# arpg/vicalib

Measured on AMD Instinct MI355X. Metric: corner_residuals_per_sec, higher is better.
Workload: dtype f64

## Files before the change

include/vicalib_amd.h:

```cpp
#ifndef VICALIB_AMD_H_
#define VICALIB_AMD_H_

#ifdef __cplusplus
extern "C" {
#endif

typedef struct vc_calibrator vc_calibrator;

enum {
  VC_OK = 0,
  VC_ERR_NO_DEVICE = -1,
  VC_ERR_BAD_ARG = -2,
  VC_ERR_RUNNING = -3,
  VC_ERR_TIME_ORDER = -4,
  VC_ERR_TOO_MANY_POINTS = -5,
  VC_ERR_NUMERIC = -6,
  VC_ERR_UNSUPPORTED = -7,
  VC_ERR_NO_CONVERGENCE = -8
};

enum { VC_MODEL_FOV = 0, VC_MODEL_POLY2 = 1, VC_MODEL_POLY3 = 2, VC_MODEL_KB4 = 3, VC_MODEL_LINEAR = 4, VC_MODEL_RATIONAL6 = 5 };

int vc_create(vc_calibrator** out, int device);
void vc_destroy(vc_calibrator* h);
int vc_clear(vc_calibrator* h);

int vc_add_camera(vc_calibrator* h, int model, const double* params, int nparams, int width, int height,
                  const double T_ck[7]);
int vc_fix_camera_intrinsics(vc_calibrator* h, int should_fix);
int vc_add_frame(vc_calibrator* h, const double T_wk[7], double time);
int vc_set_frame_pose(vc_calibrator* h, int frame, const double T_wk[7]);
int vc_init_frame_poses_pnp(vc_calibrator* h, int* n_initialised);
int vc_pnp_planar(int model, const double* params, int nparams, int n, const double* p_w ,
                  const double* p_c , double T_cw[7], double* rms_px);
int vc_pnp_planar_ransac(int model, const double* params, int nparams, int n, const double* p_w, const double* p_c,
                         int iterations, double tol_px, double T_cw[7], double* rms_px, int* n_inliers, char* inlier);
int vc_set_pnp_ransac(vc_calibrator* h, int iterations, double tol_px);
int vc_add_observations(vc_calibrator* h, int frame, int camera, int n, const double* p_w ,
                        const double* p_c );
int vc_add_observation_tiles(vc_calibrator* h, int n_tiles, const int* tile_frame, const int* tile_cam,
                             const long long* tile_off , const double* points, int n_points,
                             const int* point_id, const double* p_c );
int vc_add_imu(vc_calibrator* h, int n, const double* gyro , const double* accel ,
               const double* time );

int vc_set_sigmas(vc_calibrator* h, double gyro_sigma, double accel_sigma);
int vc_set_biases(vc_calibrator* h, const double biases[6]);
int vc_set_scale_factor(vc_calibrator* h, const double scale[6]);
int vc_set_time_offset(vc_calibrator* h, double offset);
int vc_set_function_tolerance(vc_calibrator* h, double tol);
int vc_set_optimization_flags(vc_calibrator* h, int bias_active, int inertial_active, int rotation_only,
                              int optimize_time_offset);
int vc_set_max_iters(vc_calibrator* h, int max_iters);
int vc_set_tolerances(vc_calibrator* h, double gradient_tolerance, double parameter_tolerance);
int vc_set_calibrate_imu(vc_calibrator* h, int calibrate_imu);
int vc_set_remove_outliers(vc_calibrator* h, int remove_outliers, double outlier_threshold);

int vc_solve(vc_calibrator* h);
int vc_start(vc_calibrator* h);
int vc_resume(vc_calibrator* h);
int vc_set_stage_limit(vc_calibrator* h, int n);
int vc_is_running(vc_calibrator* h);
int vc_stop(vc_calibrator* h);

int vc_num_frames(vc_calibrator* h);
int vc_num_imu_blocks(vc_calibrator* h);
int vc_num_cameras(vc_calibrator* h);
int vc_get_camera(vc_calibrator* h, int camera, double* params, int* nparams, double T_ck[7]);
int vc_get_frame(vc_calibrator* h, int frame, double T_wk[7], double v_w[3], double* time);
int vc_get_biases(vc_calibrator* h, double biases[6]);
int vc_get_scale_factor(vc_calibrator* h, double scale[6]);
int vc_get_gravity(vc_calibrator* h, double g_dir[2]);
double vc_time_offset(vc_calibrator* h);
double vc_mean_squared_error(vc_calibrator* h);
int vc_get_camera_proj_rmse(vc_calibrator* h, double* rmse );
unsigned vc_get_num_iterations(vc_calibrator* h);
int vc_num_imu_measurements(vc_calibrator* h);
int vc_get_imu_measurements(vc_calibrator* h, double* gyro, double* accel, double* time, int max_n);
int vc_get_integration_poses(vc_calibrator* h, int id, double* poses, int max_poses);
int vc_print_results(vc_calibrator* h, char* buf, int len);
int vc_write_camera_models(vc_calibrator* h, const char* filename);

int vc_solution_covariance_dim(vc_calibrator* h);
int vc_get_solution_covariance(vc_calibrator* h, double* cov, int max_n, int* n);
int vc_get_solution_covariance_names(vc_calibrator* h, char* buf, int len);

int vc_set_gravity(vc_calibrator* h, const double g_dir[2]);
int vc_set_frame_velocities(vc_calibrator* h, const double* v_w , int n);
int vc_trace_len(vc_calibrator* h);
int vc_get_trace(vc_calibrator* h, double* rows, int max_rows);
typedef int (*vc_allreduce_fn)(void* ctx, double* device_buf, int count, int op );
int vc_set_shard(vc_calibrator* h, int rank, int world_size, vc_allreduce_fn fn, void* ctx);
void* vc_get_stream(vc_calibrator* h);
int vc_rccl_unique_id(void* out128);
int vc_set_shard_rccl(vc_calibrator* h, int rank, int world_size, const void* unique_id128);
typedef struct vc_shard_comm vc_shard_comm;
int vc_shard_comm_create(int device, int rank, int world_size, const void* unique_id128, vc_shard_comm** out);
int vc_set_shard_comm(vc_calibrator* h, vc_shard_comm* comm);
void vc_shard_comm_destroy(vc_shard_comm* comm);
long long vc_allreduce_calls(vc_calibrator* h);
int vc_shard_info(vc_calibrator* h, int* rank, int* world_size, int* rccl_ranks, int* rccl_rank);
int vc_pass_paths(vc_calibrator* h, int* out6);
const char* vc_last_error(void);
int vc_prepare(vc_calibrator* h);
int vc_linearize(vc_calibrator* h, double* cost, double* Hpp, double* gp, double* S, double* g_red,
                 double* hss_diag, double* g_s);
int vc_shared_dim(vc_calibrator* h);
int vc_step_hold(vc_calibrator* h, double radius, double* cost, double* delta_s, double* slam, double* frame_lam, double* poses,
                 double* vels, double* cams, double* imus);
int vc_run_iterations(vc_calibrator* h, int iters, int* jac_sweeps, int* res_sweeps);
int vc_download_state(vc_calibrator* h);
int vc_evaluate(vc_calibrator* h, double* cost, double* sum_sq);
int vc_time_kernels(vc_calibrator* h, int reps, double* jac_ms, double* res_ms);
int vc_set_kernel_timing(vc_calibrator* h, int on);
int vc_sync_timeouts(const vc_calibrator* h);
int vc_get_kernel_timing(vc_calibrator* h, char* names, int names_len, double* total_ms, long long* count, int max_entries);
int vc_time_stages(vc_calibrator* h, int reps, double out[6]);
int vc_get_imu_blocks(vc_calibrator* h, double* H, double* g, double* cost);
int vc_get_imu_weights(vc_calibrator* h, double* W);
int vc_report_compute(vc_calibrator* h, int bins_x, int bins_y);
int vc_report_corners(vc_calibrator* h, long long first, long long n, double* r, int* frame, int* camera, unsigned char* flags);
long long vc_report_num_corners(vc_calibrator* h);
int vc_report_num_views(vc_calibrator* h);
int vc_report_views(vc_calibrator* h, int* frame, int* camera, int* count, int* removed, double* sum_sq, double* max_err,
                    long long* worst_corner);
int vc_report_error_map(vc_calibrator* h, int camera, double* cells);
int vc_report_num_imu_blocks(vc_calibrator* h);
int vc_report_imu(vc_calibrator* h, double* whitened , double* unwhitened , unsigned char* flags);
int vc_time_report_sweeps(vc_calibrator* h, int reps, double out_ms[3]);
int vc_holdout_clear(vc_calibrator* h);
int vc_holdout_add_tiles(vc_calibrator* h, int n_tiles, const int* tile_frame, const int* tile_cam, const long long* tile_off ,
                         const double* points, int n_points, const int* point_id, const double* p_c );
int vc_holdout_compute(vc_calibrator* h, const double* seeds, int max_iters);
int vc_holdout_num_frames(vc_calibrator* h);
int vc_holdout_num_views(vc_calibrator* h);
long long vc_holdout_num_corners(vc_calibrator* h);
int vc_holdout_frames(vc_calibrator* h, double* T_wk , int* status, int* iterations, double* cost0, double* cost, int* behind);
int vc_holdout_views(vc_calibrator* h, int* frame, int* camera, int* count, double* sum_sq, double* max_err, long long* worst_corner);
int vc_holdout_corners(vc_calibrator* h, long long first, long long n, double* r , int* frame, int* camera);
int vc_holdout_camera_rmse(vc_calibrator* h, double* rmse , long long* count );
int vc_time_holdout(vc_calibrator* h, int reps, double out_ms[2]);
int vc_get_debug_stamps(vc_calibrator* h, long long out[32]);
long long vc_num_observations(vc_calibrator* h);
int vc_num_tiles(vc_calibrator* h);

typedef struct vc_detector vc_detector;
int vc_detector_create(int device, int width, int height, vc_detector** out);
void vc_detector_destroy(vc_detector* d);
int vc_detector_set_params(vc_detector* d, int black_on_white, double at_threshold, double at_window_ratio, double conic_min_area,
                           double conic_min_density, double conic_min_aspect);
int vc_detector_find(vc_detector* d, const unsigned char* image, int pitch, double* centres, int max_conics, int* n_found);
int vc_detector_find_conics(vc_detector* d, const unsigned char* image, int pitch, double* centres, double* conics, int* boxes, int max_conics,
                            int* n_found);
int vc_target_make_pattern(int rows, int cols, unsigned seed, int* pattern);
int vc_target_find(const double* centres, const double* conics, int n, const int* pattern, int rows, int cols, int* dot_index, int* n_matched);

typedef struct vc_undistorter vc_undistorter;
int vc_undistorter_create(int device, int model, const double* params, int nparams, int src_w, int src_h, const double dst_linear[4], int dst_w,
                          int dst_h, const double R_ds[9], int fill, vc_undistorter** out);
int vc_undistorter_create_for_camera(vc_calibrator* h, int camera, const double dst_linear[4], int dst_w, int dst_h, const double R_ds[9], int fill,
                                     vc_undistorter** out);
void vc_undistorter_destroy(vc_undistorter* u);
int vc_undistort_fit_linear(int model, const double* params, int nparams, int src_w, int src_h, int dst_w, int dst_h, double alpha, double dst_linear[4]);
int vc_undistort_images(vc_undistorter* u, int n, const unsigned char* src, int src_pitch, long long src_stride, unsigned char* dst, int dst_pitch,
                        long long dst_stride);
int vc_undistort_images_device(vc_undistorter* u, int n, const unsigned char* d_src, int src_pitch, long long src_stride, unsigned char* d_dst,
                               int dst_pitch, long long dst_stride);
void* vc_undistort_stream(vc_undistorter* u);
int vc_undistort_points(vc_undistorter* u, int n, const double* src_px , double* dst_px , unsigned char* valid );
int vc_undistort_get_map(vc_undistorter* u, float* map, unsigned char* valid);
int vc_undistort_get_linear(vc_undistorter* u, double dst_linear[4], int dst_size[2]);
int vc_time_undistort(vc_undistorter* u, int n_images, int reps, double out_ms[3]);

int vc_stereo_rectify_rotations(const double T_ck_a[7], const double T_ck_b[7], double R_ds_a[9], double R_ds_b[9], double* baseline);
int vc_stereo_fit_linear(int model_a, const double* params_a, int nparams_a, int w_a, int h_a, const double R_ds_a[9], int model_b, const double* params_b,
                         int nparams_b, int w_b, int h_b, const double R_ds_b[9], int dst_w, int dst_h, double alpha, double dst_linear[4]);
int vc_match_tiles(int n_tiles, const int* tile_frame, const int* tile_cam, const long long* tile_off , const int* point_id, int cam_a,
                   int cam_b, int* n_frames, long long* n_pairs, int* frame, long long* frame_off, long long* pos_a, long long* pos_b);
typedef struct vc_rectifier vc_rectifier;
int vc_rectifier_create(int device, int model_a, const double* params_a, int nparams_a, int w_a, int h_a, const double T_ck_a[7], int model_b,
                        const double* params_b, int nparams_b, int w_b, int h_b, const double T_ck_b[7], const double dst_linear[4], int dst_w, int dst_h,
                        double alpha, int fill, vc_rectifier** out);
int vc_rectifier_create_for_cameras(vc_calibrator* h, int cam_a, int cam_b, const double dst_linear[4], int dst_w, int dst_h, double alpha, int fill,
                                    vc_rectifier** out);
void vc_rectifier_destroy(vc_rectifier* r);
vc_undistorter* vc_rectifier_side(vc_rectifier* r, int side);
int vc_rectifier_get(vc_rectifier* r, double R_ds_a[9], double R_ds_b[9], double dst_linear[4], int dst_size[2], double* baseline, double T_ck_rect_a[7],
                     double T_ck_rect_b[7]);
int vc_rectify_pairs(vc_rectifier* r, int n, const unsigned char* src_a, int src_pitch_a, long long src_stride_a, const unsigned char* src_b, int src_pitch_b,
                     long long src_stride_b, unsigned char* dst_a, int dst_pitch_a, long long dst_stride_a, unsigned char* dst_b, int dst_pitch_b,
                     long long dst_stride_b);
int vc_rectify_check(vc_rectifier* r, int n_frames, const long long* frame_off , const double* px_a, const double* px_b, const double* target,
                     double* pairs_out, unsigned char* flags, int* count, int* invalid, double* sum_dv, double* sum_dv2, double* max_abs_dv, long long* worst,
                     double* mean_z, double* rigid_rms);
int vc_time_rectify_check(vc_rectifier* r, int reps, double* out_ms);

typedef struct vc_comparer vc_comparer;
int vc_comparer_create(int device, int model_a, const double* params_a, int nparams_a, int model_b, const double* params_b, int nparams_b, int width,
                       int height, int grid_x, int grid_y, vc_comparer** out);
int vc_comparer_create_for_camera(vc_calibrator* h, int camera, int model_b, const double* params_b, int nparams_b, int grid_x, int grid_y, vc_comparer** out);
void vc_comparer_destroy(vc_comparer* c);
int vc_compare_run(vc_comparer* c, double fit_radius, int max_iters, const double R_ba[9]);
int vc_compare_get_fit(vc_comparer* c, double R_ba[9], int* status, int* iterations, int* n_fit, int* n_left_out, double* cost0, double* cost);
int vc_compare_get_map(vc_comparer* c, double* diff , unsigned char* flags );
int vc_compare_summary(vc_comparer* c, long long* count, long long* invalid, double* sum_du, double* sum_dv, double* sum_sq, double* max_err, long long* worst);
int vc_compare_rings(vc_comparer* c, int n_rings, long long* count, long long* invalid, double* sum_sq, double* max_err);
int vc_compare_extrinsics(const double T_ck_a0[7], const double T_ck_ac[7], const double T_ck_b0[7], const double T_ck_bc[7], const double R_0[9],
                          const double R_c[9], double out4[4]);
int vc_time_compare(vc_comparer* c, int reps, double out_ms[3]);

typedef struct vc_converter vc_converter;
int vc_converter_create(int device, int model_a, const double* params_a, int nparams_a, int width, int height, int model_b, int grid_x, int grid_y,
                        vc_converter** out);
int vc_converter_create_for_camera(vc_calibrator* h, int camera, int model_b, int grid_x, int grid_y, vc_converter** out);
void vc_converter_destroy(vc_converter* c);
int vc_convert_run(vc_converter* c, double fit_radius, int max_iters, const double* start, unsigned int free_mask);
int vc_convert_get(vc_converter* c, double* params_b, int* nparams_b, int* status, int* iterations, int* n_fit, int* n_left_out, double* cost0, double* cost,
                   double* max_err, long long* worst);
int vc_convert_comparer(vc_converter* c, vc_comparer** out);
int vc_time_convert(vc_converter* c, int reps, double out_ms[3]);

typedef struct vc_uncertainty vc_uncertainty;
int vc_uncertainty_create(int device, int model, const double* params, int nparams, int width, int height, int grid_x, int grid_y, vc_uncertainty** out);
int vc_uncertainty_create_for_camera(vc_calibrator* h, int camera, int grid_x, int grid_y, vc_uncertainty** out);
void vc_uncertainty_destroy(vc_uncertainty* u);
int vc_uncertainty_run(vc_uncertainty* u, const double* cov, double sigma_px, double fit_radius);
int vc_uncertainty_get_fit(vc_uncertainty* u, double* M , double* G , int* n_fit);
int vc_uncertainty_get_map(vc_uncertainty* u, double* sigma , unsigned char* flags );
int vc_uncertainty_summary(vc_uncertainty* u, long long* count, long long* invalid, double* sum_var, double* max_lam, long long* worst);
int vc_uncertainty_rings(vc_uncertainty* u, int n_rings, long long* count, long long* invalid, double* sum_var, double* max_lam);
int vc_time_uncertainty(vc_uncertainty* u, int reps, double out_ms[3]);

#ifdef __cplusplus
}
#endif
#endif
```

vicalib_amd/csrc/vc_capi.cpp:

```cpp
#include "vc_calibrator.hpp"
#include "vc_uncertainty.hpp"

static int env_bit(const char* name) { const char* e = std::getenv(name); return (e && (e[0] == '0' || e[0] == '1')) ? e[0] - '0' : -1; }
Switches Switches::read() {
  Switches w;
  w.graphs = env_bit("VICALIB_AMD_GRAPHS") == 1;
  w.merged = env_bit("VICALIB_AMD_NO_MERGED_DECISION") != 1;
  w.batched = std::getenv("VICALIB_AMD_BATCHED") != nullptr;
  { const char* e = std::getenv("VICALIB_AMD_STREAM2_PRIORITY"); w.stream2_default = e && std::strcmp(e, "default") == 0; }
  w.flag_sync = env_bit("VICALIB_AMD_FLAG_SYNC");
  w.shard_flag_sync = env_bit("VICALIB_AMD_SHARD_FLAG_SYNC");
  w.force_shard_path = env_bit("VICALIB_AMD_FORCE_SHARD_PATH") == 1;
  { const char* e = std::getenv("VICALIB_AMD_SYNC_BOUND"); if (e && std::atoll(e) > 0) w.sync_bound = std::atoll(e); }
  { const char* e = std::getenv("VICALIB_AMD_SYNC_BOUND_FROM_PASS"); if (e) w.sync_bound_from_pass = std::atoi(e); }
  w.pre_backsub = env_bit("VICALIB_AMD_PRE_BACKSUB");
  w.chain.fold_l0 = env_bit("VICALIB_AMD_FOLD_L0") != 0; w.chain.back_path = env_bit("VICALIB_AMD_BACK_PATH") != 0;
  w.chain.hadd_early = env_bit("VICALIB_AMD_HADD_EARLY") != 0; w.chain.defer_tail = env_bit("VICALIB_AMD_DEFER_TAIL") != 0;
  return w;
}

extern "C" {

int vc_create(vc_calibrator** out, int device) {
  if (!out) return VC_ERR_BAD_ARG;
  *out = nullptr;
  int n = 0;
  if (hipGetDeviceCount(&n) != hipSuccess || n <= 0 || device < 0 || device >= n) return VC_ERR_NO_DEVICE;
  if (hipSetDevice(device) != hipSuccess) return VC_ERR_NO_DEVICE;
  vc_calibrator* h = new vc_calibrator();
  h->device = device;
  h->sw = Switches::read();
  h->use_graphs = h->sw.graphs; h->merged_enabled = h->sw.merged; h->shard_flag_sync = h->sw.shard_flag_sync == 1;
  const unsigned evf = hipEventDisableTiming | hipEventDisableSystemFence;
  int prio_least = 0, prio_greatest = 0;
  (void)hipDeviceGetStreamPriorityRange(&prio_least, &prio_greatest);
  auto make_stream2 = [&]() -> hipError_t {
    if (!h->sw.stream2_default && prio_least != prio_greatest && hipStreamCreateWithPriority(&h->stream2, hipStreamDefault, prio_least) == hipSuccess) { h->flag_sync = true; return hipSuccess; }
    (void)hipGetLastError();
    return hipStreamCreate(&h->stream2);
  };
  if (hipStreamCreate(&h->stream) != hipSuccess || make_stream2() != hipSuccess ||
      hipEventCreateWithFlags(&h->ev_state, evf) != hipSuccess || hipEventCreateWithFlags(&h->ev_pre, evf) != hipSuccess ||
      hipEventCreateWithFlags(&h->ev_weights, evf) != hipSuccess ||
      hipEventCreateWithFlags(&h->ev_imujac, evf) != hipSuccess ||
      hipEventCreateWithFlags(&h->ev_reduced, evf) != hipSuccess || hipEventCreateWithFlags(&h->ev_back, evf) != hipSuccess) { delete h; return VC_ERR_NO_DEVICE; }
  if (h->sw.flag_sync >= 0) h->flag_sync = h->sw.flag_sync == 1;
  if (h->d_sync.alloc(kSyncWords) != hipSuccess || hipMemset(h->d_sync.p, 0, kSyncWords * sizeof(long long)) != hipSuccess) { delete h; return VC_ERR_NO_DEVICE; }
  *out = h;
  return VC_OK;
}
void vc_destroy(vc_calibrator* h) { if (h) (void)hipSetDevice(h->device); delete h; }

int vc_clear(vc_calibrator* h) {
  if (!h) return VC_ERR_BAD_ARG;
  h->stop();
  h->cams.clear(); h->frames.clear(); h->o_frame.clear(); h->o_cam.clear(); h->o_pid.clear(); h->pts.clear(); h->o_pc.clear(); h->o_removed.clear();
  h->mse = 0; h->num_iterations = 0; h->is_bias_active = false; h->is_scale_active = false; h->is_inertial_active = false;
  h->is_visual_active = true; h->rotation_only = true; h->is_finished = false; h->gravity_initialized = false;
  h->outliers_removed = false; h->vis_mult = 0; h->imu_mult = 0; h->wsqrt_frames = 0; h->imu_w.clear(); h->imu_a.clear(); h->imu_t.clear(); h->imu_uploaded = 0; h->imu_end_time = -1.0; h->trace.clear(); h->stage = 0; h->device_dirty = true; h->obs_dirty = true;
  if (hipSetDevice(h->device) == hipSuccess) { h->rep.release(); h->hold.release(); }
  return VC_OK;
}

#define NOT_RUNNING(h) do { if (!(h)) return VC_ERR_BAD_ARG; if ((h)->is_running) return VC_ERR_RUNNING; } while (0)
#define BIND_DEVICE(h) do { if (hipSetDevice((h)->device) != hipSuccess) return VC_ERR_NO_DEVICE; } while (0)

int vc_add_camera(vc_calibrator* h, int model, const double* params, int nparams, int width, int height, const double T_ck[7]) {
  NOT_RUNNING(h);
  const int nk = model_nk(model);
  if (nk < 0 || !params || !T_ck || nparams != nk) return VC_ERR_BAD_ARG;
  if ((int)h->cams.size() >= kMaxCams) return VC_ERR_UNSUPPORTED;
  HostCam c; std::memset(&c, 0, sizeof(c));
  c.model = model; c.nk = nk; c.width = width; c.height = height;
  std::memcpy(c.K, params, nk * 8); std::memcpy(c.T_ck, T_ck, 56);
  h->cams.push_back(c); h->cam_rmse.resize(h->cams.size(), 0.0); h->device_dirty = true; h->hold.valid = false;
  return (int)h->cams.size() - 1;
}
int vc_fix_camera_intrinsics(vc_calibrator* h, int should_fix) { NOT_RUNNING(h); h->fix_intrinsics = should_fix != 0; h->device_dirty = true; h->hold.valid = false; return VC_OK; }
int vc_add_frame(vc_calibrator* h, const double T_wk[7], double time) {
  NOT_RUNNING(h);
  if (!T_wk) return VC_ERR_BAD_ARG;
  HostFrame f; std::memcpy(f.T, T_wk, 56); f.v[0] = f.v[1] = f.v[2] = 0; f.time = time;
  h->frames.push_back(f); h->device_dirty = true;
  return (int)h->frames.size() - 1;
}
int vc_set_frame_pose(vc_calibrator* h, int frame, const double T_wk[7]) {
  NOT_RUNNING(h);
  if (!T_wk || frame < 0 || frame >= (int)h->frames.size()) return VC_ERR_BAD_ARG;
  std::memcpy(h->frames[frame].T, T_wk, 56); h->device_dirty = true;
  return VC_OK;
}
int vc_pnp_planar(int model, const double* params, int nparams, int n, const double* p_w, const double* p_c, double T_cw[7], double* rms) {
  if (!params || !p_w || !p_c || !T_cw || model_nk(model) < 0 || nparams != model_nk(model)) return VC_ERR_BAD_ARG;
  return pnp_planar(model, params, n, p_w, p_c, T_cw, rms) ? VC_OK : VC_ERR_BAD_ARG;
}
int vc_pnp_planar_ransac(int model, const double* params, int nparams, int n, const double* p_w, const double* p_c, int iterations,
                         double tol_px, double T_cw[7], double* rms, int* n_inliers, char* inlier) {
  if (!params || !p_w || !p_c || !T_cw || model_nk(model) < 0 || nparams != model_nk(model) || iterations < 0 || !(tol_px >= 0.0)) return VC_ERR_BAD_ARG;
  return pnp_planar_ransac(model, params, n, p_w, p_c, iterations, tol_px, T_cw, rms, n_inliers, inlier) ? VC_OK : VC_ERR_BAD_ARG;
}
int vc_target_make_pattern(int rows, int cols, unsigned seed, int* pattern) {
  if (rows < 1 || cols < 1 || !pattern) return VC_ERR_BAD_ARG;
  grid_make_pattern(rows, cols, seed, pattern);
  return VC_OK;
}
int vc_target_find(const double* centres, const double* conics, int n, const int* pattern, int rows, int cols, int* dot_index, int* n_matched) {
  if (!centres || !conics || !pattern || !dot_index || n < 0 || rows < 1 || cols < 1) return VC_ERR_BAD_ARG;
  const int m = grid_find_target(centres, conics, nullptr, n, pattern, rows, cols, dot_index);
  if (n_matched) *n_matched = m;
  return VC_OK;
}
int vc_set_pnp_ransac(vc_calibrator* h, int iterations, double tol_px) {
  NOT_RUNNING(h);
  if (iterations < 0 || !(tol_px >= 0.0)) return VC_ERR_BAD_ARG;
  h->pnp_its = iterations; h->pnp_tol = tol_px;
  return VC_OK;
}
int vc_init_frame_poses_pnp(vc_calibrator* h, int* n_initialised) {
  NOT_RUNNING(h);
  const int N = (int)h->frames.size(), C = (int)h->cams.size();
  std::vector<std::vector<int>> view((size_t)N * std::max(C, 1));
  for (size_t i = 0; i < h->o_frame.size(); ++i) view[(size_t)h->o_frame[i] * C + h->o_cam[i]].push_back((int)i);
  int done = 0;
  std::vector<double> pw, pc;
  for (int f = 0; f < N; ++f) {
    bool cam0_good = false, any = false;
    for (int c = 0; c < C; ++c) {
      const std::vector<int>& ids = view[(size_t)f * C + c];
      if (ids.size() < 4) continue;
      if (c != 0 && cam0_good) break;
      pw.resize(3 * ids.size()); pc.resize(2 * ids.size());
      for (size_t k = 0; k < ids.size(); ++k) {
        std::memcpy(&pw[3 * k], &h->pts.xyz[3 * (size_t)h->o_pid[ids[k]]], 24); std::memcpy(&pc[2 * k], &h->o_pc[2 * (size_t)ids[k]], 16);
      }
      const HostCam& cm = h->cams[c];
      double T_cw[7], rms;
      if (!pnp_planar_ransac(cm.model, cm.K, (int)ids.size(), pw.data(), pc.data(), h->pnp_its, h->pnp_tol, T_cw, &rms, nullptr, nullptr)) continue;
      const double qi[4] = {-T_cw[0], -T_cw[1], -T_cw[2], T_cw[3]};
      double ti[3], tr[3], T[7];
      const double nt[3] = {-T_cw[4], -T_cw[5], -T_cw[6]};
      quat_rotate(qi, nt, ti);
      quat_mul(qi, cm.T_ck, T);
      quat_rotate(qi, cm.T_ck + 4, tr);
      for (int k = 0; k < 3; ++k) T[4 + k] = ti[k] + tr[k];
      std::memcpy(h->frames[f].T, T, 56);
      any = true;
      if (c == 0) cam0_good = true;
    }
    if (any) ++done;
  }
  if (n_initialised) *n_initialised = done;
  h->device_dirty = true;
  return VC_OK;
}
int vc_add_observations(vc_calibrator* h, int frame, int camera, int n, const double* p_w, const double* p_c) {
  NOT_RUNNING(h);
  if (n < 0 || (n > 0 && (!p_w || !p_c))) return VC_ERR_BAD_ARG;
  if (frame < 0 || frame >= (int)h->frames.size() || camera < 0 || camera >= (int)h->cams.size()) return VC_ERR_BAD_ARG;
  h->o_frame.insert(h->o_frame.end(), n, frame); h->o_cam.insert(h->o_cam.end(), n, camera);
  for (int i = 0; i < n; ++i) h->o_pid.push_back(h->pts.intern(p_w + 3 * (size_t)i));
  h->o_pc.insert(h->o_pc.end(), p_c, p_c + 2 * (size_t)n);
  h->o_removed.insert(h->o_removed.end(), n, 0); h->device_dirty = true; h->obs_dirty = true;
  return VC_OK;
}
int vc_add_observation_tiles(vc_calibrator* h, int n_tiles, const int* tile_frame, const int* tile_cam, const long long* tile_off,
                             const double* points, int n_points, const int* point_id, const double* p_c) {
  NOT_RUNNING(h);
  if (n_tiles < 0 || (n_tiles > 0 && (!tile_frame || !tile_cam || !tile_off || !points || !point_id || !p_c)) || n_points < 0) return VC_ERR_BAD_ARG;
  const int N = (int)h->frames.size(), C = (int)h->cams.size();
  for (int t = 0; t < n_tiles; ++t)
// ... 259 lines not shown
  return (int)out.size();
}

int vc_write_camera_models(vc_calibrator* h, const char* filename) {
  if (!h || !filename) return VC_ERR_BAD_ARG;
  FILE* f = std::fopen(filename, "w");
  if (!f) return VC_ERR_BAD_ARG;
  static const char* kType[] = {"calibu_fu_fv_u0_v0_w", "calibu_fu_fv_u0_v0_k1_k2", "calibu_fu_fv_u0_v0_k1_k2_k3",
                                "calibu_fu_fv_u0_v0_kb4", "calibu_fu_fv_u0_v0", "calibu_fu_fv_u0_v0_rational6"};
  std::lock_guard<std::mutex> lk(h->result_mutex);
  const bool robotics = h->calibrate_imu;
  const double rdf_rob[9] = {0, 1, 0, 0, 0, 1, 1, 0, 0}, rdf_vis[9] = {1, 0, 0, 0, 1, 0, 0, 0, 1};
  const double* rdf = robotics ? rdf_rob : rdf_vis;
  std::fprintf(f, "<rig>\n");
  for (size_t c = 0; c < h->cams.size(); ++c) {
    const HostCam& cm = h->cams[c];
    double R[9], Rt[9], t[3], M[9];
    quat_to_R(cm.T_ck, R);
    for (int i = 0; i < 3; ++i) for (int j = 0; j < 3; ++j) Rt[3 * i + j] = R[3 * j + i];
    for (int i = 0; i < 3; ++i) t[i] = -(Rt[3 * i] * cm.T_ck[4] + Rt[3 * i + 1] * cm.T_ck[5] + Rt[3 * i + 2] * cm.T_ck[6]);
    if (robotics) {
      for (int i = 0; i < 3; ++i) for (int j = 0; j < 3; ++j) M[3 * i + j] = Rt[3 * i] * rdf[3 * j] + Rt[3 * i + 1] * rdf[3 * j + 1] + Rt[3 * i + 2] * rdf[3 * j + 2];
    } else std::memcpy(M, Rt, sizeof(M));
    std::fprintf(f, "  <camera>\n    <camera_model name=\"\" index=\"%zu\" serialno=\"-1\" type=\"%s\" version=\"8\">\n", c, kType[cm.model]);
    std::fprintf(f, "      <width> %d </width>\n      <height> %d </height>\n", cm.width, cm.height);
    std::fprintf(f, "      <right> [ %g; %g; %g ] </right>\n      <down> [ %g; %g; %g ] </down>\n      <forward> [ %g; %g; %g ] </forward>\n",
                 rdf[0], rdf[1], rdf[2], rdf[3], rdf[4], rdf[5], rdf[6], rdf[7], rdf[8]);
    std::fprintf(f, "      <params> [ ");
    for (int i = 0; i < cm.nk; ++i) std::fprintf(f, "%.17g%s", cm.K[i], i + 1 < cm.nk ? "; " : " ");
    std::fprintf(f, "] </params>\n    </camera_model>\n    <pose>\n      <T_wc> [ %.17g, %.17g, %.17g, %.17g; %.17g, %.17g, %.17g, %.17g; %.17g, %.17g, %.17g, %.17g ] </T_wc>\n    </pose>\n  </camera>\n",
                 M[0], M[1], M[2], t[0], M[3], M[4], M[5], t[1], M[6], M[7], M[8], t[2]);
  }
  std::fprintf(f, "</rig>\n");
  std::fclose(f);
  return VC_OK;
}

int vc_trace_len(vc_calibrator* h) { if (!h) return VC_ERR_BAD_ARG; std::lock_guard<std::mutex> lk(h->result_mutex); return (int)h->trace.size(); }
int vc_get_trace(vc_calibrator* h, double* rows, int max_rows) {
  if (!h || !rows) return VC_ERR_BAD_ARG;
  std::lock_guard<std::mutex> lk(h->result_mutex);
  const int n = std::min<int>(max_rows, (int)h->trace.size());
  for (int i = 0; i < n; ++i) {
    const IterRecord& r = h->trace[i];
    double* o = rows + 10 * i;
    o[0] = r.iteration; o[1] = r.cost; o[2] = r.cost_change; o[3] = r.gmax; o[4] = r.gnorm; o[5] = r.step_norm; o[6] = r.rho;
    o[7] = r.radius; o[8] = r.accepted; o[9] = r.stage;
  }
  return n;
}
int vc_set_shard(vc_calibrator* h, int rank, int world_size, vc_allreduce_fn fn, void* ctx) {
  NOT_RUNNING(h);
  if (world_size < 1 || rank < 0 || rank >= world_size || (world_size > 1 && !fn)) return VC_ERR_BAD_ARG;
  h->drop_comm();
  h->rank = rank; h->world = world_size; h->allreduce = fn; h->allreduce_ctx = ctx; h->device_dirty = true;
  return VC_OK;
}
int vc_rccl_unique_id(void* out128) {
  if (!out128) return VC_ERR_BAD_ARG;
  if (!g_rccl.load()) return VC_ERR_UNSUPPORTED;
  RcclUniqueId id;
  if (g_rccl.GetUniqueId(&id) != 0) return VC_ERR_NO_DEVICE;
  std::memcpy(out128, &id, sizeof(id));
  return VC_OK;
}
static int rccl_comm_init(int device, int rank, int world_size, const void* unique_id128, void** comm) {
  g_last_error.clear();
  *comm = nullptr;
  if (world_size < 1 || rank < 0 || rank >= world_size || !unique_id128) return VC_ERR_BAD_ARG;
  if (!g_rccl.load()) {
    const char* de = dlerror();
    g_last_error = std::string("librccl could not be loaded: ") + (de ? de : "ncclGetUniqueId / ncclCommInitRank / ncclAllReduce / ncclCommDestroy not all found");
    return VC_ERR_UNSUPPORTED;
  }
  if (hipSetDevice(device) != hipSuccess) { g_last_error = "hipSetDevice(" + std::to_string(device) + ") failed"; return VC_ERR_NO_DEVICE; }
  RcclUniqueId id;
  std::memcpy(&id, unique_id128, sizeof(id));
  const int nrc = g_rccl.CommInitRank(comm, world_size, id, rank);
  if (nrc != 0) {
    g_last_error = "ncclCommInitRank(rank " + std::to_string(rank) + " of " + std::to_string(world_size) + ", device " + std::to_string(device) + ") = " + std::to_string(nrc);
    if (g_rccl.GetErrorString) g_last_error += std::string(" (") + g_rccl.GetErrorString(nrc) + ")";
    if (g_rccl.GetLastError) { const char* le = g_rccl.GetLastError(nullptr); if (le && le[0]) g_last_error += std::string(": ") + le; }
    *comm = nullptr; return VC_ERR_NO_DEVICE;
  }
  int cnt = -1, ur = -1;
  if (g_rccl.CommCount && g_rccl.CommCount(*comm, &cnt) == 0 && g_rccl.CommUserRank && g_rccl.CommUserRank(*comm, &ur) == 0 && (cnt != world_size || ur != rank)) {
    g_last_error = "ncclCommInitRank built a communicator of " + std::to_string(cnt) + " ranks with this process at rank " + std::to_string(ur) + "; asked for rank " +
                   std::to_string(rank) + " of " + std::to_string(world_size);
    (void)g_rccl.CommDestroy(*comm); *comm = nullptr; return VC_ERR_BAD_ARG;
  }
  return VC_OK;
}
static void attach_rccl(vc_calibrator* h, int rank, int world_size, void* comm, bool owned) {
  h->drop_comm();
  h->rccl_comm = comm; h->rccl_comm_owned = owned;
  h->rank = rank; h->world = world_size; h->allreduce = nullptr; h->allreduce_ctx = nullptr; h->device_dirty = true;
  if (world_size > 1 && h->sw.shard_flag_sync != 0) h->shard_flag_sync = true;
}
int vc_set_shard_rccl(vc_calibrator* h, int rank, int world_size, const void* unique_id128) {
  g_last_error.clear();
  NOT_RUNNING(h);
  h->drop_comm();
  void* comm = nullptr;
  const int rc = rccl_comm_init(h->device, rank, world_size, unique_id128, &comm);
  if (rc) return rc;
  attach_rccl(h, rank, world_size, comm, true);
  return VC_OK;
}
struct vc_shard_comm { void* comm; int device, rank, world; };
int vc_shard_comm_create(int device, int rank, int world_size, const void* unique_id128, vc_shard_comm** out) {
  if (!out) return VC_ERR_BAD_ARG;
  *out = nullptr;
  void* comm = nullptr;
  const int rc = rccl_comm_init(device, rank, world_size, unique_id128, &comm);
  if (rc) return rc;
  *out = new vc_shard_comm{comm, device, rank, world_size};
  return VC_OK;
}
int vc_set_shard_comm(vc_calibrator* h, vc_shard_comm* c) {
  g_last_error.clear();
  NOT_RUNNING(h);
  if (!c || !c->comm) return VC_ERR_BAD_ARG;
  if (c->device != h->device) { g_last_error = "vc_set_shard_comm: the communicator lives on device " + std::to_string(c->device) + ", the calibrator on " + std::to_string(h->device); return VC_ERR_BAD_ARG; }
  attach_rccl(h, c->rank, c->world, c->comm, false);
  return VC_OK;
}
void vc_shard_comm_destroy(vc_shard_comm* c) {
  if (!c) return;
  if (c->comm && g_rccl.CommDestroy) { (void)hipSetDevice(c->device); (void)hipDeviceSynchronize(); (void)g_rccl.CommDestroy(c->comm); }
  delete c;
}
long long vc_allreduce_calls(vc_calibrator* h) { return h ? h->rccl_calls : 0; }
int vc_shard_info(vc_calibrator* h, int* rank, int* world_size, int* rccl_ranks, int* rccl_rank) {
  if (!h) return VC_ERR_BAD_ARG;
  if (rank) *rank = h->rank;
  if (world_size) *world_size = h->world;
  int cnt = -1, ur = -1;
  if (h->rccl_comm && g_rccl.CommCount && g_rccl.CommUserRank) {
    if (g_rccl.CommCount(h->rccl_comm, &cnt) != 0) cnt = -1;
    if (g_rccl.CommUserRank(h->rccl_comm, &ur) != 0) ur = -1;
  }
  if (rccl_ranks) *rccl_ranks = cnt;
  if (rccl_rank) *rccl_rank = ur;
  return VC_OK;
}
const char* vc_last_error(void) { return g_last_error.c_str(); }
int vc_pass_paths(vc_calibrator* h, int* out6) {
  if (!h || !out6) return VC_ERR_BAD_ARG;
  const ChainPlan& p = h->plan;
  out6[0] = p.fold_l0; out6[1] = p.back_path; out6[2] = p.gram_top_stride > 0 ? 1 : 0; out6[3] = p.top_gram_launch;
  out6[4] = p.tail_deferred; out6[5] = p.hadd_early;
  return VC_OK;
}
void* vc_get_stream(vc_calibrator* h) { return h ? (void*)h->stream : nullptr; }
int vc_prepare(vc_calibrator* h) {
  NOT_RUNNING(h);
  if (h->vis_mult == 0) h->vis_mult = 1;
  if (h->imu_on() && h->imu_mult == 0) h->imu_mult = 1;
  return h->upload();
}
int vc_shared_dim(vc_calibrator* h) { return h ? h->dv.D : VC_ERR_BAD_ARG; }
int vc_linearize(vc_calibrator* h, double* cost, double* Hpp, double* gp, double* S, double* g_red, double* hss_diag, double* g_s) {
  NOT_RUNNING(h);
  BIND_DEVICE(h);
  if (h->device_dirty) { int rc = vc_prepare(h); if (rc) return rc; }
  double lin_cost = 0;
  int rc = h->linearize_hold(1e300, &lin_cost); if (rc) return rc;
  const int N = h->dv.n_frames - h->dv.pin_last, D = h->dv.D;
  if (cost) *cost = lin_cost;
  std::vector<double> fr((size_t)N * kFrStride);
  if ((Hpp || gp) && N) {
    if (hipMemcpy(fr.data(), h->dv.fr, fr.size() * 8, hipMemcpyDeviceToHost) != hipSuccess) return VC_ERR_NO_DEVICE;
    for (int f = 0; f < N; ++f) {
      const double* p = &fr[(size_t)f * kFrStride];
      if (gp) std::memcpy(gp + 6 * (size_t)f, p + kFrG, 48);
      if (Hpp) {
        double L[36] = {0}; int k = 0;
        for (int i = 0; i < 6; ++i) for (int j = 0; j <= i; ++j) L[i * 6 + j] = p[kFrL + k++];
        for (int i = 0; i < 6; ++i) for (int j = 0; j < 6; ++j) {
          double s = 0; for (int q = 0; q < 6; ++q) s += L[i * 6 + q] * L[j * 6 + q];
          Hpp[36 * (size_t)f + i * 6 + j] = s - (i == j ? p[kFrLam + i] : 0.0);
        }
      }
    }
  }
  std::vector<double> sb((size_t)D * D + 3 * D + 2);
  if (hipMemcpy(sb.data(), h->dv.Sbuf, sb.size() * 8, hipMemcpyDeviceToHost) != hipSuccess) return VC_ERR_NO_DEVICE;
  if (S) std::memcpy(S, sb.data(), (size_t)D * D * 8);
  if (g_red) std::memcpy(g_red, sb.data() + (size_t)D * D, D * 8);
  if (hss_diag) std::memcpy(hss_diag, sb.data() + (size_t)D * D + D, D * 8);
  if (g_s) std::memcpy(g_s, sb.data() + (size_t)D * D + 2 * D, D * 8);
  return VC_OK;
}
int vc_step_hold(vc_calibrator* h, double radius, double* cost, double* delta_s, double* slam, double* frame_lam, double* poses,
                 double* vels, double* cams, double* imus) {
  NOT_RUNNING(h);
  BIND_DEVICE(h);
  if (!(radius > 0.0)) return VC_ERR_BAD_ARG;
  if (h->device_dirty) { int rc = vc_prepare(h); if (rc) return rc; }
  double lin_cost = 0;
  int rc = h->linearize_hold(radius, &lin_cost); if (rc) return rc;
  const int N = h->dv.n_frames - h->dv.pin_last, C = h->dv.n_cams, D = h->dv.D, tr = 1 - h->cur;
  auto get = [&](double* dst, const double* src, size_t n) { return !dst || !n || hipMemcpy(dst, src, n * 8, hipMemcpyDeviceToHost) == hipSuccess; };
  if (cost) *cost = lin_cost;
  if (!get(delta_s, h->dv.delta_s, D) || !get(slam, h->dv.slam, D)) return VC_ERR_NO_DEVICE;
  if (frame_lam && N) {
    if (h->dv.imu_on) { if (!get(frame_lam, h->dv.clam, (size_t)N * 9)) return VC_ERR_NO_DEVICE; }
    else {
      std::vector<double> fr((size_t)N * kFrStride);
      if (!get(fr.data(), h->dv.fr, fr.size())) return VC_ERR_NO_DEVICE;
      for (int f = 0; f < N; ++f) for (int i = 0; i < 9; ++i) frame_lam[(size_t)f * 9 + i] = i < 6 ? fr[(size_t)f * kFrStride + kFrLam + i] : 0.0;
    }
  }
  if ((poses || vels) && N) {
    std::vector<double> p((size_t)N * kPoseStride), w((size_t)N * 4, 0.0);
    if (!get(p.data(), h->dv.poses[tr], p.size())) return VC_ERR_NO_DEVICE;
    if (h->dv.imu_on && !get(w.data(), h->dv.vel[tr], w.size())) return VC_ERR_NO_DEVICE;
    for (int f = 0; f < N; ++f) {
      if (poses) std::memcpy(poses + 7 * (size_t)f, &p[(size_t)f * kPoseStride], 56);
      if (vels) std::memcpy(vels + 3 * (size_t)f, &w[(size_t)f * 4], 24);
    }
  }
  if (cams && C) {
    std::vector<double> cr((size_t)C * kCamStride);
    if (!get(cr.data(), h->dv.cams[tr], cr.size())) return VC_ERR_NO_DEVICE;
    for (int c = 0; c < C; ++c) {
      double* o = cams + 17 * (size_t)c;
      std::memcpy(o, &cr[(size_t)c * kCamStride], 56);
      for (int i = 0; i < 10; ++i) o[7 + i] = i < h->cams[c].nk ? cr[(size_t)c * kCamStride + kCamK + i] : 0.0;
    }
  }
  if (imus) {
    double r[16] = {0};
    if (h->dv.imu_on && !get(r, h->dv.imus[tr], 16)) return VC_ERR_NO_DEVICE;
    std::memcpy(imus, r, 15 * 8);
  }
  return VC_OK;
}
int vc_evaluate(vc_calibrator* h, double* cost, double* sum_sq) {
  NOT_RUNNING(h);
  BIND_DEVICE(h);
  if (h->device_dirty) { int rc = vc_prepare(h); if (rc) return rc; }
  launch_reproj_res(h->dv, h->cur, (double)h->vis_mult, h->stream);
  launch_sum_tile_cost(h->dv, h->d_tmp.p, h->stream);
  double out[2];
  if (hipMemcpyAsync(out, h->d_tmp.p, 16, hipMemcpyDeviceToHost, h->stream) != hipSuccess) return VC_ERR_NO_DEVICE;
  if (hipStreamSynchronize(h->stream) != hipSuccess) return VC_ERR_NO_DEVICE;
  if (cost) *cost = out[0];
  if (sum_sq) *sum_sq = out[1];
  return VC_OK;
}
int vc_run_iterations(vc_calibrator* h, int iters, int* jac_sweeps, int* res_sweeps) {
  NOT_RUNNING(h);
  BIND_DEVICE(h);
  if (h->device_dirty) { int rc = vc_prepare(h); if (rc) return rc; }
  const int mi = h->max_iters;
  const long j0 = h->jac_sweeps, r0 = h->res_sweeps;
  h->should_run = true;
  ++h->solve_epoch;
  int done = 0, rc = VC_OK, guard = 0;
  while (done < iters && guard++ < iters + 4) {
    h->max_iters = std::min(mi, iters - done);
    const auto ts0 = std::chrono::steady_clock::now();
    rc = h->reset_state(); if (rc) break;
    Termination t; double fc; long nr;
    rc = h->solve_once(&t, &fc, &nr);
    if (rc) break;
    const int ran = h->last_iters;
    if (std::getenv("VICALIB_AMD_TIMING"))
      std::fprintf(stderr, "[vicalib_amd]   run_iterations: solve of %d iterations in %.3f ms\n", ran, std::chrono::duration<double, std::milli>(std::chrono::steady_clock::now() - ts0).count());
    done += std::max(ran, 1);
  }
  h->max_iters = mi;
  if (jac_sweeps) *jac_sweeps = (int)(h->jac_sweeps - j0);
  if (res_sweeps) *res_sweeps = (int)(h->res_sweeps - r0);
  return rc ? rc : done;
}
int vc_download_state(vc_calibrator* h) {
  NOT_RUNNING(h);
  BIND_DEVICE(h);
  if (h->device_dirty) return VC_OK;
  return h->download_state();
}
int vc_time_kernels(vc_calibrator* h, int reps, double* jac_ms, double* res_ms) {
  NOT_RUNNING(h);
  BIND_DEVICE(h);
  if (h->device_dirty) { int rc = vc_prepare(h); if (rc) return rc; }
  EventSet<3> evs;
  if (!evs.create()) return VC_ERR_NO_DEVICE;
  hipEvent_t e0 = evs.e[0], e1 = evs.e[1], e2 = evs.e[2];
  Ctrl c; h->init_ctrl(&c); c.hold = 1; if (c.mult < 1) c.mult = 1;
  if (hipMemcpy(h->d_ctrl.p, &c, sizeof(Ctrl), hipMemcpyHostToDevice) != hipSuccess) return VC_ERR_NO_DEVICE;
  h->dv.merged = 0; h->dv.par = 0; h->dv.ctrl = h->d_ctrl.p; h->dv.ctrl_prev = h->d_ctrl.p + 1;
  const double mult = c.mult;
  launch_reproj_jac(h->dv, h->stream); launch_reproj_res(h->dv, h->cur, mult, h->stream);
  (void)hipEventRecord(e0, h->stream);
  for (int i = 0; i < reps; ++i) launch_reproj_jac(h->dv, h->stream);
  (void)hipEventRecord(e1, h->stream);
  for (int i = 0; i < reps; ++i) launch_reproj_res(h->dv, h->cur, mult, h->stream);
  (void)hipEventRecord(e2, h->stream);
  if (hipEventSynchronize(e2) != hipSuccess) return VC_ERR_NO_DEVICE;
  float m1 = 0, m2 = 0;
  (void)hipEventElapsedTime(&m1, e0, e1); (void)hipEventElapsedTime(&m2, e1, e2);
  if (jac_ms) *jac_ms = m1 / reps;
  if (res_ms) *res_ms = m2 / reps;
  return VC_OK;
// ... 166 lines not shown
```

vicalib_amd/csrc/vc_chain_plan.hpp:

```cpp
#pragma once
#include <algorithm>

namespace vc {

constexpr int kChainM = 8;
constexpr int kChainMaxLevels = 16;
constexpr int kChainEarlyTopD = 31;

struct ChainSwitches { bool fold_l0 = true, back_path = true, hadd_early = true, defer_tail = true; };

struct ChainPlan {
  int n_levels = 0;
  int stride[kChainMaxLevels] = {}, m[kChainMaxLevels] = {}, groups[kChainMaxLevels] = {};
  int two[kChainMaxLevels] = {};
  int top_stride = 1;
  int forward_launches = 0;
  int bottom_groups = 1;
  int fold_l0 = 0;
  int gram_top_stride = 0;
  int back_path = 0;
  int top_gram_launch = 0;
  int hadd_early = 0;
  int tail_deferred = 0;
};

inline ChainPlan plan_chain(int N, int D, int n_cams, bool imu_on, bool sharded, const ChainSwitches& sw) {
  ChainPlan p;
  if (N < 1) return p;
  long st = 1;
  while ((N - 1) / st + 1 > kChainM - 1) {
    const int l = p.n_levels++;
    p.stride[l] = (int)st; p.m[l] = kChainM; p.groups[l] = (int)((N - 1) / (st * kChainM) + 1);
    st *= kChainM;
  }
  p.top_stride = (int)st;
  p.forward_launches = p.n_levels + 1;
  if (p.n_levels > 0) p.bottom_groups = p.groups[0];
  const int cpl = (D + 1 + 27 + 63) / 64;
  for (int l = 0; l < p.n_levels; ++l) p.two[l] = (cpl <= 1 || (cpl <= 2 && p.groups[l] <= 256)) ? 1 : 0;
  if (!imu_on) return p;
  p.fold_l0 = (sw.fold_l0 && !sharded && D + 1 + 27 <= 64 && n_cams <= 2 && p.n_levels >= 1) ? 1 : 0;
  p.gram_top_stride = (N <= 4096 && D + 1 + 27 <= 128) ? p.top_stride : 0;
  p.back_path = (sw.back_path && N <= 4096) ? 1 : 0;
  p.top_gram_launch = (p.gram_top_stride > 0 && !(D <= kChainEarlyTopD && !sharded)) ? 1 : 0;
  p.hadd_early = (sw.hadd_early && p.gram_top_stride > 0 && p.n_levels >= 2 && p.two[1]) ? 1 : 0;
  p.tail_deferred = (sw.defer_tail && p.back_path && p.n_levels >= 3 && p.n_levels <= 5) ? 1 : 0;
  return p;
}

}
```

vicalib_amd/csrc/vc_imu_kernels.hip:

```cpp
#include <hip/hip_runtime.h>
#include <algorithm>
#include <cstdlib>
#include "vc_math.hpp"
#include "vc_imu.hpp"
#include "vc_imu_weights.hpp"
#include "vc_device.h"
#include "vc_kutil.hpp"
#include "vc_reduced_tail.hpp"
#include "vc_shared_blocks.hpp"

namespace vc {

__device__ __forceinline__ ImuView imu_view(const DevView& v) { ImuView b = {v.imu_t, v.imu_w, v.imu_a, v.n_imu, v.imu_avg_dt}; return b; }

constexpr int kImuJacLds = 34 * 9 + 6;
struct SegTab {
  unsigned short v[kSegStride];
  constexpr SegTab() : v() { for (int e = 0; e < kSegLen; ++e) { int a = 0, b = 0; seg_entry(e, &a, &b); v[e] = (unsigned short)(a | (b << 8)); } }
};
__constant__ SegTab d_seg_tab = SegTab();
constexpr int kSegIters = (kSegLen + 31) / 32;
#ifndef VC_IJ_MFMA
#define VC_IJ_MFMA 1
#endif
struct SegInv {
  unsigned short v[9][64][4];
  constexpr SegInv() : v() {
    for (int t = 0; t < 9; ++t) for (int l = 0; l < 64; ++l) for (int g = 0; g < 4; ++g) v[t][l][g] = 0xffff;
    for (int e = 0; e < kSegLen; ++e) {
      int a = 0, b = 0; seg_entry(e, &a, &b);
      const int I = a / 16, J = b / 16, rt = a % 16;
      v[I * 3 + J][(rt % 4) * 16 + b % 16][rt / 4] = (unsigned short)e;
    }
  }
};
__constant__ SegInv d_seg_inv = SegInv();
#ifdef VC_IJ_STAMPS
#define IJSTAMP(i) do { if (blockIdx.x == 0 && threadIdx.x == 0) v.dbg[i] = (long long)__builtin_amdgcn_s_memrealtime(); } while (0)
#else
#define IJSTAMP(i) do { } while (0)
#endif
__global__ __launch_bounds__(256) void k_imu_jac(DevView v, int wr, int trial) {
  __shared__ double sh[8 * kImuJacLds];
  __shared__ double s_wq[8 * 84];
  IJSTAMP(0);
  if (trial && v.sync_seq > 0 && workgroup_pass_void(v)) return;
  const Ctrl* ct = v.ctrl;
  if (ct->done || (!trial && !ct->need_lin)) {
    if (trial && v.final_wait > 0 && threadIdx.x == 0) __hip_atomic_fetch_add(v.sync_flags + 11, 1LL, __ATOMIC_RELAXED, __HIP_MEMORY_SCOPE_AGENT);
    return;
  }
  const int wave = threadIdx.x >> 6, lane = threadIdx.x & 63;
  const int half = lane >> 5, l = lane & 31;
  const int n_blocks = v.n_frames - 1;
  const int s_raw = (blockIdx.x * 4 + wave) * 2 + half;
  const bool exists = s_raw < n_blocks;
  const int s = exists ? s_raw : n_blocks - 1;
  const int cur = trial ? 1 - ct->cur : ct->cur, j = s + 1;
  double* Jl = sh + (wave * 2 + half) * kImuJacLds;
  const double* T2 = v.poses[cur] + (size_t)j * kPoseStride;
  const double* T1 = v.poses[cur] + (size_t)(j - 1) * kPoseStride;
  const double* v2 = v.vel[cur] + (size_t)j * 4;
  const double* v1 = v.vel[cur] + (size_t)(j - 1) * 4;
  const double* wq_g = v.wsqrtb[wr] + (size_t)s * 81;
  double* wq = s_wq + (wave * 2 + half) * 84;
  {
    double t3[3];
#pragma unroll
    for (int t = 0; t < 3; ++t) { const int idx = l + 32 * t; t3[t] = wq_g[idx < 81 ? idx : 0]; }
#pragma unroll
    for (int t = 0; t < 3; ++t) { const int idx = l + 32 * t; if (idx < 81) wq[idx] = t3[t]; }
  }
  const double* brec = v.imu_delta_blk + (size_t)s * kBlockDeltaStride;
  double r[9], dr[9];
  const int col = (l < 6) ? l : (l < 30 ? l + 3 : -1);
  const bool valid = brec[10] >= 0.0;
#if VC_IJ_MFMA
  unsigned long long seg_at[9];
#pragma unroll
  for (int t = 0; t < 9; ++t) seg_at[t] = t == 6 ? ~0ull : *reinterpret_cast<const unsigned long long*>(&d_seg_inv.v[t][lane][0]);
#else
  int seg_ab[kSegIters];
#pragma unroll
  for (int it = 0; it < kSegIters; ++it) { const int e = l + 32 * it; seg_ab[it] = d_seg_tab.v[e < kSegLen ? e : 0]; }
#endif
  wave_lds_sync();
  IJSTAMP(1);
  imu_block_final_direction(valid, brec, wq, v.rotation_only, T2, T1, v2, v1, v.imu_grav + cur * 16, col, r, dr);
  IJSTAMP(2);
  if (col >= 0) {
#pragma unroll
    for (int k = 0; k < 9; ++k) Jl[col * 9 + k] = dr[k];
  }
  if (l < 3) {
#pragma unroll
    for (int k = 0; k < 9; ++k) {
      const bool zeroed = v.rotation_only && (k < 3 || k >= 6);
      Jl[(6 + l) * 9 + k] = (valid && !zeroed) ? -wq[(6 + l) * 9 + k] : 0.0;
    }
  }
  if (l == 31) {
#pragma unroll
    for (int k = 0; k < 9; ++k) Jl[33 * 9 + k] = r[k];
  }
  wave_lds_sync();
  double ss = 0.0;
#pragma unroll
  for (int k = 0; k < 9; ++k) ss += r[k] * r[k];
  double rho, rho1;
  loss_cauchy100(ss, &rho, &rho1);
  const double w = ct->imu_mult * rho1;
  if (trial) {
    __shared__ double s_cost[8];
    if (l == 0) s_cost[wave * 2 + half] = exists ? ct->imu_mult * rho : 0.0;
    __syncthreads();
    if (threadIdx.x == 0) {
      const double wc = ((s_cost[0] + s_cost[1]) + (s_cost[2] + s_cost[3])) + ((s_cost[4] + s_cost[5]) + (s_cost[6] + s_cost[7]));
      if (v.final_wait > 0) {
        __hip_atomic_store(v.wg_imu_trial + blockIdx.x, wc, __ATOMIC_RELAXED, __HIP_MEMORY_SCOPE_AGENT);
        __builtin_amdgcn_s_waitcnt(0);
        __hip_atomic_fetch_add(v.sync_flags + 4, 1LL, __ATOMIC_RELAXED, __HIP_MEMORY_SCOPE_AGENT);
      } else v.wg_imu_trial[blockIdx.x] = wc;
    }
  }
  IJSTAMP(3);
  const bool counted2 = trial && v.final_wait > 0;
#if VC_IJ_MFMA
  {
    const int i16 = lane & 15, kq = lane >> 4;
#pragma unroll
    for (int h = 0; h < 2; ++h) {
      if (!__builtin_amdgcn_readlane((int)exists, 32 * h)) continue;
      const double wh = readlane_f64(w, 32 * h);
      const int sb = __builtin_amdgcn_readlane(s, 32 * h);
      const double* Jb = sh + (wave * 2 + h) * kImuJacLds;
      double op[3][3];
#pragma unroll
      for (int T = 0; T < 3; ++T)
#pragma unroll
        for (int ks = 0; ks < 3; ++ks) {
          const int c = 16 * T + i16, rr = 4 * ks + kq;
          const bool in = c < 34 && rr < 9;
          const double x = Jb[in ? c * 9 + rr : 0];
          op[T][ks] = in ? x : 0.0;
        }
      double* rec = v.segb[cur] + (size_t)sb * kSegStride;
#pragma unroll
      for (int I = 0; I < 3; ++I)
#pragma unroll
        for (int J = 0; J < 3; ++J) {
          if (I == 2 && J == 0) continue;
          v4d acc = (v4d){0.0, 0.0, 0.0, 0.0};
#pragma unroll
          for (int ks = 0; ks < 3; ++ks) acc = __builtin_amdgcn_mfma_f64_16x16x4f64(op[I][ks], op[J][ks], acc, 0, 0, 0);
          const unsigned long long at = seg_at[I * 3 + J];
#pragma unroll
          for (int g = 0; g < 4; ++g) {
            const unsigned e = (unsigned)(at >> (16 * g)) & 0xffffu;
            if (e != 0xffffu) { if (counted2) __hip_atomic_store(rec + e, wh * acc[g], __ATOMIC_RELAXED, __HIP_MEMORY_SCOPE_AGENT); else rec[e] = wh * acc[g]; }
// ... 1258 lines not shown
#pragma unroll
        for (int k = 0; k < 9; ++k) img[k * ldx] += rp[(size_t)(a / s) * isz + k * ldx + pc];
      } else if (role == 3) {
#pragma unroll
        for (int k = 0; k < 9; ++k) img[k * ldx] = 0.0;
      }
    }
    return;
  }
  const int q = min(m - 1, (N - 1 - first) / s + 1);
  const int r = first + q * s;
  const bool has_r = q == m - 1 && r < N;
  const int nl = (q - 1) / 2, mid = nl + 1, nr = q - 1 - nl;
  const int dir = wave == 0 ? 1 : -1, cnt = wave == 0 ? nl : nr, i0 = wave == 0 ? 1 : q;
  double* XS = XS2[wave]; double* An = An2[wave]; double* Ls = Ls2[wave];
  const unsigned ldxb = 8u * (unsigned)ldx, iszb = 9u * ldxb;
  unsigned c0b = 0, stb = ldxb; int fsel = 0;
  if (role == 0 || role == 2) c0b = 8u * (unsigned)pc;
  else if (role == 1) { if (dir > 0) { c0b = 8u * (unsigned)(sub * ldx + ldw + 18); stb = 8; fsel = 1; } else c0b = 8u * (unsigned)(ldw + 18 + sub); }
  else if (role == 3) { if (dir > 0) c0b = 8u * (unsigned)pc; else { c0b = 8u * (unsigned)(sub * ldx + ldw + 18); stb = 8; fsel = 2; } }
  const unsigned ab = (unsigned)a * iszb;
  const int qa = group * m;
  auto load_cols = [&](int idx , bool first_of_sweep, bool with_image, double* x) {
    const int e = a + idx * s;
    const unsigned eb = (unsigned)e * iszb, emb = (unsigned)(e - s) * iszb;
    const unsigned fb = fsel == 1 ? ab : (fsel == 2 ? emb : eb);
    const unsigned pb = (unsigned)(qa + idx) * iszb;
    const bool live0 = with_image && (role == 0 || role == 2 || role == 3 || (role == 1 && first_of_sweep));
    const bool live1 = with_image && pend && (role == 0 || role == 2);
    double y0[9], y1[9];
#pragma unroll
    for (int k = 0; k < 9; ++k) y0[k] = ld_boff(v.cW, fb + c0b + k * stb);
    if (pend) {
#pragma unroll
      for (int k = 0; k < 9; ++k) y1[k] = ld_boff(rp, pb + c0b + k * stb);
    } else {
#pragma unroll
      for (int k = 0; k < 9; ++k) y1[k] = 0.0;
    }
#pragma unroll
    for (int k = 0; k < 9; ++k) x[k] = (live0 ? y0[k] : 0.0) + (live1 ? y1[k] : 0.0);
  };
  double xin[9], o[9], dacc[9];
#pragma unroll
  for (int k = 0; k < 9; ++k) { dacc[k] = 0.0; o[k] = 0.0; }
  double sep0[9];
  {
    const bool pa = pend && a > 0;
    const int pcd = role == 1 ? ldw + 9 + sub : pc;
    const double* img = v.cW + (size_t)a * isz + pcd;
    const double* rpa = rp + (size_t)(a / s) * isz + pcd;
    const bool mine = wave == 0 && (role == 0 || role == 1);
#pragma unroll
    for (int k = 0; k < 9; ++k) sep0[k] = mine ? img[k * ldx] + (pa ? rpa[k * ldx] : 0.0) : 0.0;
  }
  load_cols(cnt > 0 ? i0 : mid, true, cnt > 0 || wave == 0, xin);
  if (done) return;
#ifdef VC_F2_STAMPS
  if (NW == 1 && blockIdx.x == 0 && lvl == 1 && threadIdx.x == 0) v.dbg[0] = f2_t0;
#endif
  F2STAMP(1);
  if (role == 2) {
#pragma unroll
    for (int k = 0; k < 9; ++k) An[k * 9 + sub] = xin[k];
  }
  const ElimLds elds = {XS, An, Ls};
#ifdef VC_F2_STAMPS
  int el_n_ = 0;
  auto eliminate = [&](int e, double* x, double* out) {
    long long* st = (NW == 1 && blockIdx.x == 0 && lvl == 1 && threadIdx.x == 0 && el_n_ == 1) ? v.dbg + 16 : nullptr;
    ++el_n_;
    chain_eliminate<(NW > 1)>(v, v.cW + (size_t)e * isz, ldx, role, pc, sub, c == 0, elds, x, out, st);
  };
#else
  auto eliminate = [&](int e, double* x, double* out) { chain_eliminate<(NW > 1)>(v, v.cW + (size_t)e * isz, ldx, role, pc, sub, c == 0, elds, x, out); };
#endif
  for (int j = 0; ; ++j) {
    const bool at_mid = j == cnt;
    F2STAMP(2 + 2 * j);
    if (at_mid) {
      if (NW > 1) for (int jj = cnt; jj < max(nl, nr); ++jj) { gsync(); gsync(); }
      if (wave == 1) {
        if (cnt == 0) {
#pragma unroll
          for (int k = 0; k < 9; ++k) MID[k * W + c] = 0.0;
        }
#pragma unroll
        for (int k = 0; k < 9; ++k) SEPR[k * W + c] = dacc[k];
      }
      F2STAMP(12);
      __syncthreads();
      F2STAMP(13);
      if (wave == 1) return;
#pragma unroll
      for (int k = 0; k < 9; ++k) {
        if (role == 0 || role == 2) xin[k] += MID[k * W + c];
        else if (role == 3 && nr > 0) xin[k] = MID[k * W + nW + sub];
      }
      if (role == 2) {
#pragma unroll
        for (int k = 0; k < 9; ++k) An[k * 9 + sub] = xin[k];
      }
    }
    const int e = a + (at_mid ? mid : i0 + dir * j) * s;
#ifdef VC_EXP_NO_O_LOADS
    if (!at_mid) { for (int k = 0; k < 9; ++k) o[k] = xin[k] * 0.999; }
#else
    if (!at_mid)
      load_cols(j + 1 < cnt ? i0 + dir * (j + 1) : mid, false, j + 1 < cnt || wave == 0, o);
#endif
    double x[9], out[18];
#pragma unroll
    for (int k = 0; k < 9; ++k) x[k] = xin[k];
    eliminate(e, x, out);
    F2STAMP(3 + 2 * j);
#pragma unroll
    for (int k = 0; k < 9; ++k) dacc[k] += out[k];
    if (at_mid) {
      if (has_r && role < 4) {
        double* ri = rw + (size_t)(r / gs) * isz + pc;
        const bool keep = role == 0 || role == 2;
        const int src = role == 2 ? nW + sub : c;
#pragma unroll
        for (int k = 0; k < 9; ++k) ri[k * ldx] = keep ? -out[9 + k] - SEPR[k * W + src] : 0.0;
      }
      if (role == 3) {
        double* img = v.cW + (size_t)a * isz + pc;
#pragma unroll
        for (int k = 0; k < 9; ++k) img[k * ldx] = has_r ? -out[k] : 0.0;
      }
      break;
    }
    if (wave == 1 && j + 1 == cnt) {
#pragma unroll
      for (int k = 0; k < 9; ++k) MID[k * W + c] = -out[9 + k];
    } else {
#pragma unroll
      for (int k = 0; k < 9; ++k) xin[k] = o[k] - (role == 3 ? 0.0 : out[9 + k]);
      if (role == 2) {
#pragma unroll
        for (int k = 0; k < 9; ++k) An[k * 9 + sub] = xin[k];
      }
    }
  }
  if (role == 0 || role == 1) {
    const int pcd = role == 1 ? ldw + 9 + sub : pc;
    double* img = v.cW + (size_t)a * isz + pcd;
#pragma unroll
    for (int k = 0; k < 9; ++k) img[k * ldx] = sep0[k] - dacc[k];
  }
  F2STAMP(14);
}

constexpr int kL0Ld = 48;
template <int CMAX>
__global__ __launch_bounds__(256) void k_chain_l0(DevView v) {
  constexpr int W = 64;
  __shared__ __attribute__((aligned(16))) double XS2[2][9 * kXsLd];
  __shared__ double An2[2][81], Ls2[2][81];
  __shared__ double MID[9 * W], SEPR[9 * W];
  __shared__ double IMG[8][9 * kL0Ld];
  __shared__ int READY[12];
  __shared__ double BW[4][CMAX * kGStride + kInitPad];
  __shared__ double SUMW[4][CMAX * kGStride + kGStride + 16];
  __shared__ CamDesc s_cd2[4][kMaxCams];
  __shared__ double s_R2[4][kMaxCams * 9];
  const int tid = threadIdx.x, wv = __builtin_amdgcn_readfirstlane((int)(threadIdx.x >> 6)), lane = threadIdx.x & 63, group = blockIdx.x;
#ifdef VC_L0_STAMPS
  const long long l0t0_ = (long long)__builtin_amdgcn_s_memrealtime();
  int l0n_ = 1;
#define L0STAMP() do { if (blockIdx.x == gridDim.x / 2 && lane == 0 && l0n_ < 16) { v.dbg[(wv == 0 ? 0 : 16) + l0n_] = (long long)__builtin_amdgcn_s_memrealtime(); ++l0n_; } } while (0)
#define L0B(i) do { if (blockIdx.x == gridDim.x / 2 && lane == 0 && wv == 2 && it == 1) v.dbg[24 + (i)] = (long long)__builtin_amdgcn_s_memrealtime(); } while (0)
#else
#define L0STAMP() do { } while (0)
#define L0B(i) do { } while (0)
#endif
  const int N = v.n_frames, D = v.D, C = v.n_cams, ldw = v.ldw, ldx = v.ldx, nW = D + 1, ncol = nW + 27;
  const Ctrl* ct = v.ctrl;
  const int a = group * 8, first = a + 1;
  const int q = first < N ? min(7, N - 1 - first + 1) : 0;
  const int r = first + q;
  const bool has_r = q == 7 && r < N;
  const int nl = q > 0 ? (q - 1) / 2 : 0, mid = nl + 1, nr = q > 0 ? q - 1 - nl : 0;
  const size_t isz = (size_t)9 * ldx;
  auto wait_ready = [&](int slot) {
    while (__hip_atomic_load(&READY[slot], __ATOMIC_RELAXED, __HIP_MEMORY_SCOPE_WORKGROUP) == 0) __builtin_amdgcn_s_sleep(1);
    __builtin_amdgcn_fence(__ATOMIC_ACQUIRE, "wavefront");
    __builtin_amdgcn_wave_barrier();
  };
  auto set_ready = [&](int slot) {
    __builtin_amdgcn_fence(__ATOMIC_RELEASE, "wavefront");
    __builtin_amdgcn_s_waitcnt(0xc07f);
    __builtin_amdgcn_wave_barrier();
    if (lane == 0) __hip_atomic_store(&READY[slot], 1, __ATOMIC_RELAXED, __HIP_MEMORY_SCOPE_WORKGROUP);
  };
  if (tid < 12) READY[tid] = 0;
  __syncthreads();
  const int b = wv;
  const int nmine = q == 0 ? (wv == 3 ? 1 : 0)
                  : wv == 0 ? 1 : wv == 1 ? (nr > 0 ? 1 : 0) : wv == 2 ? (nl > 0 ? nl : 0) : (nr > 0 ? nr - 1 : 0) + 1;
  auto slot_of = [&](int i) {
    return q == 0 ? 0 : wv == 0 ? (nl > 0 ? 1 : mid) : wv == 1 ? q : wv == 2 ? (i < nl - 1 ? 2 + i : mid) : (i < nr - 1 ? q - 1 - i : 0);
  };
  int sp_col = -1;
#pragma unroll
  for (int a2 = 0; a2 < 15; ++a2) sp_col = (lane == a2) ? v.imu_param_col[a2] : sp_col;
  auto load_fct = [&](int f) { return (lane < C && f < N) ? v.frame_cam_tile[(size_t)f * C + lane] : -1; };
  int fctA = -1, fctB = -1;
  if (nmine > 0) fctA = load_fct(a + slot_of(0));
  if (nmine > 1) fctB = load_fct(a + slot_of(1));
  if (ct->done) return;
  const int cur = ct->cur;
  const double* segc = v.segb[cur];
  const int init_scale = ct->init_scale, reuse = ct->reuse_diag;
  const double radius = ct->radius;
  const bool par = lane < 15 && sp_col >= 0;
  const int o_wc = par ? kSegWc + lane : 0, o_wp = par ? kSegWp + lane : 0, s_par = par ? 15 : 0;
  const int o_acc0 = kSegAcc + lane, o_acc1 = kSegAcc + (lane + 64 < 81 ? lane + 64 : 0), o_app0 = kSegApp + lane, o_app1 = kSegApp + (lane + 64 < 81 ? lane + 64 : 0);
  const int l9 = lane < 9 ? lane : 0;
  int o_ii[4];
#pragma unroll
  for (int qq = 0; qq < 4; ++qq) { const int e = lane + 64 * qq, a2 = e >> 4, b2 = e & 15; o_ii[qq] = a2 < 15 ? ((b2 < 15) ? kSegHii + a2 * 15 + b2 : kSegGi + a2) : 0; }
  auto issue = [&](int f_in, int fct_f, InitLoads<CMAX>& R) {
    const int f = __builtin_amdgcn_readfirstlane(f_in);
    const bool has_c = f >= 1, has_p = f + 1 < N;
    const double* rcs = segc + (size_t)(has_c ? f - 1 : 0) * kSegStride;
    const double* rps = segc + (size_t)(has_p ? f : 0) * kSegStride;
#pragma unroll
    for (int cc = 0; cc < CMAX; ++cc) {
      const int tc = __builtin_amdgcn_readfirstlane(__shfl(fct_f, cc, 64));
#pragma unroll
      for (int qq = 0; qq < 3; ++qq) R.gv[cc][qq] = 0.0;
      if (cc < C && tc >= 0) {
        const double* g = v.Gb[cur] + (size_t)tc * kGPack;
#pragma unroll
        for (int qq = 0; qq < 3; ++qq) { const int e = qq * 64 + lane; const double x = g[e < kGPack ? e : 0]; R.gv[cc][qq] = e < kGPack ? x : 0.0; }
      }
    }
    {
      const bool tile_cost = lane < C && fct_f >= 0, blk_cost = lane == 8 && has_c;
      const double* pcst = tile_cost ? v.tile_costb[cur] + fct_f : (blk_cost ? v.seg_costb[cur] + (f - 1) : v.cg);
      const double x = *pcst;
      R.cost_in = (tile_cost || blk_cost) ? x : 0.0;
    }
    double xa[9], xb[9], xc0, xc1, xp0, xp1, xi[4];
#pragma unroll
    for (int i = 0; i < 9; ++i) { xa[i] = rcs[o_wc + i * s_par]; xb[i] = rps[o_wp + i * s_par]; }
    xc0 = rcs[o_acc0]; xc1 = rcs[o_acc1]; xp0 = rps[o_app0]; xp1 = rps[o_app1];
    const double gc = rcs[kSegGc + l9], gp = rps[kSegGp + l9], s2 = v.cscale2[(size_t)f * 9 + l9], dgv = v.cdiag[(size_t)f * 9 + l9];
#pragma unroll
    for (int qq = 0; qq < 4; ++qq) xi[qq] = rcs[o_ii[qq]];
#pragma unroll
    for (int i = 0; i < 9; ++i) R.pre[i] = ((par && has_c) ? xa[i] : 0.0) + ((par && has_p) ? xb[i] : 0.0);
    const bool in1 = lane + 64 < 81, in9 = lane < 9;
    R.a_imu[0] = (has_c ? xc0 : 0.0) + (has_p ? xp0 : 0.0);
    R.a_imu[1] = ((in1 && has_c) ? xc1 : 0.0) + ((in1 && has_p) ? xp1 : 0.0);
    R.g_imu = ((in9 && has_c) ? gc : 0.0) + ((in9 && has_p) ? gp : 0.0);
    R.sc2_in = (in9 && !init_scale) ? s2 : 0.0;
    R.dg_in = (in9 && reuse) ? dgv : 0.0;
#pragma unroll
    for (int qq = 0; qq < 4; ++qq) R.isum_in[qq] = ((lane + 64 * qq) < 240 && has_c) ? xi[qq] : 0.0;
  };
  InitLoads<CMAX> RA, RB;
  if (nmine > 0) issue(a + slot_of(0), fctA, RA);
  if (nmine > 1) issue(a + slot_of(1), fctB, RB);
  int col_ci = 0;
  if (nmine > 0) {
    if (lane < kMaxCams) s_cd2[b][lane] = v.cd[lane];
    if (lane < C) { double Rm[9]; quat_to_R(v.cams[cur] + (size_t)lane * kCamStride, Rm); for (int k2 = 0; k2 < 9; ++k2) s_R2[b][lane * 9 + k2] = Rm[k2]; }
    if (lane < ncol) {
      const int col = lane, e = col - nW;
      int cam = 255, loc = 0, skip = (e >= 18 && e < 27) ? 1 : 0;
      if (col < D) {
        const int cc = v.col_cam[col];
        cam = cc >= 0 ? cc : 255; loc = v.col_local[col];
#pragma unroll
        for (int a2 = 0; a2 < 15; ++a2) skip |= (v.imu_param_col[a2] == col) ? 1 : 0;
      }
      col_ci = cam | (loc << 8) | (skip << 16);
    }
    wave_lds_sync_local();
  }
  double* Gw = BW[b];
  double* Hs = Gw + C * kGStride;
  double* As = Hs + 42;
  double* gs = As + 81;
  double* ls = gs + 9;
  int* tcam = reinterpret_cast<int*>(ls + 9);
  int* tinv = tcam + kMaxCams;
  double gsum[CMAX][3];
  double isum[4] = {0.0, 0.0, 0.0, 0.0};
  double csum = 0.0;
  int po[3], pm[3];
#pragma unroll
  for (int qq = 0; qq < 3; ++qq) {
    const int e = qq * 64 + lane;
    int rr = 0;
#pragma unroll
    for (int a2 = 1; a2 < 16; ++a2) rr += (e >= a2 * 16 - (a2 * (a2 - 1)) / 2) ? 1 : 0;
    const int cidx = rr + (e - (rr * 16 - (rr * (rr - 1)) / 2));
    po[qq] = e < kGPackGrad ? rr * 16 + cidx : (e < kGPack ? kGGrad + (e - kGPackGrad) : -1);
    pm[qq] = (e < kGPackGrad && cidx != rr) ? cidx * 16 + rr : -1;
  }
#pragma unroll
  for (int cc = 0; cc < CMAX; ++cc)
#pragma unroll
// ... 218 lines not shown
#pragma unroll
        for (int k = 0; k < 9; ++k) x[k] = im[k * kL0Ld + icol];
      }
    };
    double xin[9], o[9], dacc[9];
#pragma unroll
    for (int k = 0; k < 9; ++k) { dacc[k] = 0.0; o[k] = 0.0; }
    {
      const int e = a + (cnt > 0 ? i0 : mid);
      const bool wi = cnt > 0 || wave == 0;
      load_b(e, true, wi, xin);
      take_img(e, wi, xin);
    }
    if (role == 2) {
#pragma unroll
      for (int k = 0; k < 9; ++k) An[k * 9 + sub] = xin[k];
    }
    const ElimLds elds = {XS, An, Ls};
    auto eliminate = [&](int e, double* x, double* out) { chain_eliminate<false>(v, v.cW + (size_t)e * isz, ldx, role, pc, sub, c == 0, elds, x, out); };
    for (int j = 0; ; ++j) {
      const bool at_mid = j == cnt;
      if (at_mid) {
        if (wave == 1) {
          if (cnt == 0) {
#pragma unroll
            for (int k = 0; k < 9; ++k) MID[k * W + c] = 0.0;
          }
#pragma unroll
          for (int k = 0; k < 9; ++k) SEPR[k * W + c] = dacc[k];
        }
        publish_sums();
        __syncthreads();
        if (wave == 1) return;
#pragma unroll
        for (int k = 0; k < 9; ++k) {
          if (role == 0 || role == 2) xin[k] += MID[k * W + c];
          else if (role == 3 && nr > 0) xin[k] = MID[k * W + nW + sub];
        }
        if (role == 2) {
#pragma unroll
          for (int k = 0; k < 9; ++k) An[k * 9 + sub] = xin[k];
        }
      }
      const int e = a + (at_mid ? mid : i0 + dir * j);
      int en = 0; bool wn = false;
      if (!at_mid) {
        en = a + (j + 1 < cnt ? i0 + dir * (j + 1) : mid); wn = j + 1 < cnt || wave == 0;
        load_b(en, false, wn, o);
      }
      double x[9], out[18];
#pragma unroll
      for (int k = 0; k < 9; ++k) x[k] = xin[k];
      if (wv == 0) L0STAMP();
      eliminate(e, x, out);
      if (wv == 0) L0STAMP();
#pragma unroll
      for (int k = 0; k < 9; ++k) dacc[k] += out[k];
      if (at_mid) {
        if (has_r && role < 4) {
          double* ri = v.rX[0] + (size_t)(r / 8) * isz + pc;
          const bool keep = role == 0 || role == 2;
          const int src = role == 2 ? nW + sub : c;
#pragma unroll
          for (int k = 0; k < 9; ++k) ri[k * ldx] = keep ? -out[9 + k] - SEPR[k * W + src] : 0.0;
        }
        if (role == 3) {
          double* img = v.cW + (size_t)a * isz + pc;
#pragma unroll
          for (int k = 0; k < 9; ++k) img[k * ldx] = has_r ? -out[k] : 0.0;
        }
        break;
      }
      if (wave == 1 && j + 1 == cnt) {
#pragma unroll
        for (int k = 0; k < 9; ++k) MID[k * W + c] = -out[9 + k];
      } else {
        take_img(en, wn, o);
#pragma unroll
        for (int k = 0; k < 9; ++k) xin[k] = o[k] - (role == 3 ? 0.0 : out[9 + k]);
        if (role == 2) {
#pragma unroll
          for (int k = 0; k < 9; ++k) An[k * 9 + sub] = xin[k];
        }
      }
    }
    wait_ready(0);
    if (role == 0 || role == 1) {
      const int pcd = role == 1 ? ldw + 9 + sub : pc;
      double* img = v.cW + (size_t)a * isz + pcd;
#pragma unroll
      for (int k = 0; k < 9; ++k) img[k * ldx] = IMG[0][k * kL0Ld + icol] - dacc[k];
    }
#ifdef VC_L0_STAMPS
    __builtin_amdgcn_s_waitcnt(0);
    if (wv == 0) L0STAMP();
#endif
    return;
  }
  __syncthreads();
  const int nsum = C * kGStride + kGStride;
  if (wv == 3) {
#pragma unroll
    for (int cc = 0; cc < CMAX; ++cc)
      if (cc < C) {
#pragma unroll
        for (int qq = 0; qq < 3; ++qq) {
          if (po[qq] >= 0) SUMW[3][cc * kGStride + po[qq]] = gsum[cc][qq];
          if (pm[qq] >= 0) SUMW[3][cc * kGStride + pm[qq]] = gsum[cc][qq];
        }
      }
#pragma unroll
    for (int qq = 0; qq < 4; ++qq) SUMW[3][C * kGStride + qq * 64 + lane] = isum[qq];
    if (lane < 9) SUMW[3][nsum + lane] = csum;
    set_ready(8 + 3);
    return;
  }
#pragma unroll
  for (int cc = 0; cc < CMAX; ++cc)
    if (cc < C) {
#pragma unroll
      for (int qq = 0; qq < 3; ++qq) {
        if (po[qq] >= 0) Gw[cc * kGStride + po[qq]] = gsum[cc][qq];
        if (pm[qq] >= 0) Gw[cc * kGStride + pm[qq]] = gsum[cc][qq];
      }
    }
  wave_lds_sync_local();
  wait_ready(8 + 3);
  const bool sw = q > 0;
  if (sw) { wait_ready(8 + 0); wait_ready(8 + 1); }
  double* part = v.part + (size_t)group * v.part_stride;
  for (int e = lane; e < C * kGStride; e += 64) part[D * D + D + e] = ((Gw[e] + SUMW[3][e]) + (sw ? SUMW[0][e] : 0.0)) + (sw ? SUMW[1][e] : 0.0);
#pragma unroll
  for (int qq = 0; qq < 4; ++qq) {
    const int e = C * kGStride + qq * 64 + lane;
    part[D * D + D + e] = ((isum[qq] + SUMW[3][e]) + (sw ? SUMW[0][e] : 0.0)) + (sw ? SUMW[1][e] : 0.0);
  }
  for (int e = C * kGStride + 256 + lane; e < nsum; e += 64) part[D * D + D + e] = 0.0;
  {
    const double t2 = (lane < 9) ? csum : 0.0, t3 = (lane < 9) ? SUMW[3][nsum + lane] : 0.0;
    const double t0 = (lane < 9 && sw) ? SUMW[0][nsum + lane] : 0.0, t1 = (lane < 9 && sw) ? SUMW[1][nsum + lane] : 0.0;
    double u2 = 0.0, u3 = 0.0, u0 = 0.0, u1 = 0.0;
#pragma unroll
    for (int kk = 0; kk < 9; ++kk) { u2 += readlane_f64(t2, kk); u3 += readlane_f64(t3, kk); u0 += readlane_f64(t0, kk); u1 += readlane_f64(t1, kk); }
    if (lane == 0) part[v.part_stride - 1] = ((u2 + u3) + u0) + u1;
  }
}

#ifdef VC_BACK_STAMPS
#define BSTAMP(i) do { if (blockIdx.x == (top ? 0 : gridDim.x / 2) && threadIdx.x == 0 && lvl < 4) v.dbg[8 * lvl + (i)] = (long long)__builtin_amdgcn_s_memrealtime(); } while (0)
#else
#define BSTAMP(i) do { } while (0)
#endif
constexpr int kBackT0Frames = 1;
struct BackLevels { int n; int start[8]; int stride[8]; int m[8]; int two[8]; };
template <bool FUSED>
__device__ __forceinline__ void chain_back_group(const DevView& v, int s, int m, int top, int lvl, int two, int group, double* ds, double* dl) {
  const int done = v.ctrl->done;
  const int lane = threadIdx.x;
#ifdef VC_BACK_STAMPS
  const long long bs0_ = (long long)__builtin_amdgcn_s_memrealtime();
#endif
  const int N = v.n_frames, D = v.D, ldw = v.ldw, ldx = v.ldx;
  const long gs = (long)m * s;
  const int a = top ? -1 : (int)(group * gs);
  const int first = top ? 0 : a + s;
  const size_t isz = (size_t)9 * ldx;
  for (int j = lane; j < D; j += 64) ds[j] = v.delta_s[j];
  const int q = first < N ? (top ? (N - 1) / s + 1 : min(m - 1, (N - 1 - first) / s + 1)) : 0;
  const int r = first + q * s;
  double da[9], dn[9];
  const bool has_a = a >= 0 && a < N, has_r = !top && q > 0 && r < N;
  if (!FUSED) {
#pragma unroll
    for (int k = 0; k < 9; ++k) { da[k] = has_a ? v.cdelta[(size_t)a * 9 + k] : 0.0; dn[k] = has_r ? v.cdelta[(size_t)r * 9 + k] : 0.0; }
  }
  const int fi = lane / 9, k = lane % 9;
  const bool mine = fi < q;
  const int e = first + (mine ? fi : 0) * s;
  const bool two_sided = two && !top && q >= 1;
  const int fmid = (q - 1) / 2;
  double t = 0.0, dinv = 1.0, Qrow[9], Lcol[9];
#pragma unroll
  for (int c = 0; c < 9; ++c) { Qrow[c] = 0.0; Lcol[c] = 0.0; }
  if (top) wave_lds_sync();
#ifdef VC_BACK_STAMPS
  const long long bs1_ = (long long)__builtin_amdgcn_s_memrealtime();
#endif
  if (mine) {
    const double* img = v.cW + (size_t)e * isz;
    const double* Wr = img + (size_t)k * ldx;
#pragma unroll
    for (int c = 0; c < 9; ++c) { Qrow[c] = Wr[ldw + 18 + c]; Lcol[c] = (c > k) ? img[c * ldx + ldw + 9 + k] : 0.0; }
    dinv = 1.0 / Wr[ldw + 9 + k];
    double acc;
    if (top) { acc = Wr[D]; for (int j = 0; j < D; ++j) acc += Wr[j] * ds[j]; }
    else acc = v.ct0[(size_t)e * 9 + k];
    t = acc;
  }
  double Xs[9];
#pragma unroll
  for (int c = 0; c < 9; ++c) Xs[c] = (mine && a >= 0) ? v.cW[(size_t)e * isz + (size_t)k * ldx + ldw + c] : 0.0;
  if (done) return;
  if (FUSED) {
    if (lane == 0) {
      long long n = 0;
      while ((has_a && __hip_atomic_load(v.cready + a, __ATOMIC_RELAXED, __HIP_MEMORY_SCOPE_AGENT) < v.pass_id) ||
             (has_r && __hip_atomic_load(v.cready + r, __ATOMIC_RELAXED, __HIP_MEMORY_SCOPE_AGENT) < v.pass_id)) {
        __builtin_amdgcn_s_sleep(2);
        if (++n > 4000000) {
          if (v.sync_seq > 0) mark_sync_timeout(v, v.sync_seq); else atomicAdd(&v.flags[4 + 2 * v.par], 1);
          atomicAdd((unsigned long long*)&v.dbg[21], 1ull);
          break;
        }
      }
    }
    __builtin_amdgcn_wave_barrier();
    (void)__builtin_amdgcn_readfirstlane(lane);
#pragma unroll
    for (int k2 = 0; k2 < 9; ++k2) {
      da[k2] = has_a ? __hip_atomic_load(v.cdelta + (size_t)a * 9 + k2, __ATOMIC_RELAXED, __HIP_MEMORY_SCOPE_AGENT) : 0.0;
      dn[k2] = has_r ? __hip_atomic_load(v.cdelta + (size_t)r * 9 + k2, __ATOMIC_RELAXED, __HIP_MEMORY_SCOPE_AGENT) : 0.0;
    }
  }
  if (mine && a >= 0) {
    const bool right = two_sided && fi > fmid;
#pragma unroll
    for (int c = 0; c < 9; ++c) t += Xs[c] * (right ? dn[c] : da[c]);
  }
#ifdef VC_BACK_STAMPS
  if (__builtin_amdgcn_readfirstlane(__double2loint(t)) == 0x7fffffff) return;
  if (blockIdx.x == (top ? 0 : gridDim.x / 2) && threadIdx.x == 0 && lvl < 4) { v.dbg[8 * lvl] = bs0_; v.dbg[8 * lvl + 1] = bs1_; }
#endif
  BSTAMP(2);
  double my = 0.0;
  if (two_sided) {
    {
      double y = t;
#pragma unroll
      for (int c = 0; c < 9; ++c) y += Qrow[c] * dn[c];
#pragma unroll
      for (int j = 8; j >= 0; --j) {
        const double xj = readlane_f64(y * dinv, fmid * 9 + j);
        dn[j] = -xj;
        y -= Lcol[j] * xj;
      }
      if (fi == fmid) {
#pragma unroll
        for (int j = 0; j < 9; ++j) my = (j == k) ? dn[j] : my;
      }
    }
    double dl_[9], dr_[9];
#pragma unroll
    for (int j = 0; j < 9; ++j) { dl_[j] = dn[j]; dr_[j] = dn[j]; }
    const int nleft = fmid, nright = q - 1 - fmid;
    for (int st = 1; st <= max(nleft, nright); ++st) {
      const bool hl = st <= nleft, hr = st <= nright;
      const int il = hl ? fmid - st : 0, ir = hr ? fmid + st : 0;
      double yl = t, yr = t;
#pragma unroll
      for (int c = 0; c < 9; ++c) { yl += Qrow[c] * dl_[c]; yr += Qrow[c] * dr_[c]; }
#pragma unroll
      for (int j = 8; j >= 0; --j) {
        const double xl = readlane_f64(yl * dinv, il * 9 + j), xr = readlane_f64(yr * dinv, ir * 9 + j);
        if (hl) { dl_[j] = -xl; yl -= Lcol[j] * xl; }
        if (hr) { dr_[j] = -xr; yr -= Lcol[j] * xr; }
      }
      if (hl && fi == il) {
#pragma unroll
        for (int j = 0; j < 9; ++j) my = (j == k) ? dl_[j] : my;
      }
      if (hr && fi == ir) {
#pragma unroll
        for (int j = 0; j < 9; ++j) my = (j == k) ? dr_[j] : my;
      }
    }
  } else
  for (int i = q - 1; i >= 0; --i) {
    double y = t;
#pragma unroll
    for (int c = 0; c < 9; ++c) y += Qrow[c] * dn[c];
#pragma unroll
    for (int j = 8; j >= 0; --j) {
      const double xj = readlane_f64(y * dinv, i * 9 + j);
      dn[j] = -xj;
      y -= Lcol[j] * xj;
    }
    if (fi == i) {
#pragma unroll
      for (int j = 0; j < 9; ++j) my = (j == k) ? dn[j] : my;
    }
  }
#ifdef VC_BACK_STAMPS
  if (__builtin_amdgcn_readfirstlane(__double2loint(my)) == 0x7fffffff) return;
#endif
  BSTAMP(3);
  if (lvl != 0 && v.cready) {
    if (mine) __hip_atomic_store(v.cdelta + (size_t)e * 9 + k, my, __ATOMIC_RELAXED, __HIP_MEMORY_SCOPE_AGENT);
    __builtin_amdgcn_s_waitcnt(0);
    __builtin_amdgcn_wave_barrier();
    if (mine && k == 0) __hip_atomic_store(v.cready + e, v.pass_id, __ATOMIC_RELAXED, __HIP_MEMORY_SCOPE_AGENT);
  } else if (mine) v.cdelta[(size_t)e * 9 + k] = my;
  if (lvl != 0) { BSTAMP(4); return; }
  if (mine) dl[(fi + 1) * 9 + k] = my;
  if (lane < 9) dl[lane] = da[lane];
  wave_lds_sync();
  const int base = top ? 0 : a, cnt = top ? q : (a < N ? q + 1 : 0), off = top ? 1 : 0;
  double gd = 0, dld = 0, step2 = 0, x2 = 0, g2 = 0, gmax = 0;
  if (lane < cnt) {
    const int f = base + lane;
    const int cur = v.ctrl->cur;
    const bool pin_f = (f == 0 && v.pin_first), pin_l = (f == N - 1 && v.pin_last);
    double d[9];
#pragma unroll
    for (int i = 0; i < 9; ++i) d[i] = pin_f ? ds[v.sep_col0 + i] : pin_l ? ds[v.sep_col1 + i] : dl[(lane + off) * 9 + i];
    const double* pin = v.poses[cur] + (size_t)f * kPoseStride;
    double* pout = v.poses[1 - cur] + (size_t)f * kPoseStride;
    double Tin[7], Tout[7], dd[6];
    for (int i = 0; i < 7; ++i) Tin[i] = pin[i];
    for (int i = 0; i < 6; ++i) dd[i] = d[i];
    se3_plus(Tin, dd, Tout);
    for (int i = 0; i < 7; ++i) { pout[i] = Tout[i]; const double ee = Tout[i] - Tin[i]; step2 += ee * ee; x2 += Tin[i] * Tin[i]; }
    pout[7] = 0.0;
    const double* vin = v.vel[cur] + (size_t)f * 4;
    double* vout = v.vel[1 - cur] + (size_t)f * 4;
    for (int i = 0; i < 3; ++i) { const double dv = d[6 + i]; vout[i] = vin[i] + dv; step2 += dv * dv; x2 += vin[i] * vin[i]; }
    vout[3] = 0.0;
    for (int i = 0; i < 9; ++i) {
      const double gi = v.cg[(size_t)f * 9 + i];
      gd += gi * d[i]; dld += v.clam[(size_t)f * 9 + i] * d[i] * d[i]; g2 += gi * gi; gmax = fmax(gmax, fabs(gi));
    }
    if (pin_f || pin_l) { gd = 0; dld = 0; g2 = 0; gmax = 0; }
    if (pin_l) { step2 = 0; x2 = 0; }
  }
  gd = wave_sum(gd); dld = wave_sum(dld); step2 = wave_sum(step2); x2 = wave_sum(x2); g2 = wave_sum(g2);
#pragma unroll
  for (int o2 = 32; o2 > 0; o2 >>= 1) gmax = fmax(gmax, __shfl_down(gmax, o2, 64));
  if (lane == 0) {
    double* o = v.grp_part + (size_t)group * kNumScal;
    o[kScGd] = gd; o[kScDld] = dld; o[kScStep2] = step2; o[kScX2] = x2; o[kScG2] = g2; o[kScCost] = 0.0; o[kScGmax] = gmax; o[kScSq] = 0.0;
  }
  BSTAMP(4);
}

__global__ __launch_bounds__(64) void k_chain_back(DevView v, int s, int m, int top, int lvl, int two) {
  __shared__ double ds[192 + 8];
  __shared__ double dl[kChainM * 9];
  const int lane = threadIdx.x;
  const int D = v.D, ldx = v.ldx;
  const size_t isz = (size_t)9 * ldx;
  if (top && blockIdx.x > 0) {
    if (v.ctrl->done) return;
    const int f = (int)blockIdx.x - 1;
    double dsl[3];
#pragma unroll
    for (int u = 0; u < 3; ++u) { const int j = lane + 64 * u; dsl[u] = j < D ? v.delta_s[j] : (j == D ? 1.0 : 0.0); }
    double p[9];
#pragma unroll
    for (int kk = 0; kk < 9; ++kk) {
      const double* Wr = v.cW + (size_t)f * isz + (size_t)kk * ldx;
      double acc = 0.0;
#pragma unroll
      for (int w = 0; w < 3; ++w) { const int j = lane + 64 * w; if (j <= D) acc += Wr[j] * dsl[w]; }
      p[kk] = acc;
    }
#pragma unroll
    for (int kk = 0; kk < 9; ++kk) {
      const double t0 = wave_sum(p[kk]);
      if (lane == 0) v.ct0[(size_t)f * 9 + kk] = t0;
    }
    return;
  }
  chain_back_group<false>(v, s, m, top, lvl, two, (int)blockIdx.x, ds, dl);
}
__global__ __launch_bounds__(256) void k_chain_t0(DevView v) {
  if (v.ctrl->done) return;
  const int lane = threadIdx.x & 63, f = (int)blockIdx.x * 4 + (int)(threadIdx.x >> 6);
  if (f >= v.n_frames) return;
  const int D = v.D, ldx = v.ldx;
  double dsl[3];
#pragma unroll
  for (int u = 0; u < 3; ++u) { const int j = lane + 64 * u; dsl[u] = j < D ? v.delta_s[j] : (j == D ? 1.0 : 0.0); }
  double p[9];
#pragma unroll
  for (int kk = 0; kk < 9; ++kk) {
    const double* Wr = v.cW + ((size_t)f * 9 + kk) * ldx;
    double x[3];
#pragma unroll
    for (int w = 0; w < 3; ++w) { const int j = lane + 64 * w; x[w] = Wr[j <= D ? j : 0]; }
    double acc = 0.0;
#pragma unroll
    for (int w = 0; w < 3; ++w) { const int j = lane + 64 * w; acc += (j <= D) ? x[w] * dsl[w] : 0.0; }
    p[kk] = acc;
  }
#pragma unroll
  for (int kk = 0; kk < 9; ++kk) {
    const double t0 = wave_sum(p[kk]);
    if (lane == 0) v.ct0[(size_t)f * 9 + kk] = t0;
  }
}
__global__ __launch_bounds__(64) void k_chain_back_levels(DevView v, BackLevels L) {
  __shared__ double ds[192 + 8];
  __shared__ double dl[kChainM * 9];
  int li = 0;
#pragma unroll
  for (int i = 1; i < 8; ++i) if (i < L.n && (int)blockIdx.x >= L.start[i]) li = i;
  const int lvl = L.n - 1 - li;
  chain_back_group<true>(v, L.stride[li], L.m[li], 0, lvl, L.two[li], (int)blockIdx.x - L.start[li], ds, dl);
}

struct BackPath { int n; int stride[6]; int m[6]; int two[6]; int top_stride; int ldr; int dsw; int tail; };
constexpr int kTailLds = kMaxCams * kCamStride + 16 + 8 + 6 * 256;
__device__ __forceinline__ void reduced_tail_workgroup(const DevView& v, double* lds) {
  const int tid = threadIdx.x, D = v.D;
  if (tid >= 256) return;
  const Ctrl* ct = v.ctrl;
  const int cur = ct->cur, done = ct->done;
  if (done) return;
  double* s_cam = lds;
  CamDesc* s_cd = reinterpret_cast<CamDesc*>(lds + kMaxCams * kCamStride);
  int* s_ipc = reinterpret_cast<int*>(lds + kMaxCams * kCamStride + 16);
  double* red = lds + kMaxCams * kCamStride + 16 + 8;
  for (int i = tid; i < v.n_cams * kCamStride; i += 256) s_cam[i] = v.cams[cur][i];
  if (tid < kMaxCams) s_cd[tid] = v.cd[tid];
  if (tid >= 64 && tid < 64 + 15) s_ipc[tid - 64] = v.imu_param_col[tid - 64];
  double pre_imu = 0.0;
  if (v.imu_on && (tid >> 6) == (D <= 64 ? 0 : 1) && (tid & 63) < 16) pre_imu = v.imus[cur][tid & 63];
  __syncthreads();
  reduced_tail(v, cur, v.delta_s, v.Sbuf + (size_t)D * D + 2 * D, v.slam, s_cam, s_cd, s_ipc, pre_imu, nullptr, red, false, false);
}
constexpr int kPathRowCols = 37;
constexpr int kPathRowLoads = 37;
constexpr int kPathDl = 96;
template <int NWMAX, bool CT0>
#ifdef VC_BACK_PATH_EU
__global__ __launch_bounds__(64 * NWMAX) __attribute__((amdgpu_waves_per_eu(VC_BACK_PATH_EU, VC_BACK_PATH_EU))) void k_chain_back_path(DevView v, BackPath P) {
#else
__global__ __launch_bounds__(64 * NWMAX) void k_chain_back_path(DevView v, BackPath P) {
#endif
  extern __shared__ __attribute__((aligned(16))) double bp_lds[];
  if (P.tail && blockIdx.x == gridDim.x - 1) { reduced_tail_workgroup(v, bp_lds); return; }
  const int wv = __builtin_amdgcn_readfirstlane((int)(threadIdx.x >> 6)), lane = threadIdx.x & 63;
  const int nw = P.n + 1;
  double* DLall = bp_lds;
  double* DSW = DLall + nw * kPathDl + (size_t)wv * P.dsw;
  int* READY = reinterpret_cast<int*>(DLall + nw * kPathDl + nw * P.dsw);
  double* RW = DLall + nw * kPathDl + nw * P.dsw + 4 + (size_t)wv * 63 * P.ldr;
  double* DL = DLall + (size_t)wv * kPathDl;
  if (threadIdx.x < 8) READY[threadIdx.x] = 0;
  __syncthreads();
  auto wait_ready = [&](int slot) {
    while (__hip_atomic_load(&READY[slot], __ATOMIC_RELAXED, __HIP_MEMORY_SCOPE_WORKGROUP) == 0) __builtin_amdgcn_s_sleep(1);
    __builtin_amdgcn_fence(__ATOMIC_ACQUIRE, "wavefront");
    __builtin_amdgcn_wave_barrier();
  };
  auto set_ready = [&](int slot) {
    __builtin_amdgcn_fence(__ATOMIC_RELEASE, "wavefront");
    __builtin_amdgcn_s_waitcnt(0xc07f);
    __builtin_amdgcn_wave_barrier();
    if (lane == 0) __hip_atomic_store(&READY[slot], 1, __ATOMIC_RELAXED, __HIP_MEMORY_SCOPE_WORKGROUP);
  };
  const int done = v.ctrl->done;
  const int N = v.n_frames, D = v.D, ldw = v.ldw, ldx = v.ldx;
  const size_t isz = (size_t)9 * ldx;
  const bool top = wv == P.n;
  const int lvl = top ? P.n : wv;
  const int s = top ? P.top_stride : P.stride[lvl], m = top ? kChainM : P.m[lvl], two = top ? 0 : P.two[lvl];
  const long gs = (long)m * s;
  const long a0 = (long)blockIdx.x * P.m[0] * P.stride[0];
  const int a = top ? -1 : (int)((a0 / gs) * gs);
  const int first = top ? 0 : a + s;
  const int q = first < N ? (top ? (N - 1) / s + 1 : min(m - 1, (N - 1 - first) / s + 1)) : 0;
  const int r = first + q * s;
  const bool has_a = a >= 0 && a < N, has_r = !top && q > 0 && r < N;
  const int fi = lane / 9, k = lane % 9;
  const bool mine = fi < q;
  const int e = first + (mine ? fi : 0) * s;
  const bool two_sided = two && !top && q >= 1;
  const int fmid = (q - 1) / 2;
  const int ncolr = D + 1, nel = q * 9 * ncolr;
  double rv[CT0 ? 1 : kPathRowLoads];
  if (!CT0) {
    const int step_r = 64 / ncolr, step_c = 64 - step_r * ncolr;
    int row = lane / ncolr, col = lane - row * ncolr;
#pragma unroll
    for (int u = 0; u < kPathRowLoads; ++u) {
      const int idx = lane + 64 * u;
      const int f2 = (row * 57) >> 9, k2 = row - 9 * f2;
      const bool in = idx < nel;
      const double* src = v.cW + (size_t)(in ? first + f2 * s : 0) * isz + (size_t)(in ? k2 : 0) * ldx + (in ? col : 0);
      const double x = *src;
      rv[u] = in ? x : 0.0;
      row += step_r; col += step_c;
      if (col >= ncolr) { col -= ncolr; ++row; }
    }
  }
  double dsv[3];
#pragma unroll
  for (int u = 0; u < (CT0 ? 3 : 1); ++u) { const int j = lane + 64 * u; dsv[u] = v.delta_s[j < D ? j : 0]; }
  double dinv = 1.0, Qrow[9], Lcol[9], Xs[9], t0_in = 0.0;
  {
    const double* img = v.cW + (size_t)(mine ? e : 0) * isz;
    const double* Wr = img + (size_t)k * ldx;
#pragma unroll
    for (int c = 0; c < 9; ++c) {
      const double qv = Wr[ldw + 18 + c], lv = img[c * ldx + ldw + 9 + k], xv = Wr[ldw + c];
      Qrow[c] = mine ? qv : 0.0; Lcol[c] = (mine && c > k) ? lv : 0.0; Xs[c] = (mine && a >= 0) ? xv : 0.0;
    }
    const double dg = Wr[ldw + 9 + k];
    dinv = mine ? 1.0 / dg : 1.0;
    if (CT0) { const double tv = v.ct0[(size_t)(mine ? e : 0) * 9 + k]; t0_in = mine ? tv : 0.0; }
  }
  const int base = a, cnt = (a < N) ? q + 1 : 0;
  if (done) return;
#pragma unroll
  for (int u = 0; u < (CT0 ? 3 : 1); ++u) { const int j = lane + 64 * u; if (j < D) DSW[j] = dsv[u]; }
  double t = t0_in;
  if (!CT0) {
    int row = lane / ncolr, col = lane - row * ncolr;
    const int step_r = 64 / ncolr, step_c = 64 - step_r * ncolr;
#pragma unroll
    for (int u = 0; u < kPathRowLoads; ++u) {
      const int idx = lane + 64 * u;
      if (idx < nel) RW[row * P.ldr + col] = rv[u];
      row += step_r; col += step_c;
      if (col >= ncolr) { col -= ncolr; ++row; }
    }
    wave_lds_sync_local();
    if (mine) {
      const double* Rr = RW + (size_t)(fi * 9 + k) * P.ldr;
      double acc = Rr[D];
      for (int j = 0; j < D; ++j) acc += Rr[j] * DSW[j];
      t = acc;
    }
  }
  double da[9], dn[9], dr_in[9];
#pragma unroll
  for (int c = 0; c < 9; ++c) { da[c] = 0.0; dn[c] = 0.0; }
  if (!top) {
    wait_ready(lvl + 1);
    const double* DLp = DLall + (size_t)(lvl + 1) * kPathDl;
    int pos;
    if (lvl + 1 == P.n) pos = a / P.top_stride;
    else { const long gp = (long)P.m[lvl + 1] * P.stride[lvl + 1]; const int ap = (int)((a0 / gp) * gp); pos = (a - ap) / P.stride[lvl + 1]; }
#pragma unroll
    for (int c = 0; c < 9; ++c) {
      const double x0 = DLp[pos * 9 + c], x1 = DLp[(pos + 1) * 9 + c];
      da[c] = has_a ? x0 : 0.0; dn[c] = has_r ? x1 : 0.0;
    }
  }
#pragma unroll
  for (int c = 0; c < 9; ++c) dr_in[c] = dn[c];
  if (mine && a >= 0) {
    const bool right = two_sided && fi > fmid;
#pragma unroll
    for (int c = 0; c < 9; ++c) t += Xs[c] * (right ? dn[c] : da[c]);
  }
  double my = 0.0;
  if (two_sided) {
    {
      double y = t;
#pragma unroll
      for (int c = 0; c < 9; ++c) y += Qrow[c] * dn[c];
#pragma unroll
      for (int j = 8; j >= 0; --j) {
        const double xj = readlane_f64(y * dinv, fmid * 9 + j);
        dn[j] = -xj;
        y -= Lcol[j] * xj;
      }
      if (fi == fmid) {
#pragma unroll
        for (int j = 0; j < 9; ++j) my = (j == k) ? dn[j] : my;
      }
    }
    double dl_[9], dr_[9];
#pragma unroll
    for (int j = 0; j < 9; ++j) { dl_[j] = dn[j]; dr_[j] = dn[j]; }
    const int nleft = fmid, nright = q - 1 - fmid;
    for (int st = 1; st <= max(nleft, nright); ++st) {
      const bool hl = st <= nleft, hr = st <= nright;
      const int il = hl ? fmid - st : 0, ir = hr ? fmid + st : 0;
      double yl = t, yr = t;
#pragma unroll
      for (int c = 0; c < 9; ++c) { yl += Qrow[c] * dl_[c]; yr += Qrow[c] * dr_[c]; }
#pragma unroll
      for (int j = 8; j >= 0; --j) {
        const double xl = readlane_f64(yl * dinv, il * 9 + j), xr = readlane_f64(yr * dinv, ir * 9 + j);
        if (hl) { dl_[j] = -xl; yl -= Lcol[j] * xl; }
        if (hr) { dr_[j] = -xr; yr -= Lcol[j] * xr; }
      }
      if (hl && fi == il) {
#pragma unroll
        for (int j = 0; j < 9; ++j) my = (j == k) ? dl_[j] : my;
      }
      if (hr && fi == ir) {
#pragma unroll
        for (int j = 0; j < 9; ++j) my = (j == k) ? dr_[j] : my;
      }
    }
  } else
  for (int i = q - 1; i >= 0; --i) {
    double y = t;
#pragma unroll
    for (int c = 0; c < 9; ++c) y += Qrow[c] * dn[c];
#pragma unroll
    for (int j = 8; j >= 0; --j) {
      const double xj = readlane_f64(y * dinv, i * 9 + j);
      dn[j] = -xj;
      y -= Lcol[j] * xj;
    }
    if (fi == i) {
#pragma unroll
      for (int j = 0; j < 9; ++j) my = (j == k) ? dn[j] : my;
    }
  }
  if (mine) DL[(fi + (top ? 0 : 1)) * 9 + k] = my;
  if (!top && lane < 9) { DL[lane] = da[lane]; DL[(q + 1) * 9 + lane] = dr_in[lane]; }
  if (lvl != 0 || top) { set_ready(lvl); return; }
  wave_lds_sync_local();
  double gd = 0, dld = 0, step2 = 0, x2 = 0, g2 = 0, gmax = 0;
  if (lane < cnt) {
    const int f = base + lane;
    const int cur = v.ctrl->cur;
    double d[9], Tin[7], vin[3], gi9[9], lam9[9];
    {
      const double* pin = v.poses[cur] + (size_t)f * kPoseStride;
      const double* vi = v.vel[cur] + (size_t)f * 4;
#pragma unroll
      for (int i = 0; i < 7; ++i) Tin[i] = pin[i];
#pragma unroll
      for (int i = 0; i < 3; ++i) vin[i] = vi[i];
#pragma unroll
      for (int i = 0; i < 9; ++i) { gi9[i] = v.cg[(size_t)f * 9 + i]; lam9[i] = v.clam[(size_t)f * 9 + i]; }
    }
    const bool pin_f = (f == 0 && v.pin_first), pin_l = (f == N - 1 && v.pin_last);
    const int sc = pin_f ? v.sep_col0 : (pin_l ? v.sep_col1 : 0);
#pragma unroll
    for (int i = 0; i < 9; ++i) { const double dch = DL[lane * 9 + i], dsp = DSW[sc + i]; d[i] = (pin_f || pin_l) ? dsp : dch; }
    double* pout = v.poses[1 - cur] + (size_t)f * kPoseStride;
    double Tout[7], dd[6];
    for (int i = 0; i < 6; ++i) dd[i] = d[i];
    se3_plus(Tin, dd, Tout);
    for (int i = 0; i < 7; ++i) { pout[i] = Tout[i]; const double ee = Tout[i] - Tin[i]; step2 += ee * ee; x2 += Tin[i] * Tin[i]; }
    pout[7] = 0.0;
    double* vout = v.vel[1 - cur] + (size_t)f * 4;
    for (int i = 0; i < 3; ++i) { const double dv = d[6 + i]; vout[i] = vin[i] + dv; step2 += dv * dv; x2 += vin[i] * vin[i]; }
    vout[3] = 0.0;
    for (int i = 0; i < 9; ++i) {
      const double gi = gi9[i];
      gd += gi * d[i]; dld += lam9[i] * d[i] * d[i]; g2 += gi * gi; gmax = fmax(gmax, fabs(gi));
    }
    if (pin_f || pin_l) { gd = 0; dld = 0; g2 = 0; gmax = 0; }
    if (pin_l) { step2 = 0; x2 = 0; }
  }
  gd = wave_sum(gd); dld = wave_sum(dld); step2 = wave_sum(step2); x2 = wave_sum(x2); g2 = wave_sum(g2);
#pragma unroll
  for (int o2 = 32; o2 > 0; o2 >>= 1) gmax = fmax(gmax, __shfl_down(gmax, o2, 64));
  if (lane == 0) {
    double* o = v.grp_part + (size_t)blockIdx.x * kNumScal;
    o[kScGd] = gd; o[kScDld] = dld; o[kScStep2] = step2; o[kScX2] = x2; o[kScG2] = g2; o[kScCost] = 0.0; o[kScGmax] = gmax; o[kScSq] = 0.0;
  }
}

constexpr int kMaxPairsPerWaveI = 9;
#ifdef VC_GRAM_STAMPS
#define GSTAMP(i) do { if (blockIdx.x == gridDim.x / 2 && threadIdx.x == 0 && (i) < 16) v.dbg[i] = (long long)__builtin_amdgcn_s_memrealtime(); } while (0)
#else
#define GSTAMP(i) do { } while (0)
#endif
template <int NQ, int NL>
__device__ __forceinline__ void chain_gram_chunk(const DevView& v, int chunk, double* R , unsigned short* s_pair , int mask_stride, int gather_stride = 0, bool publish = false) {
  const Ctrl* ct = v.ctrl;
  if (ct->done) return;
  GSTAMP(0);
  const int tid = threadIdx.x, wave = __builtin_amdgcn_readfirstlane(tid >> 6), lane = tid & 63;
  const int D = v.D, ld = v.ldw, N = v.n_frames;
  const int nT = (D + 1 + 15) / 16, nPairs = nT * (nT + 1) / 2;
  const int fstep = gather_stride > 0 ? gather_stride : 1;
  const int f0 = gather_stride > 0 ? 0 : chunk * v.chunk_frames, f1 = gather_stride > 0 ? (N - 1) / gather_stride + 1 : min(f0 + v.chunk_frames, N);
  double* part = v.part + (size_t)chunk * v.part_stride;
  if (tid < nPairs) {
    int I = 0, J = 0;
    for (int k = 0; k < tid; ++k) if (++J == nT) { ++I; J = I; }
    s_pair[tid] = (unsigned short)(I | (J << 8));
  }
  const int step_r = 256 / ld, step_c = 256 - step_r * ld, row0 = tid / ld, col0 = tid - row0 * ld;
  [[maybe_unused]] int gs_ = 1;
  for (int pb = 0; pb < nPairs; pb += 4 * NQ) {
    v4d acc[NQ];
#pragma unroll
    for (int q = 0; q < NQ; ++q) acc[q] = (v4d){0.0, 0.0, 0.0, 0.0};
    double tmp[NL];
    auto request = [&](int fg) {
      const int nrow = min(4, f1 - fg) * 9;
      const double* src = v.cW + (size_t)fg * fstep * 9 * v.ldx;
      const unsigned skip = (unsigned)(fstep - 1) * 9u * (unsigned)v.ldx;
      unsigned mbits = 0u;
      if (mask_stride > 0) {
#pragma unroll
        for (int q = 0; q < 4; ++q) mbits |= ((fg + q) % mask_stride == 0) ? (1u << q) : 0u;
      }
      int row = row0, col = col0;
#pragma unroll
      for (int u = 0; u < NL; ++u) {
        const unsigned qf = (unsigned)(row * 57) >> 9;
        const bool masked = (mbits >> qf) & 1u;
        tmp[u] = (row < nrow && !masked) ? src[(unsigned)(row * v.ldx + col) + qf * skip] : 0.0;
        row += step_r; col += step_c;
        if (col >= ld) { col -= ld; ++row; }
      }
    };
    request(f0);
    for (int fg = f0; fg < f1; fg += 4) {
#pragma unroll
      for (int u = 0; u < NL; ++u) { const int i = tid + 256 * u; if (i < 36 * ld) R[i] = tmp[u]; }
      __syncthreads();
      GSTAMP(gs_); ++gs_;
      if (fg + 4 < f1) request(fg + 4);
      const double* rq = R + (lane >> 4) * ld + (lane & 15);
      int oa[NQ], ob[NQ];
#pragma unroll
      for (int q = 0; q < NQ; ++q) {
        const int p = min(pb + 4 * q + wave, nPairs - 1);
        const int ij = s_pair[p];
        oa[q] = (ij & 255) * 16; ob[q] = (ij >> 8) * 16;
      }
#pragma unroll
      for (int ks = 0; ks < 9; ++ks)
#pragma unroll
        for (int q = 0; q < NQ; ++q) acc[q] = __builtin_amdgcn_mfma_f64_16x16x4f64(rq[ks * 4 * ld + oa[q]], rq[ks * 4 * ld + ob[q]], acc[q], 0, 0, 0);
      __syncthreads();
      GSTAMP(gs_); ++gs_;
    }
#pragma unroll
    for (int q = 0; q < NQ; ++q) {
      const int p = pb + 4 * q + wave;
      if (p < nPairs) {
        const int ij = s_pair[p], I = ij & 255, J = ij >> 8;
#pragma unroll
        for (int g = 0; g < 4; ++g) {
          const int row = I * 16 + (lane >> 4) + 4 * g, col = J * 16 + (lane & 15);
          if (row < D && col <= D) {
            double* dst = col < D ? part + row * D + col : part + D * D + row;
            if (publish) __hip_atomic_store(dst, acc[q][g], __ATOMIC_RELAXED, __HIP_MEMORY_SCOPE_AGENT); else *dst = acc[q][g];
          }
        }
      }
    }
  }
  if (publish) {
    __builtin_amdgcn_s_waitcnt(0);
    __syncthreads();
    if (tid == 0) __hip_atomic_store(v.part_ready + chunk, v.pass_id, __ATOMIC_RELAXED, __HIP_MEMORY_SCOPE_AGENT);
  }
#ifdef VC_GRAM_STAMPS
  __builtin_amdgcn_s_waitcnt(0);
  GSTAMP(15);
#endif
}
template <int NQ, int NL>
__global__ __launch_bounds__(256, 2) void k_chain_gram(DevView v, int gather) {
  extern __shared__ __attribute__((aligned(16))) double R[];
  __shared__ unsigned short s_pair[128];
  if (gather) chain_gram_chunk<NQ, NL>(v, v.n_chunks, R, s_pair, 0, v.gram_top_stride);
  else chain_gram_chunk<NQ, NL>(v, (int)blockIdx.x, R, s_pair, v.gram_top_stride);
}
template <int NW, int NQ, int NL>
__global__ __launch_bounds__(256) void k_chain_top_gram(DevView v, int s, int m, int lvl) {
  extern __shared__ __attribute__((aligned(16))) double R[];
  __shared__ unsigned short s_pair[128];
  __shared__ __attribute__((aligned(16))) double XS[9 * kXsLd];
  __shared__ double An[81];
  __shared__ double Ls_all[NW * 81];
  if (blockIdx.x == 0) {
    if ((int)threadIdx.x >= 64 * NW) return;
    chain_fwd_group<1, NW>(v, s, m, 1, lvl, 0, (int)(threadIdx.x >> 6), XS, An, Ls_all);
    return;
  }
  if ((int)blockIdx.x == 1 + v.n_chunks) { hadd_side_job(v, R, 256); return; }
  if ((int)blockIdx.x > 1 + v.n_chunks) { part_sum_ride_job(v, (int)blockIdx.x - 2 - v.n_chunks, R); return; }
  chain_gram_chunk<NQ, NL>(v, (int)blockIdx.x - 1, R, s_pair, v.gram_top_stride, 0, v.part_ride != 0);
}

void launch_imu_delta(const DevView& v, hipStream_t s, int trial) {
  if (v.n_frames < 2) return;
  hipLaunchKernelGGL(k_imu_block, dim3((v.n_frames - 1 + 3) / 4), dim3(256), 0, s, v, trial);
}
void launch_imu_jac(const DevView& v, int wr, hipStream_t s, int trial) {
  if (v.n_frames < 2) return;
  hipLaunchKernelGGL(k_imu_jac, dim3((v.n_frames - 1 + 7) / 8), dim3(256), 0, s, v, wr, trial);
}
void launch_imu_weights(const DevView& v, int wr, hipStream_t s) {
  if (v.n_frames < 2) return;
  hipLaunchKernelGGL(k_imu_weights, dim3((v.n_frames - 1 + 3) / 4), dim3(64), 0, s, v, wr);
}
void launch_chain_gram(const DevView& v, hipStream_t s);
static void chain_levels(const DevView& v, const ChainPlan& p, hipStream_t s, bool forward) {
  const int N = v.n_frames;
  if (N < 1) return;
  const int nl = p.n_levels, top_stride = p.top_stride, m_top = kChainM;
  const int cpl = (v.D + 1 + 27 + 63) / 64;
  auto fwd = [&](int groups, int stride, int m, int top, int lvl) {
    if (!top && p.two[lvl]) {
      const int extra = (v.hadd_early && lvl == 1) ? (v.part_stride - (v.D * v.D + v.D) + 15) / 16 : 0;
      if (cpl <= 1) hipLaunchKernelGGL(k_chain_fwd2<1>, dim3(groups + extra), dim3(128), 0, s, v, stride, m, lvl, groups);
      else hipLaunchKernelGGL(k_chain_fwd2<2>, dim3(groups + extra), dim3(256), 0, s, v, stride, m, lvl, groups);
    }
    else if (cpl <= 1) hipLaunchKernelGGL((k_chain_fwd<1, 1>), dim3(groups), dim3(64), 0, s, v, stride, m, top, lvl);
    else if (cpl <= 2) hipLaunchKernelGGL((k_chain_fwd<1, 2>), dim3(groups), dim3(128), 0, s, v, stride, m, top, lvl);
    else if (cpl <= 3) hipLaunchKernelGGL((k_chain_fwd<1, 3>), dim3(groups), dim3(192), 0, s, v, stride, m, top, lvl);
    else hipLaunchKernelGGL((k_chain_fwd<1, 4>), dim3(groups), dim3(256), 0, s, v, stride, m, top, lvl);
  };
  if (forward) {
    for (int l = 0; l < nl; ++l) {
      if (l == 0 && v.fold_l0) {
        if (v.n_cams <= 1) hipLaunchKernelGGL(k_chain_l0<1>, dim3(p.groups[0]), dim3(256), 0, s, v);
        else hipLaunchKernelGGL(k_chain_l0<2>, dim3(p.groups[0]), dim3(256), 0, s, v);
      } else fwd(p.groups[l], p.stride[l], p.m[l], 0, l);
    }
    if (v.gram_top_stride > 0) {
      const size_t lds = std::max((size_t)36 * v.ldw, (size_t)(v.hadd_early ? kHaddLds : 0)) * sizeof(double);
      const int ride_blocks = (v.part_ride && v.hadd_early) ? (v.D * v.D + v.D + 15) / 16 : 0;
      const int nT = (v.D + 1 + 15) / 16, nPairs = nT * (nT + 1) / 2, nq = std::min(kMaxPairsPerWaveI, (nPairs + 3) / 4);
      const int nlr = (36 * v.ldw + 255) / 256;
      auto go = [&](auto kern) {
        if (lds > 40000) (void)hipFuncSetAttribute((const void*)kern, hipFuncAttributeMaxDynamicSharedMemorySize, (int)lds);
        hipLaunchKernelGGL(kern, dim3(1 + v.n_chunks + (v.hadd_early ? 1 : 0) + ride_blocks), dim3(256), lds, s, v, top_stride, m_top, nl);
      };
      if (cpl <= 1) { if (nq <= 1) go(k_chain_top_gram<1, 1, 7>); else go(k_chain_top_gram<1, 2, 7>); }
      else if (cpl <= 2) { if (nlr <= 12) go(k_chain_top_gram<2, 4, 12>); else if (nq <= 6) go(k_chain_top_gram<2, 6, 16>); else go(k_chain_top_gram<2, 9, 16>); }
      else if (cpl <= 3) { if (nlr <= 16) go(k_chain_top_gram<3, 9, 16>); else if (nlr <= 21) go(k_chain_top_gram<3, 9, 21>); else go(k_chain_top_gram<3, 9, 25>); }
      else { if (nlr <= 25) go(k_chain_top_gram<4, 9, 25>); else go(k_chain_top_gram<4, 9, 30>); }
    } else {
      fwd(1, top_stride, m_top, 1, nl);
    }
  } else {
    if (v.back_path && nl >= 1 && nl <= 5) {
      BackPath P; P.n = nl;
      for (int l = 0; l < 6; ++l) { P.stride[l] = l < nl ? p.stride[l] : 1; P.m[l] = l < nl ? p.m[l] : 2; P.two[l] = l < nl ? p.two[l] : 0; }
      const bool ct0 = v.D + 1 > kPathRowCols;
      P.top_stride = top_stride; P.ldr = ct0 ? 1 : ((v.D + 1) | 1); P.dsw = ((v.D + 63) / 64) * 64;
      if (ct0) hipLaunchKernelGGL(k_chain_t0, dim3((N + 3) / 4), dim3(256), 0, s, v);
      const int nw = nl + 1;
      P.tail = (v.tail_deferred && nw >= 4) ? 1 : 0;
      const size_t lds = std::max(((size_t)nw * kPathDl + (size_t)nw * P.dsw + 4 + (ct0 ? 0 : (size_t)nw * 63 * P.ldr)), (size_t)(P.tail ? kTailLds : 0)) * sizeof(double);
      static LdsGrant g4, g6;
      auto go = [&](auto kern, LdsGrant& g) {
        if (lds > 60000 && g.need(lds)) (void)hipFuncSetAttribute((const void*)kern, hipFuncAttributeMaxDynamicSharedMemorySize, (int)lds);
        hipLaunchKernelGGL(kern, dim3(p.groups[0] + P.tail), dim3(64 * nw), lds, s, v, P);
      };
      if (nw <= 4) { if (ct0) go(k_chain_back_path<4, true>, g4); else go(k_chain_back_path<4, false>, g4); }
      else { if (ct0) go(k_chain_back_path<6, true>, g6); else go(k_chain_back_path<6, false>, g6); }
      return;
    }
    hipLaunchKernelGGL(k_chain_back, dim3(1 + (nl > 0 ? (N + kBackT0Frames - 1) / kBackT0Frames : 0)), dim3(64), 0, s, v, top_stride, m_top, 1, nl, 0);
    int total_groups = 0;
    for (int l = 0; l < nl; ++l) total_groups += p.groups[l];
    static const int resident_limit = [] {
      int dev = 0, per_cu = 0; hipDeviceProp_t pr;
      if (hipGetDevice(&dev) != hipSuccess || hipGetDeviceProperties(&pr, dev) != hipSuccess ||
          hipOccupancyMaxActiveBlocksPerMultiprocessor(&per_cu, (const void*)k_chain_back_levels, 64, 0) != hipSuccess || per_cu <= 0) return 2048;
      return std::max(64, per_cu * pr.multiProcessorCount / 2);
    }();
    if (nl > 0 && nl <= 8 && v.cready && total_groups <= resident_limit) {
      BackLevels L; L.n = nl;
      int at = 0;
      for (int i = 0; i < nl; ++i) {
        const int l = nl - 1 - i;
        L.start[i] = at; L.stride[i] = p.stride[l]; L.m[i] = p.m[l]; L.two[i] = p.two[l];
        at += p.groups[l];
      }
      for (int i = nl; i < 8; ++i) { L.start[i] = 1 << 30; L.stride[i] = 1; L.m[i] = 2; L.two[i] = 0; }
      hipLaunchKernelGGL(k_chain_back_levels, dim3(at), dim3(64), 0, s, v, L);
    } else
    for (int l = nl - 1; l >= 0; --l)
      hipLaunchKernelGGL(k_chain_back, dim3(p.groups[l]), dim3(64), 0, s, v, p.stride[l], p.m[l], 0, l, p.two[l]);
  }
}
void launch_chain_init(const DevView& v, hipStream_t s) {
  const size_t slot = (size_t)v.n_cams * kGStride + kGStride;
  const size_t lds = std::max((size_t)4 * (v.n_cams * kGStride + kInitPad), 4 * slot) * sizeof(double);
  auto go = [&](auto kern) {
    if (lds > 65536) (void)hipFuncSetAttribute((const void*)kern, hipFuncAttributeMaxDynamicSharedMemorySize, (int)lds);
    hipLaunchKernelGGL(kern, dim3(v.n_chunks), dim3(256), lds, s, v);
  };
  if (v.n_cams <= 1) go(k_chain_init<1>); else if (v.n_cams <= 2) go(k_chain_init<2>); else if (v.n_cams <= 4) go(k_chain_init<4>); else go(k_chain_init<8>);
}
void launch_chain_fwd(const DevView& v, const ChainPlan& p, hipStream_t s) { chain_levels(v, p, s, true); }
static void chain_gram_go(const DevView& v, hipStream_t s, int gather) {
  const size_t lds = (size_t)36 * v.ldw * sizeof(double);
  const int nT = (v.D + 1 + 15) / 16, nPairs = nT * (nT + 1) / 2, nq = std::min(kMaxPairsPerWaveI, (nPairs + 3) / 4);
  auto go = [&](auto kern) {
    if (lds > 65536) (void)hipFuncSetAttribute((const void*)kern, hipFuncAttributeMaxDynamicSharedMemorySize, (int)lds);
    hipLaunchKernelGGL(kern, dim3(gather ? 1 : v.n_chunks), dim3(256), lds, s, v, gather);
  };
  const int nl = (36 * v.ldw + 255) / 256;
  if (nl <= 7) { if (nq <= 1) go(k_chain_gram<1, 7>); else go(k_chain_gram<2, 7>); }
  else if (nl <= 12) go(k_chain_gram<4, 12>);
  else if (nl <= 16) { if (nq <= 6) go(k_chain_gram<6, 16>); else go(k_chain_gram<9, 16>); }
  else if (nl <= 21) go(k_chain_gram<9, 21>);
  else if (nl <= 25) go(k_chain_gram<9, 25>);
  else go(k_chain_gram<9, 30>);
}
void launch_chain_gram(const DevView& v, hipStream_t s) { chain_gram_go(v, s, 0); }
void launch_chain_gram_top(const DevView& v, hipStream_t s) { chain_gram_go(v, s, 1); }
void launch_chain_solve_b(const DevView& v, const ChainPlan& p, hipStream_t s) { chain_levels(v, p, s, false); }

}
```

vicalib_amd/lib.py:

```python
from __future__ import annotations

import ctypes as C
import os
import numpy as np

_HERE = os.path.dirname(os.path.abspath(__file__))
LIB_PATH = os.environ.get("VICALIB_AMD_LIB") or os.path.join(_HERE, "libvicalib_amd.so")
_lib = None

VC_OK = 0
ERRORS = {-1: "VC_ERR_NO_DEVICE", -2: "VC_ERR_BAD_ARG", -3: "VC_ERR_RUNNING", -4: "VC_ERR_TIME_ORDER",
          -5: "VC_ERR_TOO_MANY_POINTS", -6: "VC_ERR_NUMERIC", -7: "VC_ERR_UNSUPPORTED", -8: "VC_ERR_NO_CONVERGENCE"}
ALLREDUCE_FN = C.CFUNCTYPE(C.c_int, C.c_void_p, C.c_void_p, C.c_int, C.c_int)

SYMBOLS = [
    "vc_create", "vc_destroy", "vc_clear", "vc_add_camera", "vc_fix_camera_intrinsics", "vc_add_frame", "vc_set_frame_pose",
    "vc_add_observations", "vc_add_observation_tiles", "vc_add_imu", "vc_set_sigmas", "vc_set_biases", "vc_set_scale_factor", "vc_set_time_offset",
    "vc_set_function_tolerance", "vc_set_optimization_flags", "vc_set_max_iters", "vc_set_tolerances", "vc_set_gravity", "vc_set_frame_velocities", "vc_set_calibrate_imu", "vc_set_remove_outliers",
    "vc_solve", "vc_start", "vc_resume", "vc_set_stage_limit", "vc_sync_timeouts", "vc_set_kernel_timing", "vc_get_kernel_timing", "vc_is_running", "vc_stop", "vc_num_frames", "vc_num_imu_blocks", "vc_num_cameras", "vc_get_camera", "vc_get_frame",
    "vc_get_biases", "vc_get_scale_factor", "vc_get_gravity", "vc_time_offset", "vc_mean_squared_error", "vc_get_camera_proj_rmse",
    "vc_get_num_iterations", "vc_num_imu_measurements", "vc_get_imu_measurements", "vc_get_integration_poses", "vc_print_results", "vc_write_camera_models", "vc_trace_len", "vc_get_trace", "vc_set_shard", "vc_get_stream", "vc_prepare",
    "vc_linearize", "vc_step_hold", "vc_shared_dim", "vc_run_iterations", "vc_download_state", "vc_evaluate", "vc_time_kernels", "vc_time_stages", "vc_get_imu_blocks", "vc_get_debug_stamps", "vc_num_observations", "vc_num_tiles",
    "vc_init_frame_poses_pnp", "vc_pnp_planar", "vc_pnp_planar_ransac", "vc_set_pnp_ransac", "vc_rccl_unique_id", "vc_set_shard_rccl", "vc_shard_comm_create", "vc_set_shard_comm", "vc_shard_comm_destroy", "vc_allreduce_calls", "vc_shard_info", "vc_pass_paths", "vc_last_error", "vc_get_imu_weights",
    "vc_solution_covariance_dim", "vc_get_solution_covariance", "vc_get_solution_covariance_names",
    "vc_target_make_pattern", "vc_target_find",
    "vc_report_compute", "vc_report_num_corners", "vc_report_corners", "vc_report_num_views", "vc_report_views", "vc_report_error_map", "vc_report_num_imu_blocks", "vc_report_imu", "vc_time_report_sweeps",
    "vc_holdout_clear", "vc_holdout_add_tiles", "vc_holdout_compute", "vc_holdout_num_frames", "vc_holdout_num_views", "vc_holdout_num_corners", "vc_holdout_frames", "vc_holdout_views",
    "vc_holdout_corners", "vc_holdout_camera_rmse", "vc_time_holdout",
    "vc_detector_create", "vc_detector_destroy", "vc_detector_set_params", "vc_detector_find", "vc_detector_find_conics",
    "vc_undistorter_create", "vc_undistorter_create_for_camera", "vc_undistorter_destroy", "vc_undistort_fit_linear", "vc_undistort_images",
    "vc_undistort_images_device", "vc_undistort_stream", "vc_undistort_points", "vc_undistort_get_map", "vc_undistort_get_linear", "vc_time_undistort",
    "vc_stereo_rectify_rotations", "vc_stereo_fit_linear", "vc_match_tiles", "vc_rectifier_create", "vc_rectifier_create_for_cameras", "vc_rectifier_destroy",
    "vc_rectifier_side", "vc_rectifier_get", "vc_rectify_pairs", "vc_rectify_check", "vc_time_rectify_check",
    "vc_comparer_create", "vc_comparer_create_for_camera", "vc_comparer_destroy", "vc_compare_run", "vc_compare_get_fit", "vc_compare_get_map",
    "vc_compare_summary", "vc_compare_rings", "vc_compare_extrinsics", "vc_time_compare",
    "vc_converter_create", "vc_converter_create_for_camera", "vc_converter_destroy", "vc_convert_run", "vc_convert_get", "vc_convert_comparer", "vc_time_convert",
    "vc_uncertainty_create", "vc_uncertainty_create_for_camera", "vc_uncertainty_destroy", "vc_uncertainty_run", "vc_uncertainty_get_fit", "vc_uncertainty_get_map",
    "vc_uncertainty_summary", "vc_uncertainty_rings", "vc_time_uncertainty",
]


class VicalibError(RuntimeError):
    pass


def target_make_pattern(rows, cols, seed=71):
    out = np.zeros((rows, cols), dtype=np.int32)
    _check(load().vc_target_make_pattern(int(rows), int(cols), C.c_uint(seed), out.ctypes.data_as(C.c_void_p)), "target_make_pattern")
    return out


def target_find(centres, conics, pattern):
    centres = np.ascontiguousarray(centres, dtype=np.float64); conics = np.ascontiguousarray(conics, dtype=np.float64)
    pattern = np.ascontiguousarray(pattern, dtype=np.int32)
    n = len(centres)
    idx = np.full(n, -1, dtype=np.int32); m = C.c_int(0)
    _check(load().vc_target_find(_d(centres), _d(conics), n, pattern.ctypes.data_as(C.c_void_p), pattern.shape[0], pattern.shape[1],
                                 idx.ctypes.data_as(C.c_void_p), C.byref(m)), "target_find")
    return idx, m.value


def pnp_planar(model, params, p_w, p_c):
    L = load()
    params = np.ascontiguousarray(params, dtype=np.float64)
    p_w = np.ascontiguousarray(p_w, dtype=np.float64); p_c = np.ascontiguousarray(p_c, dtype=np.float64)
    T = np.zeros(7); rms = C.c_double(0)
    from .synth import MODEL_IDS
    m = MODEL_IDS[model] if isinstance(model, str) else int(model)
    _check(L.vc_pnp_planar(m, _d(params), len(params), len(p_w), _d(p_w), _d(p_c), _d(T), C.byref(rms)), "pnp_planar")
    return T, rms.value


def pnp_planar_ransac(model, params, p_w, p_c, iterations=64, tol_px=2.0):
    L = load()
    params = np.ascontiguousarray(params, dtype=np.float64)
    p_w = np.ascontiguousarray(p_w, dtype=np.float64); p_c = np.ascontiguousarray(p_c, dtype=np.float64)
    T = np.zeros(7); rms = C.c_double(0); n_in = C.c_int(0); flags = np.zeros(len(p_w), dtype=np.int8)
    from .synth import MODEL_IDS
    m = MODEL_IDS[model] if isinstance(model, str) else int(model)
    _check(L.vc_pnp_planar_ransac(m, _d(params), len(params), len(p_w), _d(p_w), _d(p_c), int(iterations), C.c_double(tol_px), _d(T),
                                  C.byref(rms), C.byref(n_in), flags.ctypes.data_as(C.c_void_p)), "pnp_planar_ransac")
    return T, rms.value, flags.astype(bool)


def load():
    global _lib
    if _lib is None:
        if not os.path.exists(LIB_PATH):
            raise VicalibError(f"{LIB_PATH} is missing: build it with vicalib_amd/csrc/build.sh (no CPU fallback exists)")
        L = C.CDLL(LIB_PATH)
        L.vc_time_offset.restype = C.c_double
        L.vc_mean_squared_error.restype = C.c_double
        L.vc_get_num_iterations.restype = C.c_uint
        L.vc_get_stream.restype = C.c_void_p
        L.vc_undistort_stream.restype = C.c_void_p
        L.vc_rectifier_side.restype = C.c_void_p
        L.vc_num_observations.restype = C.c_longlong
        L.vc_report_num_corners.restype = C.c_longlong
        L.vc_holdout_num_corners.restype = C.c_longlong
        L.vc_allreduce_calls.restype = C.c_longlong
        L.vc_last_error.restype = C.c_char_p
        for name in ("vc_destroy", "vc_detector_destroy", "vc_shard_comm_destroy", "vc_undistorter_destroy", "vc_rectifier_destroy", "vc_comparer_destroy", "vc_converter_destroy",
                     "vc_uncertainty_destroy"):
            getattr(L, name).restype = None
        _lib = L
    return _lib


def _check(rc, what):
    if rc < 0:
        raise VicalibError(f"{what} failed: {ERRORS.get(rc, rc)}")
    return rc


def _d(a):
    return np.ascontiguousarray(a, dtype=np.float64).ctypes.data_as(C.c_void_p)


class ShardComm:

    def __init__(self, device, rank, world, group=None):
        import torch.distributed as dist
        self.L = load()
        self.rank, self.world = int(rank), int(world)
        buf = C.create_string_buffer(128)
        if rank == 0:
            _check(self.L.vc_rccl_unique_id(buf), "rccl_unique_id")
        box = [bytes(buf.raw)]
        if world > 1:
            dist.broadcast_object_list(box, src=0, group=group)
        self.h = C.c_void_p()
        rc = self.L.vc_shard_comm_create(int(device), self.rank, self.world, C.create_string_buffer(box[0], 128), C.byref(self.h))
        if rc != 0:
            self.h = None
            raise VicalibError("shard_comm_create: status %d: %s" % (rc, (self.L.vc_last_error() or b"").decode(errors="replace")))

    def close(self):
        if getattr(self, "h", None):
            self.L.vc_shard_comm_destroy(self.h)
            self.h = None


class ViCalibrator:
    def __init__(self, device: int = 0):
        self.L = load()
        self.h = C.c_void_p()
        _check(self.L.vc_create(C.byref(self.h), int(device)), "vc_create")
        self._cb = None
        self.nk = []

    def close(self):
        if getattr(self, "h", None):
            self.L.vc_destroy(self.h)
            self.h = None

    def __del__(self):
        self.close()

    def AddCamera(self, model, params, T_ck, width=640, height=480):
        params = np.ascontiguousarray(params, dtype=np.float64)
        self.nk.append(len(params))
        if isinstance(model, str):
            from .synth import MODEL_IDS
            model = MODEL_IDS[model]
        return _check(self.L.vc_add_camera(self.h, int(model), _d(params), len(params), int(width), int(height), _d(T_ck)), "AddCamera")

    def Clear(self):
        _check(self.L.vc_clear(self.h), "Clear")
        self.nk = []

    def FixCameraIntrinsics(self, should_fix=True):
        _check(self.L.vc_fix_camera_intrinsics(self.h, int(should_fix)), "FixCameraIntrinsics")

    def AddFrame(self, T_wk, time):
        return _check(self.L.vc_add_frame(self.h, _d(T_wk), C.c_double(time)), "AddFrame")

# ... 13 lines not shown

    def AddObservationTiles(self, tile_frame, tile_cam, tile_off, points, point_id, p_c):
        tf = np.ascontiguousarray(tile_frame, dtype=np.int32); tc = np.ascontiguousarray(tile_cam, dtype=np.int32)
        off = np.ascontiguousarray(tile_off, dtype=np.int64); pid = np.ascontiguousarray(point_id, dtype=np.int32)
        pts = np.ascontiguousarray(points, dtype=np.float64); pc = np.ascontiguousarray(p_c, dtype=np.float64)
        vp = lambda a: a.ctypes.data_as(C.c_void_p)
        _check(self.L.vc_add_observation_tiles(self.h, len(tf), vp(tf), vp(tc), vp(off), vp(pts), len(pts), vp(pid), vp(pc)), "AddObservationTiles")

    def AddImuMeasurements(self, gyro, accel, time):
        time = np.ascontiguousarray(time, dtype=np.float64)
        _check(self.L.vc_add_imu(self.h, int(len(time)), _d(gyro), _d(accel), _d(time)), "AddImuMeasurements")

    def SetSigmas(self, g, a): _check(self.L.vc_set_sigmas(self.h, C.c_double(g), C.c_double(a)), "SetSigmas")
    def SetBiases(self, b): _check(self.L.vc_set_biases(self.h, _d(b)), "SetBiases")
    def SetGravity(self, g): _check(self.L.vc_set_gravity(self.h, _d(np.asarray(g, dtype=np.float64))), "SetGravity")
    def SetScaleFactor(self, s): _check(self.L.vc_set_scale_factor(self.h, _d(s)), "SetScaleFactor")
    def SetTimeOffset(self, o): _check(self.L.vc_set_time_offset(self.h, C.c_double(o)), "SetTimeOffset")
    def SetFunctionTolerance(self, t): _check(self.L.vc_set_function_tolerance(self.h, C.c_double(t)), "SetFunctionTolerance")

    def SetOptimizationFlags(self, bias_active, inertial_active, rotation_only, optimize_time_offset):
        _check(self.L.vc_set_optimization_flags(self.h, int(bias_active), int(inertial_active), int(rotation_only), int(optimize_time_offset)), "SetOptimizationFlags")

    def SetTolerances(self, gradient_tolerance=1e-10, parameter_tolerance=1e-8):
        _check(self.L.vc_set_tolerances(self.h, C.c_double(gradient_tolerance), C.c_double(parameter_tolerance)), "SetTolerances")

    def SetMaxIters(self, m): _check(self.L.vc_set_max_iters(self.h, int(m)), "max_iters")
    def SetCalibrateImu(self, c): _check(self.L.vc_set_calibrate_imu(self.h, int(c)), "calibrate_imu")
    def SetRemoveOutliers(self, r, th=2.0): _check(self.L.vc_set_remove_outliers(self.h, int(r), C.c_double(th)), "remove_outliers")

    def Solve(self): return _check(self.L.vc_solve(self.h), "Solve")
    def Start(self): _check(self.L.vc_start(self.h), "Start")
    def SetStageLimit(self, n): _check(self.L.vc_set_stage_limit(self.h, int(n)), "SetStageLimit")
    def Resume(self): _check(self.L.vc_resume(self.h), "Resume")
    def IsRunning(self): return bool(self.L.vc_is_running(self.h))
    def Stop(self): _check(self.L.vc_stop(self.h), "Stop")
    def NumFrames(self): return self.L.vc_num_frames(self.h)
    def num_imu_blocks(self): return _check(self.L.vc_num_imu_blocks(self.h), "num_imu_blocks")
    def NumCameras(self): return self.L.vc_num_cameras(self.h)

    def GetCamera(self, c):
        K = np.zeros(10); n = C.c_int(0); T = np.zeros(7)
        _check(self.L.vc_get_camera(self.h, int(c), _d(K), C.byref(n), _d(T)), "GetCamera")
        return K[:n.value].copy(), T

    def GetFrame(self, f):
        T = np.zeros(7); v = np.zeros(3); t = C.c_double(0)
        _check(self.L.vc_get_frame(self.h, int(f), _d(T), _d(v), C.byref(t)), "GetFrame")
        return T, v, t.value

    def GetVelocities(self):
        n = self.NumFrames()
        v = np.zeros((n, 3))
        for f in range(n):
            v[f] = self.GetFrame(f)[1]
        return v

    def GetFrames(self):
        n = self.NumFrames()
        T = np.zeros((n, 7))
        for f in range(n):
            T[f] = self.GetFrame(f)[0]
        return T

    def GetBiases(self):
        b = np.zeros(6); _check(self.L.vc_get_biases(self.h, _d(b)), "GetBiases"); return b

    def GetScaleFactor(self):
        s = np.zeros(6); _check(self.L.vc_get_scale_factor(self.h, _d(s)), "GetScaleFactor"); return s

    def GetGravity(self):
        g = np.zeros(2); _check(self.L.vc_get_gravity(self.h, _d(g)), "GetGravity"); return g

    def time_offset(self): return self.L.vc_time_offset(self.h)
    def MeanSquaredError(self): return self.L.vc_mean_squared_error(self.h)

    def GetCameraProjRMSE(self):
        r = np.zeros(max(self.NumCameras(), 1)); _check(self.L.vc_get_camera_proj_rmse(self.h, _d(r)), "GetCameraProjRMSE")
        return r[:self.NumCameras()]

    def GetNumIterations(self): return self.L.vc_get_num_iterations(self.h)

    def imu_buffer(self):
        n = _check(self.L.vc_num_imu_measurements(self.h), "imu_buffer")
        g = np.zeros((n, 3)); a = np.zeros((n, 3)); t = np.zeros(n)
        _check(self.L.vc_get_imu_measurements(self.h, _d(g), _d(a), _d(t), n), "imu_buffer")
        return g, a, t

    def GetIntegrationPoses(self, frame_id):
        n = _check(self.L.vc_get_integration_poses(self.h, int(frame_id), None, 0), "GetIntegrationPoses")
        out = np.zeros((max(n, 1), 11))
        if n > 0:
            _check(self.L.vc_get_integration_poses(self.h, int(frame_id), _d(out), n), "GetIntegrationPoses")
        return out[:n]

    def PrintResults(self):
        for _ in range(8):
            n = _check(self.L.vc_print_results(self.h, None, 0), "PrintResults")
            buf = C.create_string_buffer(n + 65)
            if self.L.vc_print_results(self.h, buf, n + 65) >= 0:
                return buf.value.decode()
        raise VicalibError("PrintResults: the text kept growing")
    def WriteCameraModels(self, path): _check(self.L.vc_write_camera_models(self.h, path.encode()), "WriteCameraModels")

    def load_problem(self, prob, init=True):
        for c, m in enumerate(prob.cam_model):
            self.AddCamera(m, prob.cam_K_init[c] if init else prob.cam_K_gt[c], prob.cam_T_ck_init[c] if init else prob.cam_T_ck_gt[c],
                           prob.cfg.width, prob.cfg.height)
        T = prob.frame_T_wk_init if init else prob.frame_T_wk_gt
        for n in range(len(prob.frame_time)):
            self.AddFrame(T[n], prob.frame_time[n])
        if getattr(prob, "flat", None) is not None:
            tf, tc, off, ids, pix = prob.flat
            self.AddObservationTiles(tf, tc, off, prob.grid_points, ids, pix)
        else:
            for (f, c, ids, pix) in prob.tiles:
                self.AddObservations(f, c, prob.grid_points[ids], pix)
        if prob.imu_t is not None:
            self.AddImuMeasurements(prob.imu_gyro, prob.imu_accel, prob.imu_t)
        return self

    def trace(self):
        n = _check(self.L.vc_trace_len(self.h), "trace_len")
        out = np.zeros((max(n, 1), 10))
        _check(self.L.vc_get_trace(self.h, _d(out), n), "get_trace")
        return out[:n]

    def set_shard(self, rank, world, fn=None):
        self._cb = ALLREDUCE_FN(fn) if fn is not None else None
        _check(self.L.vc_set_shard(self.h, int(rank), int(world), self._cb, None), "set_shard")

    def set_shard_rccl(self, rank, world, group=None):
        import torch.distributed as dist
        buf = C.create_string_buffer(128)
        if rank == 0:
            _check(self.L.vc_rccl_unique_id(buf), "rccl_unique_id")
        box = [bytes(buf.raw)]
        if world > 1:
            dist.broadcast_object_list(box, src=0, group=group)
        rc = self.L.vc_set_shard_rccl(self.h, int(rank), int(world), C.create_string_buffer(box[0], 128))
        if rc != 0:
            raise VicalibError("set_shard_rccl: status %d: %s" % (rc, (self.L.vc_last_error() or b"").decode(errors="replace")))

    def set_shard_comm(self, comm):
        rc = self.L.vc_set_shard_comm(self.h, comm.h)
        if rc != 0:
            raise VicalibError("set_shard_comm: status %d: %s" % (rc, (self.L.vc_last_error() or b"").decode(errors="replace")))

    def allreduce_calls(self): return int(self.L.vc_allreduce_calls(self.h))

    def pass_paths(self):
        out = (C.c_int * 6)()
        _check(self.L.vc_pass_paths(self.h, out), "pass_paths")
        return dict(fold_l0=out[0], back_path=out[1], early_gram=out[2], top_gram_launch=out[3], tail_deferred=out[4], shared_blocks_ahead=out[5])

    def shard_info(self):
        v = [C.c_int(-1) for _ in range(4)]
        _check(self.L.vc_shard_info(self.h, *[C.byref(x) for x in v]), "shard_info")
        return dict(rank=v[0].value, world=v[1].value, rccl_ranks=v[2].value, rccl_rank=v[3].value)

    def stream(self): return self.L.vc_get_stream(self.h)
    def prepare(self): _check(self.L.vc_prepare(self.h), "prepare")
    def shared_dim(self): return _check(self.L.vc_shared_dim(self.h), "shared_dim")

    def linearize(self):
        self.prepare()
        n, D = self.NumFrames(), self.shared_dim()
        cost = C.c_double(0); H = np.zeros((n, 6, 6)); g = np.zeros((n, 6)); S = np.zeros((D, D)); gr = np.zeros(D); hd = np.zeros(D); gs = np.zeros(D)
        _check(self.L.vc_linearize(self.h, C.byref(cost), _d(H), _d(g), _d(S), _d(gr), _d(hd), _d(gs)), "linearize")
        return dict(cost=cost.value, Hpp=H, gp=g, S=S, g_red=gr, hss_diag=hd, g_s=gs)

    def step_hold(self, radius):
        self.prepare()
        n, D, nc = self.NumFrames(), self.shared_dim(), self.NumCameras()
        cost = C.c_double(0); ds = np.zeros(max(D, 1)); sl = np.zeros(max(D, 1)); fl = np.zeros((n, 9))
        T = np.zeros((n, 7)); v = np.zeros((n, 3)); cams = np.zeros((max(nc, 1), 17)); imus = np.zeros(15)
        _check(self.L.vc_step_hold(self.h, C.c_double(radius), C.byref(cost), _d(ds), _d(sl), _d(fl), _d(T), _d(v), _d(cams), _d(imus)), "step_hold")
        return dict(cost=cost.value, delta_s=ds[:D], slam=sl[:D], frame_lam=fl, poses=T, vels=v, cams=cams[:nc], imus=imus)

    def evaluate(self):
        cost = C.c_double(0); sq = C.c_double(0)
        _check(self.L.vc_evaluate(self.h, C.byref(cost), C.byref(sq)), "evaluate")
        return cost.value, sq.value

    def run_iterations(self, iters):
        j = C.c_int(0); r = C.c_int(0)
        n = _check(self.L.vc_run_iterations(self.h, int(iters), C.byref(j), C.byref(r)), "run_iterations")
        return n, j.value, r.value

    def download_state(self):
        _check(self.L.vc_download_state(self.h), "download_state")

    def time_kernels(self, reps=20):
        a = C.c_double(0); b = C.c_double(0)
        _check(self.L.vc_time_kernels(self.h, int(reps), C.byref(a), C.byref(b)), "time_kernels")
        return a.value, b.value

    def time_stages(self, reps=50):
        out = np.zeros(6)
        _check(self.L.vc_time_stages(self.h, int(reps), _d(out)), "time_stages")
        return dict(zip(["jac", "frame_schur", "-", "reduced", "trial", "final"], (out * 1e3).tolist()))

    def set_kernel_timing(self, on=True): _check(self.L.vc_set_kernel_timing(self.h, int(on)), "set_kernel_timing")

    def sync_timeouts(self):
        return int(self.L.vc_sync_timeouts(self.h))

    def kernel_timing(self):
        names = C.create_string_buffer(2048); tot = np.zeros(64); cnt = np.zeros(64, dtype=np.int64)
        n = _check(self.L.vc_get_kernel_timing(self.h, names, len(names), _d(tot), cnt.ctypes.data_as(C.c_void_p), 64), "kernel_timing")
        keys = names.value.decode().split(";") if n else []
        return {k: (int(cnt[i]), float(tot[i] / cnt[i])) for i, k in enumerate(keys)}

    def imu_weights(self):
        ns = self.num_imu_blocks()
        W = np.zeros((ns, 9, 9))
        _check(self.L.vc_get_imu_weights(self.h, _d(W)), "imu_weights")
        return W

    def GetSolutionCovariance(self):
        n = _check(self.L.vc_solution_covariance_dim(self.h), "solution_covariance_dim")
        cov = np.zeros((n, n)); m = C.c_int(0)
        _check(self.L.vc_get_solution_covariance(self.h, _d(cov), n, C.byref(m)), "solution_covariance")
        buf = C.create_string_buffer(64 * max(1, self.NumCameras()))
        _check(self.L.vc_get_solution_covariance_names(self.h, buf, len(buf)), "solution_covariance_names")
        return cov, buf.value.decode().split()

    def imu_blocks(self):
        ns = self.num_imu_blocks()
        H = np.zeros((ns, 33, 33)); g = np.zeros((ns, 33)); c = np.zeros(ns)
        _check(self.L.vc_get_imu_blocks(self.h, _d(H), _d(g), _d(c)), "imu_blocks")
        return H, g, c

    def report(self, bins=(16, 12), corners=True):
        bx, by = int(bins[0]), int(bins[1])
        _check(self.L.vc_report_compute(self.h, bx, by), "report_compute")
        vp = lambda a: a.ctypes.data_as(C.c_void_p)
        out = {"bins": (bx, by)}
        if corners:
            n = _check(self.L.vc_report_num_corners(self.h), "report_num_corners")
            r = np.zeros((n, 2)); fr = np.zeros(n, dtype=np.int32); cm = np.zeros(n, dtype=np.int32); fl = np.zeros(n, dtype=np.uint8)
            _check(self.L.vc_report_corners(self.h, C.c_longlong(0), C.c_longlong(n), _d(r), vp(fr), vp(cm), vp(fl)), "report_corners")
            out.update(r=r, frame=fr, camera=cm, flags=fl)
        nv = _check(self.L.vc_report_num_views(self.h), "report_num_views")
        v = dict(frame=np.zeros(nv, dtype=np.int32), camera=np.zeros(nv, dtype=np.int32), count=np.zeros(nv, dtype=np.int32), removed=np.zeros(nv, dtype=np.int32),
                 sum_sq=np.zeros(nv), max_err=np.zeros(nv), worst_corner=np.zeros(nv, dtype=np.int64))
        _check(self.L.vc_report_views(self.h, vp(v["frame"]), vp(v["camera"]), vp(v["count"]), vp(v["removed"]), vp(v["sum_sq"]), vp(v["max_err"]),
                                      vp(v["worst_corner"])), "report_views")
        out["views"] = v
        maps = np.zeros((self.NumCameras(), by, bx, 4))
        for c in range(self.NumCameras()):
            _check(self.L.vc_report_error_map(self.h, c, vp(maps[c])), "report_error_map")
        out["maps"] = maps
        nb = _check(self.L.vc_report_num_imu_blocks(self.h), "report_num_imu_blocks")
        w = np.zeros((nb, 9)); u = np.zeros((nb, 9)); f = np.zeros(nb, dtype=np.uint8)
        _check(self.L.vc_report_imu(self.h, vp(w), vp(u), vp(f)), "report_imu")
        out["imu"] = dict(whitened=w, unwhitened=u, flags=f)
        return out

    def time_report_sweeps(self, reps=20):
        out = np.zeros(3)
        _check(self.L.vc_time_report_sweeps(self.h, int(reps), _d(out)), "time_report_sweeps")
        return dict(vision=out[0], error_map=out[1], imu=out[2])

    HOLDOUT_STATUS = ("converged", "max_iters", "underdetermined", "no_seed", "failed")

    def HoldoutClear(self): _check(self.L.vc_holdout_clear(self.h), "HoldoutClear")

    def HoldoutAddTiles(self, tile_frame, tile_cam, tile_off, points, point_id, p_c):
        tf = np.ascontiguousarray(tile_frame, dtype=np.int32); tc = np.ascontiguousarray(tile_cam, dtype=np.int32)
        off = np.ascontiguousarray(tile_off, dtype=np.int64); pid = np.ascontiguousarray(point_id, dtype=np.int32)
        pts = np.ascontiguousarray(points, dtype=np.float64); pc = np.ascontiguousarray(p_c, dtype=np.float64)
        vp = lambda a: a.ctypes.data_as(C.c_void_p)
        _check(self.L.vc_holdout_add_tiles(self.h, len(tf), vp(tf), vp(tc), vp(off), vp(pts), len(pts), vp(pid), vp(pc)), "HoldoutAddTiles")

    def HoldoutCompute(self, seeds=None, max_iters=0, corners=True):
        sp = None
        if seeds is not None:
            seeds = np.ascontiguousarray(seeds, dtype=np.float64).reshape(-1, 7)
            sp = seeds.ctypes.data_as(C.c_void_p)
        _check(self.L.vc_holdout_compute(self.h, sp, int(max_iters)), "HoldoutCompute")
        return self.HoldoutResults(corners)

    def HoldoutResults(self, corners=True):
        vp = lambda a: a.ctypes.data_as(C.c_void_p)
        nf = _check(self.L.vc_holdout_num_frames(self.h), "holdout_num_frames")
        f = dict(T_wk=np.zeros((nf, 7)), status=np.zeros(nf, dtype=np.int32), iterations=np.zeros(nf, dtype=np.int32), cost0=np.zeros(nf), cost=np.zeros(nf),
                 behind=np.zeros(nf, dtype=np.int32))
        _check(self.L.vc_holdout_frames(self.h, vp(f["T_wk"]), vp(f["status"]), vp(f["iterations"]), vp(f["cost0"]), vp(f["cost"]), vp(f["behind"])), "holdout_frames")
        nv = _check(self.L.vc_holdout_num_views(self.h), "holdout_num_views")
        v = dict(frame=np.zeros(nv, dtype=np.int32), camera=np.zeros(nv, dtype=np.int32), count=np.zeros(nv, dtype=np.int32), sum_sq=np.zeros(nv), max_err=np.zeros(nv),
                 worst_corner=np.zeros(nv, dtype=np.int64))
        _check(self.L.vc_holdout_views(self.h, vp(v["frame"]), vp(v["camera"]), vp(v["count"]), vp(v["sum_sq"]), vp(v["max_err"]), vp(v["worst_corner"])), "holdout_views")
        out = dict(frames=f, views=v)
        if corners:
            n = _check(self.L.vc_holdout_num_corners(self.h), "holdout_num_corners")
            r = np.zeros((n, 2)); fr = np.zeros(n, dtype=np.int32); cm = np.zeros(n, dtype=np.int32)
            _check(self.L.vc_holdout_corners(self.h, C.c_longlong(0), C.c_longlong(n), vp(r), vp(fr), vp(cm)), "holdout_corners")
            out.update(r=r, frame=fr, camera=cm)
        nc = self.NumCameras()
        rm = np.zeros(max(nc, 1)); cnt = np.zeros(max(nc, 1), dtype=np.int64)
        _check(self.L.vc_holdout_camera_rmse(self.h, vp(rm), vp(cnt)), "holdout_camera_rmse")
        out.update(rmse=rm[:nc], count=cnt[:nc])
        return out

    def time_holdout(self, reps=20):
        out = np.zeros(2)
# ... 514 lines not shown
```

Measured before the change: 2.093 billion.

## Use odd-even (cyclic) reduction order for IMU chain groups across waves

Adds an odd-even elimination order for the per-group block-tridiagonal IMU chain: up to seven frames per group are eliminated in log-depth rounds spread over four waves with LDS exchange and barriers, replacing the sequential or two-sided sweep. The back-substitution kernels get a matching odd-even path, and the top gram kernel can run the new group solver. The aim is to shorten the serial dependency chain in the forward and backward chain solves. In exchange it adds more LDS, block barriers and fill-in arithmetic, and it only applies when the row fits in one 64-lane wave and the run is unsharded. An env switch and a query API are added.

```diff
diff --git a/include/vicalib_amd.h b/include/vicalib_amd.h
--- a/include/vicalib_amd.h
+++ b/include/vicalib_amd.h
@@ -101,6 +101,7 @@
 long long vc_allreduce_calls(vc_calibrator* h);
 int vc_shard_info(vc_calibrator* h, int* rank, int* world_size, int* rccl_ranks, int* rccl_rank);
 int vc_pass_paths(vc_calibrator* h, int* out6);
+int vc_chain_order(vc_calibrator* h, int* n_levels, int* oe_levels, int cap, int* oe_top);
 const char* vc_last_error(void);
 int vc_prepare(vc_calibrator* h);
 int vc_linearize(vc_calibrator* h, double* cost, double* Hpp, double* gp, double* S, double* g_red,
diff --git a/vicalib_amd/csrc/vc_capi.cpp b/vicalib_amd/csrc/vc_capi.cpp
--- a/vicalib_amd/csrc/vc_capi.cpp
+++ b/vicalib_amd/csrc/vc_capi.cpp
@@ -16,6 +16,7 @@
   w.pre_backsub = env_bit("VICALIB_AMD_PRE_BACKSUB");
   w.chain.fold_l0 = env_bit("VICALIB_AMD_FOLD_L0") != 0; w.chain.back_path = env_bit("VICALIB_AMD_BACK_PATH") != 0;
   w.chain.hadd_early = env_bit("VICALIB_AMD_HADD_EARLY") != 0; w.chain.defer_tail = env_bit("VICALIB_AMD_DEFER_TAIL") != 0;
+  w.chain.odd_even = env_bit("VICALIB_AMD_CHAIN_ODD_EVEN") != 0;
   return w;
 }
 
@@ -581,6 +582,13 @@
   out6[4] = p.tail_deferred; out6[5] = p.hadd_early;
   return VC_OK;
 }
+int vc_chain_order(vc_calibrator* h, int* n_levels, int* oe_levels, int cap, int* oe_top) {
+  if (!h || !n_levels || !oe_levels || !oe_top || cap < 0) return VC_ERR_BAD_ARG;
+  const ChainPlan& p = h->plan;
+  *n_levels = p.n_levels; *oe_top = p.oe_top;
+  for (int l = 0; l < cap; ++l) oe_levels[l] = l < p.n_levels ? p.oe[l] : 0;
+  return VC_OK;
+}
 void* vc_get_stream(vc_calibrator* h) { return h ? (void*)h->stream : nullptr; }
 int vc_prepare(vc_calibrator* h) {
   NOT_RUNNING(h);
diff --git a/vicalib_amd/csrc/vc_chain_order.hpp b/vicalib_amd/csrc/vc_chain_order.hpp
--- /dev/null
+++ b/vicalib_amd/csrc/vc_chain_order.hpp
@@ -0,0 +1,33 @@
+#pragma once
+
+#if defined(__HIPCC__) || defined(__CUDACC__)
+#define VC_ORDER_HD __host__ __device__
+#else
+#define VC_ORDER_HD
+#endif
+
+namespace vc {
+
+constexpr int kOeMaxQ = 7;
+constexpr int kOeMaxSteps = 3;
+constexpr int kOeWaves = 4;
+constexpr int kOeLeftSep = 0, kOeRightSep = -1, kOeNobody = -2;
+
+struct OeFrame { int step, left, right, wave; };
+
+VC_ORDER_HD constexpr int oe_low_bit(int i) { return i & -i; }
+VC_ORDER_HD constexpr int oe_steps(int q) { int k = 0; while ((1 << k) < q + 1) ++k; return k; }
+VC_ORDER_HD constexpr OeFrame oe_frame(int q, bool has_left, bool has_right, int i) {
+  const int h = oe_low_bit(i);
+  int k = 1;
+  while ((1 << (k - 1)) < h) ++k;
+  const int l = i - h, r = i + h;
+  return OeFrame{k, l >= 1 ? l : (has_left ? kOeLeftSep : kOeNobody), r <= q ? r : (has_right ? kOeRightSep : kOeNobody), (i - 1) / 2};
+}
+VC_ORDER_HD constexpr int oe_slot(int nb) { return nb == kOeRightSep ? kOeMaxQ + 1 : nb; }
+VC_ORDER_HD constexpr OeFrame oe_full(int i) { return oe_frame(kOeMaxQ, true, true, i); }
+VC_ORDER_HD constexpr int oe_last(int q) { return 1 << (oe_steps(q) - 1); }
+VC_ORDER_HD constexpr int oe_left_edge(int k) { return 1 << (k - 1); }
+VC_ORDER_HD constexpr int oe_right_edge(int k) { return kOeMaxQ + 1 - (1 << (k - 1)); }
+
+}
diff --git a/vicalib_amd/csrc/vc_chain_plan.hpp b/vicalib_amd/csrc/vc_chain_plan.hpp
--- a/vicalib_amd/csrc/vc_chain_plan.hpp
+++ b/vicalib_amd/csrc/vc_chain_plan.hpp
@@ -7,12 +7,14 @@
 constexpr int kChainMaxLevels = 16;
 constexpr int kChainEarlyTopD = 31;
 
-struct ChainSwitches { bool fold_l0 = true, back_path = true, hadd_early = true, defer_tail = true; };
+struct ChainSwitches { bool fold_l0 = true, back_path = true, hadd_early = true, defer_tail = true, odd_even = true; };
 
 struct ChainPlan {
   int n_levels = 0;
   int stride[kChainMaxLevels] = {}, m[kChainMaxLevels] = {}, groups[kChainMaxLevels] = {};
   int two[kChainMaxLevels] = {};
+  int oe[kChainMaxLevels] = {};
+  int oe_top = 0;
   int top_stride = 1;
   int forward_launches = 0;
   int bottom_groups = 1;
@@ -38,6 +40,8 @@
   if (p.n_levels > 0) p.bottom_groups = p.groups[0];
   const int cpl = (D + 1 + 27 + 63) / 64;
   for (int l = 0; l < p.n_levels; ++l) p.two[l] = (cpl <= 1 || (cpl <= 2 && p.groups[l] <= 256)) ? 1 : 0;
+  for (int l = 1; l < p.n_levels; ++l) p.oe[l] = (sw.odd_even && !sharded && p.two[l] && cpl <= 1) ? 1 : 0;
+  p.oe_top = (sw.odd_even && !sharded && cpl <= 1) ? 1 : 0;
   if (!imu_on) return p;
   p.fold_l0 = (sw.fold_l0 && !sharded && D + 1 + 27 <= 64 && n_cams <= 2 && p.n_levels >= 1) ? 1 : 0;
   p.gram_top_stride = (N <= 4096 && D + 1 + 27 <= 128) ? p.top_stride : 0;
diff --git a/vicalib_amd/csrc/vc_imu_kernels.hip b/vicalib_amd/csrc/vc_imu_kernels.hip
--- a/vicalib_amd/csrc/vc_imu_kernels.hip
+++ b/vicalib_amd/csrc/vc_imu_kernels.hip
@@ -5,6 +5,7 @@
 #include "vc_imu.hpp"
 #include "vc_imu_weights.hpp"
 #include "vc_device.h"
+#include "vc_chain_order.hpp"
 #include "vc_kutil.hpp"
 #include "vc_reduced_tail.hpp"
 #include "vc_shared_blocks.hpp"
@@ -1569,6 +1570,195 @@
   F2STAMP(14);
 }
 
+constexpr int kOeSlot = 9 * 64;
+constexpr int kOeWaveLds = 9 * kXsLd + 81 + 81 + 2;
+constexpr int kOeLds = kOeWaves * kOeWaveLds + 8 * kOeSlot;
+constexpr bool oe_closed_forms_match() {
+  for (int i = 1; i <= kOeMaxQ; ++i) {
+    const OeFrame f = oe_full(i);
+    const int h = 1 << (f.step - 1);
+    if (f.wave != (i - 1) / 2) return false;
+    if (i % h != 0 || ((i / h) & 1) != 1) return false;
+    if (oe_slot(f.left) != i - h || oe_slot(f.right) != i + h) return false;
+    for (int j = 1; j < f.step; ++j) {
+      const int hs = 1 << (j - 1);
+      if (oe_full(i - hs).step != j || oe_slot(oe_full(i - hs).right) != i) return false;
+      if (i + hs <= kOeMaxQ && (oe_full(i + hs).step != j || oe_slot(oe_full(i + hs).left) != i)) return false;
+    }
+  }
+  for (int q = 1; q <= kOeMaxQ; ++q) {
+    const OeFrame f = oe_frame(q, true, true, oe_last(q));
+    if (f.step != oe_steps(q) || f.left != kOeLeftSep || f.right != kOeRightSep) return false;
+    for (int k = 1; k <= oe_steps(q); ++k) if (oe_frame(q, true, true, oe_left_edge(k)).left != kOeLeftSep || oe_frame(q, true, true, oe_left_edge(k)).step != k) return false;
+  }
+  for (int k = 1; k <= kOeMaxSteps; ++k) if (oe_full(oe_right_edge(k)).right != kOeRightSep || oe_full(oe_right_edge(k)).step != k) return false;
+  return kOeWaves * 2 >= kOeMaxQ + 1 && kOeMaxQ == kChainM - 1;
+}
+static_assert(oe_closed_forms_match(), "the kernels' index arithmetic no longer matches vc_chain_order.hpp");
+__device__ __forceinline__ int oe_image(int i, int side) {
+  const int h = oe_low_bit(i);
+  return h == 1 ? i - 1 + side : (side == 0 ? i - h / 2 : i + h / 2 - 1);
+}
+__device__ __forceinline__ void oe_round_barrier() {
+  __builtin_amdgcn_fence(__ATOMIC_RELEASE, "wavefront");
+  __builtin_amdgcn_s_waitcnt(0xc07f);
+  __builtin_amdgcn_s_barrier();
+  __builtin_amdgcn_fence(__ATOMIC_ACQUIRE, "wavefront");
+}
+__device__ __forceinline__ void chain_oe_group(const DevView& v, int s, int lvl, int top, int group, double* lds) {
+  const int wv = __builtin_amdgcn_readfirstlane((int)(threadIdx.x >> 6)), lane = threadIdx.x & 63;
+  const int N = v.n_frames, D = v.D, ldw = v.ldw, ldx = v.ldx, nW = D + 1, ncol = nW + 27;
+  const long gs = (long)kChainM * s;
+  const int a = top ? -1 : (int)((long)group * gs), first = top ? 0 : a + s;
+  const int done = v.ctrl->done;
+  if (lvl == 1 && blockIdx.x == 0 && threadIdx.x == 0) signal_started(v, 7);
+  const bool pend = lvl > 0;
+  const double* rp = v.rX[(lvl + 1) & 1];
+  double* rw = v.rX[lvl & 1];
+  const size_t isz = (size_t)9 * ldx;
+  const int c = lane, e0 = c - nW;
+  const int role = c < nW ? 0 : (e0 < 9 ? 1 : e0 < 18 ? 2 : e0 < 27 ? 3 : 4);
+  const int pc = c < nW ? c : (c < ncol ? ldw + e0 : 0);
+  const int sub = e0 < 9 ? e0 : e0 < 18 ? e0 - 9 : e0 - 18;
+  if (first >= N) {
+    if (!done && wv == 0 && !top && a < N) {
+      double* img = v.cW + (size_t)a * isz + pc;
+      if ((role == 0 || role == 2) && pend && a > 0) {
+#pragma unroll
+        for (int k = 0; k < 9; ++k) img[k * ldx] += rp[(size_t)(a / s) * isz + k * ldx + pc];
+      } else if (role == 3) {
+#pragma unroll
+        for (int k = 0; k < 9; ++k) img[k * ldx] = 0.0;
+      }
+    }
+    return;
+  }
+  const int q = top ? (N - 1) / s + 1 : min(kOeMaxQ, (N - 1 - first) / s + 1);
+  const int r = first + q * s;
+  const bool has_l = !top, has_r = !top && q == kOeMaxQ && r < N;
+  const int K = oe_steps(q), ilast = oe_last(q), wfin = (ilast - 1) / 2;
+  const int ia = 2 * wv + 1, ib = 2 * wv + 2;
+  const bool have_a = ia <= q, have_b = ib <= q;
+  const int sb = oe_frame(q, has_l, has_r, ib).step;
+  double* XS = lds + wv * kOeWaveLds; double* An = XS + 9 * kXsLd; double* Ls = An + 81;
+  double* IMG = lds + kOeWaves * kOeWaveLds;
+  const int base = top ? -s : a, pq = top ? -1 : group * kChainM;
+  const unsigned ldxb = 8u * (unsigned)ldx, iszb = 9u * ldxb;
+  auto load_cols = [&](int i, bool round1, double* x) {
+    const int e = base + i * s;
+    const bool has_left = i > 1 || has_l;
+    const bool tr = round1 && role == 1;
+    const unsigned c0b = tr ? 8u * (unsigned)(sub * ldx + ldw + 18) : 8u * (unsigned)pc, stb = tr ? 8u : ldxb;
+    const unsigned fb = (unsigned)((tr && has_left) ? e - s : e) * iszb, pb = (unsigned)(pq + i) * iszb;
+    const bool live0 = role == 0 || role == 2 || (round1 && (role == 3 || (role == 1 && has_left)));
+    const bool live1 = pend && e > 0 && (role == 0 || role == 2);
+    double y0[9], y1[9];
+#pragma unroll
+    for (int k = 0; k < 9; ++k) y0[k] = ld_boff(v.cW, fb + c0b + k * stb);
+    if (pend) {
+#pragma unroll
+      for (int k = 0; k < 9; ++k) y1[k] = ld_boff(rp, pb + c0b + k * stb);
+    } else {
+#pragma unroll
+      for (int k = 0; k < 9; ++k) y1[k] = 0.0;
+    }
+#pragma unroll
+    for (int k = 0; k < 9; ++k) x[k] = (live0 ? y0[k] : 0.0) + (live1 ? y1[k] : 0.0);
+  };
+  double xa[9], xb[9], sep0[9];
+#pragma unroll
+  for (int k = 0; k < 9; ++k) { xa[k] = 0.0; xb[k] = 0.0; sep0[k] = 0.0; }
+  if (have_a) load_cols(ia, true, xa);
+  if (have_b) load_cols(ib, false, xb);
+  {
+    const bool pa = pend && a > 0, mine = has_l && wv == wfin && (role == 0 || role == 1);
+    const int pcd = role == 1 ? ldw + 9 + sub : pc;
+    const unsigned c0b = 8u * (unsigned)pcd;
+    const unsigned ab = (unsigned)(has_l ? a : 0) * iszb, pab = (unsigned)(has_l ? a / s : 0) * iszb;
+    double y0[9], y1[9];
+#pragma unroll
+    for (int k = 0; k < 9; ++k) y0[k] = ld_boff(v.cW, ab + c0b + k * ldxb);
+    if (pend) {
+#pragma unroll
+      for (int k = 0; k < 9; ++k) y1[k] = ld_boff(rp, pab + c0b + k * ldxb);
+    } else {
+#pragma unroll
+      for (int k = 0; k < 9; ++k) y1[k] = 0.0;
+    }
+#pragma unroll
+    for (int k = 0; k < 9; ++k) sep0[k] = mine ? y0[k] + (pa ? y1[k] : 0.0) : 0.0;
+  }
+  if (done) return;
+  const ElimLds elds = {XS, An, Ls};
+  double out[18];
+#pragma unroll
+  for (int k = 0; k < 18; ++k) out[k] = 0.0;
+  for (int st = 1; st <= K; ++st) {
+    if (st > 1) {
+      oe_round_barrier();
+      if (have_b && sb >= st) {
+        const int hs = 1 << (st - 2), il = ib - hs, ir = ib + hs;
+        const bool has_rs = ir <= q, fin = sb == st;
+        const double* L = IMG + oe_image(il, 1) * kOeSlot + c;
+        const double* R = IMG + oe_image(has_rs ? ir : il, 0) * kOeSlot + (role == 2 ? c - 9 : c);
+        double fl[9], fr[9];
+#pragma unroll
+        for (int k = 0; k < 9; ++k) { fl[k] = L[k * 64]; fr[k] = R[k * 64]; }
+#pragma unroll
+        for (int k = 0; k < 9; ++k) {
+          const double l = fl[k], r = has_rs ? fr[k] : 0.0;
+          const double acc = (xb[k] - l) - r;
+          const double cpl = role == 1 ? -l : -r;
+          xb[k] = (role == 0 || role == 2) ? acc : ((fin && (role == 1 || role == 3)) ? cpl : 0.0);
+        }
+      }
+    }
+    const int i = st == 1 ? (have_a ? ia : 0) : ((have_b && sb == st) ? ib : 0);
+    if (i > 0) {
+      double x[9];
+#pragma unroll
+      for (int k = 0; k < 9; ++k) x[k] = st == 1 ? xa[k] : xb[k];
+      if (role == 2) {
+#pragma unroll
+        for (int k = 0; k < 9; ++k) An[k * 9 + sub] = x[k];
+      }
+      chain_eliminate<false>(v, v.cW + (size_t)(base + i * s) * isz, ldx, role, pc, sub, c == 0, elds, x, out);
+      if (i != ilast) {
+        double* L = IMG + oe_image(i, 0) * kOeSlot + c;
+        double* R = IMG + oe_image(i, 1) * kOeSlot + c;
+#pragma unroll
+        for (int k = 0; k < 9; ++k) { L[k * 64] = out[k]; R[k * 64] = out[9 + k]; }
+      }
+    }
+  }
+  if (wv != wfin || !has_l) return;
+  double dl_[9], dr_[9];
+#pragma unroll
+  for (int k = 0; k < 9; ++k) { dl_[k] = 0.0; dr_[k] = 0.0; }
+  for (int st = 1; st < K; ++st) {
+    const double* L = IMG + oe_image(oe_left_edge(st), 0) * kOeSlot + c;
+    const double* R = IMG + oe_image(oe_right_edge(st), 1) * kOeSlot + c;
+#pragma unroll
+    for (int k = 0; k < 9; ++k) { dl_[k] += L[k * 64]; if (has_r) dr_[k] += R[k * 64]; }
+  }
+  if (has_r && role < 4) {
+    double* ri = rw + (size_t)(r / gs) * isz + pc;
+    const bool keep = role == 0 || role == 2;
+#pragma unroll
+    for (int k = 0; k < 9; ++k) ri[k * ldx] = keep ? -(dr_[k] + out[9 + k]) : 0.0;
+  }
+  if (role == 3) {
+    double* img = v.cW + (size_t)a * isz + pc;
+#pragma unroll
+    for (int k = 0; k < 9; ++k) img[k * ldx] = has_r ? -out[k] : 0.0;
+  }
+  if (role == 0 || role == 1) {
+    const int pcd = role == 1 ? ldw + 9 + sub : pc;
+    double* img = v.cW + (size_t)a * isz + pcd;
+#pragma unroll
+    for (int k = 0; k < 9; ++k) img[k * ldx] = sep0[k] - (dl_[k] + out[k]);
+  }
+}
 constexpr int kL0Ld = 48;
 template <int CMAX>
 __global__ __launch_bounds__(256) void k_chain_l0(DevView v) {
@@ -2093,7 +2283,55 @@
 #define BSTAMP(i) do { } while (0)
 #endif
 constexpr int kBackT0Frames = 1;
-struct BackLevels { int n; int start[8]; int stride[8]; int m[8]; int two[8]; };
+struct BackLevels { int n; int start[8]; int stride[8]; int m[8]; int two[8] ; };
+__device__ __forceinline__ double chain_back_oe(int q, int fi, int k, double t, const double* Xs, const double* Qrow, const double* Lcol, double dinv,
+                                                const double* da, const double* dr) {
+  double d[kOeMaxQ + 2][9];
+#pragma unroll
+  for (int j = 0; j < 9; ++j) {
+    d[0][j] = da[j]; d[kOeMaxQ + 1][j] = dr[j];
+#pragma unroll
+    for (int i = 1; i <= kOeMaxQ; ++i) d[i][j] = 0.0;
+  }
+  double my = 0.0;
+#pragma unroll
+  for (int st = kOeMaxSteps; st >= 1; --st) {
+    const int h = 1 << (st - 1);
+    if (h <= q) {
+      double y[4];
+#pragma unroll
+      for (int u = 0; u < 4; ++u) {
+        const int i = h * (2 * u + 1);
+        y[u] = t;
+        if (i <= kOeMaxQ) {
+          const OeFrame f = oe_full(i);
+#pragma unroll
+          for (int c = 0; c < 9; ++c) y[u] += Xs[c] * d[oe_slot(f.left)][c] + Qrow[c] * d[oe_slot(f.right)][c];
+        }
+      }
+#pragma unroll
+      for (int j = 8; j >= 0; --j) {
+#pragma unroll
+        for (int u = 0; u < 4; ++u) {
+          const int i = h * (2 * u + 1);
+          if (i <= kOeMaxQ) {
+            const double xj = readlane_f64(y[u] * dinv, (i - 1) * 9 + j);
+            if (i <= q) { d[i][j] = -xj; y[u] -= Lcol[j] * xj; }
+          }
+        }
+      }
+#pragma unroll
+      for (int u = 0; u < 4; ++u) {
+        const int i = h * (2 * u + 1);
+        if (i <= kOeMaxQ && i <= q && fi == i - 1) {
+#pragma unroll
+          for (int j = 0; j < 9; ++j) my = (j == k) ? d[i][j] : my;
+        }
+      }
+    }
+  }
+  return my;
+}
 template <bool FUSED>
 __device__ __forceinline__ void chain_back_group(const DevView& v, int s, int m, int top, int lvl, int two, int group, double* ds, double* dl) {
   const int done = v.ctrl->done;
@@ -2118,7 +2356,8 @@
   const int fi = lane / 9, k = lane % 9;
   const bool mine = fi < q;
   const int e = first + (mine ? fi : 0) * s;
-  const bool two_sided = two && !top && q >= 1;
+  const bool two_sided = two == 1 && !top && q >= 1;
+  const bool oe = two == 2;
   const int fmid = (q - 1) / 2;
   double t = 0.0, dinv = 1.0, Qrow[9], Lcol[9];
 #pragma unroll
@@ -2140,7 +2379,7 @@
   }
   double Xs[9];
 #pragma unroll
-  for (int c = 0; c < 9; ++c) Xs[c] = (mine && a >= 0) ? v.cW[(size_t)e * isz + (size_t)k * ldx + ldw + c] : 0.0;
+  for (int c = 0; c < 9; ++c) Xs[c] = (mine && (a >= 0 || oe)) ? v.cW[(size_t)e * isz + (size_t)k * ldx + ldw + c] : 0.0;
   if (done) return;
   if (FUSED) {
     if (lane == 0) {
@@ -2163,7 +2402,7 @@
       dn[k2] = has_r ? __hip_atomic_load(v.cdelta + (size_t)r * 9 + k2, __ATOMIC_RELAXED, __HIP_MEMORY_SCOPE_AGENT) : 0.0;
     }
   }
-  if (mine && a >= 0) {
+  if (mine && a >= 0 && !oe) {
     const bool right = two_sided && fi > fmid;
 #pragma unroll
     for (int c = 0; c < 9; ++c) t += Xs[c] * (right ? dn[c] : da[c]);
@@ -2174,7 +2413,8 @@
 #endif
   BSTAMP(2);
   double my = 0.0;
-  if (two_sided) {
+  if (oe) my = chain_back_oe(q, fi, k, t, Xs, Qrow, Lcol, dinv, da, dn);
+  else if (two_sided) {
     {
       double y = t;
 #pragma unroll
@@ -2349,7 +2589,7 @@
   chain_back_group<true>(v, L.stride[li], L.m[li], 0, lvl, L.two[li], (int)blockIdx.x - L.start[li], ds, dl);
 }
 
-struct BackPath { int n; int stride[6]; int m[6]; int two[6]; int top_stride; int ldr; int dsw; int tail; };
+struct BackPath { int n; int stride[6]; int m[6]; int two[6] ; int oe_top; int top_stride; int ldr; int dsw; int tail; };
 constexpr int kTailLds = kMaxCams * kCamStride + 16 + 8 + 6 * 256;
 __device__ __forceinline__ void reduced_tail_workgroup(const DevView& v, double* lds) {
   const int tid = threadIdx.x, D = v.D;
@@ -2405,7 +2645,7 @@
   const size_t isz = (size_t)9 * ldx;
   const bool top = wv == P.n;
   const int lvl = top ? P.n : wv;
-  const int s = top ? P.top_stride : P.stride[lvl], m = top ? kChainM : P.m[lvl], two = top ? 0 : P.two[lvl];
+  const int s = top ? P.top_stride : P.stride[lvl], m = top ? kChainM : P.m[lvl], two = top ? (P.oe_top ? 2 : 0) : P.two[lvl];
   const long gs = (long)m * s;
   const long a0 = (long)blockIdx.x * P.m[0] * P.stride[0];
   const int a = top ? -1 : (int)((a0 / gs) * gs);
@@ -2416,7 +2656,8 @@
   const int fi = lane / 9, k = lane % 9;
   const bool mine = fi < q;
   const int e = first + (mine ? fi : 0) * s;
-  const bool two_sided = two && !top && q >= 1;
+  const bool two_sided = two == 1 && !top && q >= 1;
+  const bool oe = two == 2;
   const int fmid = (q - 1) / 2;
   const int ncolr = D + 1, nel = q * 9 * ncolr;
   double rv[CT0 ? 1 : kPathRowLoads];
@@ -2445,7 +2686,7 @@
 #pragma unroll
     for (int c = 0; c < 9; ++c) {
       const double qv = Wr[ldw + 18 + c], lv = img[c * ldx + ldw + 9 + k], xv = Wr[ldw + c];
-      Qrow[c] = mine ? qv : 0.0; Lcol[c] = (mine && c > k) ? lv : 0.0; Xs[c] = (mine && a >= 0) ? xv : 0.0;
+      Qrow[c] = mine ? qv : 0.0; Lcol[c] = (mine && c > k) ? lv : 0.0; Xs[c] = (mine && (a >= 0 || oe)) ? xv : 0.0;
     }
     const double dg = Wr[ldw + 9 + k];
     dinv = mine ? 1.0 / dg : 1.0;
@@ -2491,13 +2732,14 @@
   }
 #pragma unroll
   for (int c = 0; c < 9; ++c) dr_in[c] = dn[c];
-  if (mine && a >= 0) {
+  if (mine && a >= 0 && !oe) {
     const bool right = two_sided && fi > fmid;
 #pragma unroll
     for (int c = 0; c < 9; ++c) t += Xs[c] * (right ? dn[c] : da[c]);
   }
   double my = 0.0;
-  if (two_sided) {
+  if (oe) my = chain_back_oe(q, fi, k, t, Xs, Qrow, Lcol, dinv, da, dn);
+  else if (two_sided) {
     {
       double y = t;
 #pragma unroll
@@ -2706,13 +2948,14 @@
   else chain_gram_chunk<NQ, NL>(v, (int)blockIdx.x, R, s_pair, v.gram_top_stride);
 }
 template <int NW, int NQ, int NL>
-__global__ __launch_bounds__(256) void k_chain_top_gram(DevView v, int s, int m, int lvl) {
+__global__ __launch_bounds__(256) void k_chain_top_gram(DevView v, int s, int m, int lvl, int oe) {
   extern __shared__ __attribute__((aligned(16))) double R[];
   __shared__ unsigned short s_pair[128];
   __shared__ __attribute__((aligned(16))) double XS[9 * kXsLd];
   __shared__ double An[81];
   __shared__ double Ls_all[NW * 81];
   if (blockIdx.x == 0) {
+    if (NW == 1 && oe) { chain_oe_group(v, s, lvl, 1, 0, R); return; }
     if ((int)threadIdx.x >= 64 * NW) return;
     chain_fwd_group<1, NW>(v, s, m, 1, lvl, 0, (int)(threadIdx.x >> 6), XS, An, Ls_all);
     return;
@@ -2720,6 +2963,12 @@
   if ((int)blockIdx.x == 1 + v.n_chunks) { hadd_side_job(v, R, 256); return; }
   if ((int)blockIdx.x > 1 + v.n_chunks) { part_sum_ride_job(v, (int)blockIdx.x - 2 - v.n_chunks, R); return; }
   chain_gram_chunk<NQ, NL>(v, (int)blockIdx.x - 1, R, s_pair, v.gram_top_stride, 0, v.part_ride != 0);
+}
+
+__global__ __launch_bounds__(256) void k_chain_oe(DevView v, int s, int lvl, int top, int n_groups) {
+  __shared__ __attribute__((aligned(16))) double oe_lds[kOeLds];
+  if ((int)blockIdx.x >= n_groups) { if (threadIdx.x < 128) part_tail_sum_job(v, (int)blockIdx.x - n_groups, oe_lds, 128); return; }
+  chain_oe_group(v, s, lvl, top, (int)blockIdx.x, oe_lds);
 }
 
 void launch_imu_delta(const DevView& v, hipStream_t s, int trial) {
@@ -2741,8 +2990,11 @@
   const int nl = p.n_levels, top_stride = p.top_stride, m_top = kChainM;
   const int cpl = (v.D + 1 + 27 + 63) / 64;
   auto fwd = [&](int groups, int stride, int m, int top, int lvl) {
-    if (!top && p.two[lvl]) {
-      const int extra = (v.hadd_early && lvl == 1) ? (v.part_stride - (v.D * v.D + v.D) + 15) / 16 : 0;
+    const int extra = (!top && v.hadd_early && lvl == 1) ? (v.part_stride - (v.D * v.D + v.D) + 15) / 16 : 0;
+    if (top ? p.oe_top : p.oe[lvl]) {
+      hipLaunchKernelGGL(k_chain_oe, dim3(groups + extra), dim3(256), 0, s, v, stride, lvl, top, groups);
+    }
+    else if (!top && p.two[lvl]) {
       if (cpl <= 1) hipLaunchKernelGGL(k_chain_fwd2<1>, dim3(groups + extra), dim3(128), 0, s, v, stride, m, lvl, groups);
       else hipLaunchKernelGGL(k_chain_fwd2<2>, dim3(groups + extra), dim3(256), 0, s, v, stride, m, lvl, groups);
     }
@@ -2759,13 +3011,14 @@
       } else fwd(p.groups[l], p.stride[l], p.m[l], 0, l);
     }
     if (v.gram_top_stride > 0) {
-      const size_t lds = std::max((size_t)36 * v.ldw, (size_t)(v.hadd_early ? kHaddLds : 0)) * sizeof(double);
+      const size_t lds_gram = std::max((size_t)36 * v.ldw, (size_t)(v.hadd_early ? kHaddLds : 0)) * sizeof(double);
+      const size_t lds = std::max(lds_gram, (size_t)(p.oe_top ? kOeLds : 0) * sizeof(double));
       const int ride_blocks = (v.part_ride && v.hadd_early) ? (v.D * v.D + v.D + 15) / 16 : 0;
       const int nT = (v.D + 1 + 15) / 16, nPairs = nT * (nT + 1) / 2, nq = std::min(kMaxPairsPerWaveI, (nPairs + 3) / 4);
       const int nlr = (36 * v.ldw + 255) / 256;
       auto go = [&](auto kern) {
-        if (lds > 40000) (void)hipFuncSetAttribute((const void*)kern, hipFuncAttributeMaxDynamicSharedMemorySize, (int)lds);
-        hipLaunchKernelGGL(kern, dim3(1 + v.n_chunks + (v.hadd_early ? 1 : 0) + ride_blocks), dim3(256), lds, s, v, top_stride, m_top, nl);
+        if (lds_gram > 40000) (void)hipFuncSetAttribute((const void*)kern, hipFuncAttributeMaxDynamicSharedMemorySize, (int)lds);
+        hipLaunchKernelGGL(kern, dim3(1 + v.n_chunks + (v.hadd_early ? 1 : 0) + ride_blocks), dim3(256), lds, s, v, top_stride, m_top, nl, p.oe_top);
       };
       if (cpl <= 1) { if (nq <= 1) go(k_chain_top_gram<1, 1, 7>); else go(k_chain_top_gram<1, 2, 7>); }
       else if (cpl <= 2) { if (nlr <= 12) go(k_chain_top_gram<2, 4, 12>); else if (nq <= 6) go(k_chain_top_gram<2, 6, 16>); else go(k_chain_top_gram<2, 9, 16>); }
@@ -2777,9 +3030,9 @@
   } else {
     if (v.back_path && nl >= 1 && nl <= 5) {
       BackPath P; P.n = nl;
-      for (int l = 0; l < 6; ++l) { P.stride[l] = l < nl ? p.stride[l] : 1; P.m[l] = l < nl ? p.m[l] : 2; P.two[l] = l < nl ? p.two[l] : 0; }
+      for (int l = 0; l < 6; ++l) { P.stride[l] = l < nl ? p.stride[l] : 1; P.m[l] = l < nl ? p.m[l] : 2; P.two[l] = l < nl ? (p.oe[l] ? 2 : p.two[l]) : 0; }
       const bool ct0 = v.D + 1 > kPathRowCols;
-      P.top_stride = top_stride; P.ldr = ct0 ? 1 : ((v.D + 1) | 1); P.dsw = ((v.D + 63) / 64) * 64;
+      P.oe_top = p.oe_top; P.top_stride = top_stride; P.ldr = ct0 ? 1 : ((v.D + 1) | 1); P.dsw = ((v.D + 63) / 64) * 64;
       if (ct0) hipLaunchKernelGGL(k_chain_t0, dim3((N + 3) / 4), dim3(256), 0, s, v);
       const int nw = nl + 1;
       P.tail = (v.tail_deferred && nw >= 4) ? 1 : 0;
@@ -2793,7 +3046,7 @@
       else { if (ct0) go(k_chain_back_path<6, true>, g6); else go(k_chain_back_path<6, false>, g6); }
       return;
     }
-    hipLaunchKernelGGL(k_chain_back, dim3(1 + (nl > 0 ? (N + kBackT0Frames - 1) / kBackT0Frames : 0)), dim3(64), 0, s, v, top_stride, m_top, 1, nl, 0);
+    hipLaunchKernelGGL(k_chain_back, dim3(1 + (nl > 0 ? (N + kBackT0Frames - 1) / kBackT0Frames : 0)), dim3(64), 0, s, v, top_stride, m_top, 1, nl, p.oe_top ? 2 : 0);
     int total_groups = 0;
     for (int l = 0; l < nl; ++l) total_groups += p.groups[l];
     static const int resident_limit = [] {
@@ -2807,14 +3060,14 @@
       int at = 0;
       for (int i = 0; i < nl; ++i) {
         const int l = nl - 1 - i;
-        L.start[i] = at; L.stride[i] = p.stride[l]; L.m[i] = p.m[l]; L.two[i] = p.two[l];
+        L.start[i] = at; L.stride[i] = p.stride[l]; L.m[i] = p.m[l]; L.two[i] = p.oe[l] ? 2 : p.two[l];
         at += p.groups[l];
       }
       for (int i = nl; i < 8; ++i) { L.start[i] = 1 << 30; L.stride[i] = 1; L.m[i] = 2; L.two[i] = 0; }
       hipLaunchKernelGGL(k_chain_back_levels, dim3(at), dim3(64), 0, s, v, L);
     } else
     for (int l = nl - 1; l >= 0; --l)
-      hipLaunchKernelGGL(k_chain_back, dim3(p.groups[l]), dim3(64), 0, s, v, p.stride[l], p.m[l], 0, l, p.two[l]);
+      hipLaunchKernelGGL(k_chain_back, dim3(p.groups[l]), dim3(64), 0, s, v, p.stride[l], p.m[l], 0, l, p.oe[l] ? 2 : p.two[l]);
   }
 }
 void launch_chain_init(const DevView& v, hipStream_t s) {
diff --git a/vicalib_amd/lib.py b/vicalib_amd/lib.py
--- a/vicalib_amd/lib.py
+++ b/vicalib_amd/lib.py
@@ -21,7 +21,7 @@
     "vc_get_biases", "vc_get_scale_factor", "vc_get_gravity", "vc_time_offset", "vc_mean_squared_error", "vc_get_camera_proj_rmse",
     "vc_get_num_iterations", "vc_num_imu_measurements", "vc_get_imu_measurements", "vc_get_integration_poses", "vc_print_results", "vc_write_camera_models", "vc_trace_len", "vc_get_trace", "vc_set_shard", "vc_get_stream", "vc_prepare",
     "vc_linearize", "vc_step_hold", "vc_shared_dim", "vc_run_iterations", "vc_download_state", "vc_evaluate", "vc_time_kernels", "vc_time_stages", "vc_get_imu_blocks", "vc_get_debug_stamps", "vc_num_observations", "vc_num_tiles",
-    "vc_init_frame_poses_pnp", "vc_pnp_planar", "vc_pnp_planar_ransac", "vc_set_pnp_ransac", "vc_rccl_unique_id", "vc_set_shard_rccl", "vc_shard_comm_create", "vc_set_shard_comm", "vc_shard_comm_destroy", "vc_allreduce_calls", "vc_shard_info", "vc_pass_paths", "vc_last_error", "vc_get_imu_weights",
+    "vc_init_frame_poses_pnp", "vc_pnp_planar", "vc_pnp_planar_ransac", "vc_set_pnp_ransac", "vc_rccl_unique_id", "vc_set_shard_rccl", "vc_shard_comm_create", "vc_set_shard_comm", "vc_shard_comm_destroy", "vc_allreduce_calls", "vc_shard_info", "vc_pass_paths", "vc_chain_order", "vc_last_error", "vc_get_imu_weights",
     "vc_solution_covariance_dim", "vc_get_solution_covariance", "vc_get_solution_covariance_names",
     "vc_target_make_pattern", "vc_target_find",
     "vc_report_compute", "vc_report_num_corners", "vc_report_corners", "vc_report_num_views", "vc_report_views", "vc_report_error_map", "vc_report_num_imu_blocks", "vc_report_imu", "vc_time_report_sweeps",
@@ -341,6 +341,11 @@
         out = (C.c_int * 6)()
         _check(self.L.vc_pass_paths(self.h, out), "pass_paths")
         return dict(fold_l0=out[0], back_path=out[1], early_gram=out[2], top_gram_launch=out[3], tail_deferred=out[4], shared_blocks_ahead=out[5])
+
+    def chain_order(self):
+        n, top, oe = C.c_int(0), C.c_int(0), (C.c_int * 16)()
+        _check(self.L.vc_chain_order(self.h, C.byref(n), oe, 16, C.byref(top)), "chain_order")
+        return dict(n_levels=n.value, oe=[int(oe[l]) for l in range(n.value)], oe_top=top.value)
 
     def shard_info(self):
         v = [C.c_int(-1) for _ in range(4)]
```

Measured after the change: 2.186 billion (median of 6 runs). +4.4%, better.
